# hyperplane-lab/RGBManip

Hardware: AMD Instinct MI355X
Metric: adapose_poses_per_sec_batch256 (higher is better)
Workload: dtype bf16

## Files before the change

include/rgbm.h:

```cpp
#ifndef RGBM_H_
#define RGBM_H_
#include <stddef.h>
#include <stdint.h>

#ifdef __cplusplus
extern "C" {
#endif

#define RGBM_VERSION 100
#define RGBM_F32 0
#define RGBM_BF16 1
#define RGBM_F16 2
#define RGBM_BF16X3 3

int rgbm_version(void);
const char* rgbm_last_error(void);

typedef struct rgbm_weight_desc {
  const char* name;
  const float* data;
  int ndim;
  const int64_t* shape;
} rgbm_weight_desc;

// ... 67 lines not shown
int rgbm_depth_fusion(const float* depth, const float* conf, const uint8_t* mask, const double* Kcrop, const double* E, int n, int V, int S,
                      double px_max, double rel_max, float conf_min, int n_min, float* fused, uint8_t* keep, uint8_t* nviews, uint16_t* agree,
                      void* stream);
int rgbm_cloud_pack_views(const float* fused, const uint8_t* keep, const double* Kcrop, const double* E, int n, int V, int S, int cap,
                          float* cloud, int32_t* index, int32_t* count, void* stream);
int rgbm_cloud_gather_views(const float* maps, const int32_t* index, int n, int V, int S2, int C, int cap, float* out, void* stream);

int rgbm_adapose_postprocess(int B, int P, int img_size, const float* nocs1, const float* depth1, const float* r1,
                             const int32_t* choose1, const double* Kcrop, const double* E1, double* bbox_world, double* ts,
                             int32_t* valid, void* stream);
int rgbm_adapose_postprocess_scratch_bytes(int B, size_t* bytes);
int rgbm_adapose_postprocess_ws(int B, int P, int img_size, const float* nocs1, const float* depth1, const float* r1,
                                const int32_t* choose1, const double* Kcrop, const double* E1, double* bbox_world, double* ts,
                                int32_t* valid, void* scratch, size_t scratch_bytes, void* stream);

int rgbm_adapose_postprocess_regressed(int B, int P, const float* nocs1, const float* r1, const float* t1, const float* s1,
                                       const double* E1, double* bbox_world, double* ts, int32_t* valid, void* stream);

int rgbm_adapose_postprocess_ransac(int B, int P, int img_size, uint32_t seed, const float* nocs1, const float* depth1,
                                    const int32_t* choose1, const double* Kcrop, const double* E1, double* bbox_world, double* srt,
                                    int32_t* valid, void* stream);
int rgbm_adapose_postprocess_pnp(int B, int P, uint32_t seed, const float* nocs1, const float* pts2d1, const float* nocs2,
                                 const float* pts2d2, const double* K, const double* E1, const double* E2, double* bbox_out,
                                 double* srt_out, int32_t* info_out, int32_t* valid_out, void* stream);

int rgbm_prepare_inputs(const float* rgb_dev, const uint8_t* mask_dev, const double* K_dev, int N, int H, int W, int S, int P,
                        uint32_t seed, float* img_out, int32_t* choose_out, float* pts2d_out, double* Kcrop_out,
                        int32_t* window_out, int32_t* valid_out, uint8_t* scratch, void* stream);

int rgbm_prepare_inputs_indexed(const float* rgb_dev, const uint8_t* mask_dev, const double* K_dev, const int32_t* frame_map_dev,
                                int N, int H, int W, int S, int P, uint32_t seed, float* img_out, int32_t* choose_out,
                                float* pts2d_out, double* Kcrop_out, int32_t* window_out, int32_t* valid_out, uint8_t* scratch,
                                void* stream);
int rgbm_prepare_inputs_ex(const float* rgb_dev, const uint8_t* mask_dev, const double* K_dev, const int32_t* frame_map_dev,
                           int frame0, int N, int H, int W, int S, int P, uint32_t seed, float* img_out, int32_t* choose_out,
                           float* pts2d_out, double* Kcrop_out, int32_t* window_out, int32_t* valid_out, uint8_t* scratch,
                           void* stream);
int rgbm_prepare_inputs_u8(const uint8_t* rgb_dev, const uint8_t* mask_dev, const double* K_dev, const int32_t* frame_map_dev,
                           int frame0, int N, int H, int W, int S, int P, uint32_t seed, float* img_out, int32_t* choose_out,
                           float* pts2d_out, double* Kcrop_out, int32_t* window_out, int32_t* valid_out, uint8_t* scratch,
                           void* stream);
int rgbm_prepare_inputs_opt(const void* rgb_dev, int pixel_type, int normalize, const uint8_t* mask_dev, const double* K_dev,
                            const int32_t* frame_map_dev, int frame0, int N, int H, int W, int S, int P, uint32_t seed, float* img_out,
                            int32_t* choose_out, float* pts2d_out, double* Kcrop_out, int32_t* window_out, int32_t* valid_out,
                            uint8_t* scratch, void* stream);
int rgbm_prepare_inputs_windows(const void* pix_dev, int pixel_type, int normalize, const uint8_t* mask_pix_dev, const int64_t* offset_dev,
                                const int32_t* window_dev, const int32_t* valid_in_dev, const double* K_dev, int frame0, int N, int H, int W,
                                int S, int P, uint32_t seed, float* img_out, int32_t* choose_out, float* pts2d_out, double* Kcrop_out,
                                int32_t* valid_out, uint8_t* scratch, void* stream);
int rgbm_quantize_frames(const float* src_dev, uint8_t* dst_dev, size_t n, void* stream);

int rgbm_projection(const double* Kcrop_dev, const double* E_dev, float* P_dev, int N, void* stream);
int rgbm_mask_extent(const uint8_t* mask_dev, int N, int H, int W, int32_t* ext_out, int32_t* count_out, void* stream);

int rgbm_lookat_quat(const double* dir_dev, int N, int batch_zero, double* quat_dev, void* stream);
int rgbm_control_action_to_pose(const float* action_dev, int lda, const double* pose_mid, const double* pose_min,
                                const double* pose_max, int N, double* pose_dev, void* stream);
typedef struct rgbm_control_reward_args {
  const float* action;
  const double* cam_pose;
  const double* target;
  const float* move_success;
  const double* bbox;
  const double* avail;
  const double* gt_bbox;
  const double* pred_bbox;
  const double* pose_cur;
  const double* pose_prev;
  const double* robot_pose;
  const double* success;
  double* reward;
  double* terms;
  double coef[14];
  double proper_pos[3];
  double precision2;
  int N, T, lda, pots, first;
  int pad_;
} rgbm_control_reward_args;
int rgbm_control_reward(const rgbm_control_reward_args* args, void* stream);
int rgbm_control_grasp_frame(const double* est_dev, int N, double* center_dev, double* direction_dev, void* stream);

typedef struct rgbm_synth_scene {
  const double* cam_pose;
  const double* robot_pose;
  const double* box;
  double fx, fy, cx, cy;
  int N, H, W, env0;
} rgbm_synth_scene;
int rgbm_synth_camera(const rgbm_synth_scene* scene, double* K_dev, double* E_dev, double* rays_dev, void* stream);
int rgbm_synth_render(const rgbm_synth_scene* scene, const double* rays_dev, float* color_dev, uint8_t* mask_dev, void* stream);
int rgbm_synth_render_u8(const rgbm_synth_scene* scene, const double* rays_dev, uint8_t* color_dev, uint8_t* mask_dev,
                         int32_t* extent_dev, int32_t* count_dev, void* stream);

int rgbm_gae(int T, int N, const float* rewards, const uint8_t* dones, const float* values, const float* last_values,
             float gamma, float lam, float* returns, float* adv, double* sums, void* stream);
int rgbm_adv_normalise(int64_t n_local, float* adv, const double* sums, double count_total, void* stream);

typedef struct rgbm_policy_layout {
  int dims[5];
  int log_std;
  int w[2][4];
  int b[2][4];
  int total;
} rgbm_policy_layout;
int rgbm_policy_forward(const float* params, const rgbm_policy_layout* L, int n, int mode, const float* obs, const float* noise,
                        float* actions, float* logp, float* value, float* mu, void* stream);
int rgbm_ppo_partial_floats(const rgbm_policy_layout* L, int n, size_t* count);
int rgbm_ppo_minibatch_fwd_bwd(const float* params, const rgbm_policy_layout* L, int n, const float* obs, const float* actions,
                               const float* old_logp, const float* adv, const float* returns, const float* old_values,
                               const float* old_mu, const float* old_log_std, float clip, float vcoef, float ecoef,
                               float* partial_scratch, float* grads_flat, void* stream);
int rgbm_ppo_clip_adam(float* params, const float* grads_flat, float* exp_avg, float* exp_avg_sq, void* opt_state,
                       const rgbm_policy_layout* L, float inv_world, float max_norm, float desired_kl, float lr_min,
                       float lr_max, int adaptive, void* stream);

#define RGBM_POLICY_MAX_HIDDEN 6
#define RGBM_POLICY_MAX_WIDTH 512
#define RGBM_POLICY_MAX_ACT 32
#define RGBM_ACT_ELU 0
#define RGBM_ACT_SELU 1
#define RGBM_ACT_RELU 2
#define RGBM_ACT_LRELU 3
#define RGBM_ACT_TANH 4
#define RGBM_ACT_SIGMOID 5
typedef struct rgbm_policy_desc {
  int obs_dim, state_dim, act_dim;
  int activation;
  int asymmetric;
  int n_hidden[2];
  int hidden[2][RGBM_POLICY_MAX_HIDDEN];
  int w[2][RGBM_POLICY_MAX_HIDDEN + 1];
  int b[2][RGBM_POLICY_MAX_HIDDEN + 1];
  int log_std;
  int total;
} rgbm_policy_desc;
int rgbm_policy_forward_ex(const float* params, const rgbm_policy_desc* D, int n, int mode, const float* obs, const float* states,
                           const float* noise, float* actions, float* logp, float* value, float* mu, void* stream);
int rgbm_ppo_scratch_floats_ex(const rgbm_policy_desc* D, int n, int clipped_value_loss, size_t* count);
int rgbm_ppo_minibatch_fwd_bwd_ex(const float* params, const rgbm_policy_desc* D, int n, const float* obs, const float* states,
                                  const float* actions, const float* old_logp, const float* adv, const float* returns,
                                  const float* old_values, const float* old_mu, const float* old_log_std, float clip, float vcoef,
                                  float ecoef, int clipped_value_loss, float* scratch, float* grads_flat, void* stream);
int rgbm_ppo_clip_adam_ex(float* params, const float* grads_flat, float* exp_avg, float* exp_avg_sq, void* opt_state, int total,
                          float inv_world, float max_norm, float desired_kl, float lr_min, float lr_max, int adaptive, void* stream);

int rgbm_conv_nd(int dtype, const void* in_dev, int N, int D, int H, int W, int Cin, int Cin_pad, const float* w_host,
                 int Cout, int Cout_pad, int KD, int KH, int KW, int stride_d, int stride_hw, int pad_d, int pad_hw,
                 int dil_hw, int transposed, const float* bias_host, const float* bn_scale_host, const float* bn_shift_host,
                 const void* res_dev, int res_mode, int act, float slope, void* out_dev, void* stream);
#define RGBM_CONV_PLAN_INTS 9
int rgbm_conv_plan(int dtype, int N, int D, int H, int W, int Cin, int Cin_pad, int Cout, int Cout_pad, int KD, int KH, int KW,
                   int stride_d, int stride_hw, int pad_d, int pad_hw, int dil_hw, int transposed, int has_bias, int res_mode, int act,
                   int cls, int n_cu, int32_t* plan);
int rgbm_bn_per_sample_scratch_bytes(int V, size_t* bytes);
int rgbm_bn_per_sample(int dtype, void* y_dev, const void* res_dev, const float* gamma_dev, const float* beta_dev, void* scratch_dev,
                       int V, int64_t nvox, int C, int relu, void* stream);
int rgbm_conv3d_tile(int layer, int dtype, const void* in_dev, int N, int D, int H, int W, const float* w_host,
                     const float* bn_scale_host, const float* bn_shift_host, const void* res_dev, void* out_dev, void* stream);
int rgbm_upsample_conv3x3(int dtype, const void* in_dev, int V, int h, int w, int Cin, const float* w_host, int Cout,
                          const float* bias_host, int act, float slope, void* z_scratch_dev, void* out_dev, void* stream);
int rgbm_upsample_conv3x3_final(int dtype, const void* in_dev, int V, int h, int w, const float* w3_host, const float* b3_host,
                                float slope, const float* wf_host, const float* bf_host, void* out_dev, int out_f32, void* stream);
int rgbm_stem(int dtype, const float* img1_dev, const float* img2_dev, const float* w_host, void* out_dev, int B, int S, void* stream);
int rgbm_maxpool3x3s2(int dtype, const void* in_dev, void* out_dev, int V, int H, int W, int C, void* stream);
int rgbm_resize_bilinear_ac(int dtype, const void* in_dev, void* out_dev, int V, int Hs, int Ws, int C, int Ho, int Wo,
                            void* stream);
int rgbm_adaptive_avgpool(int dtype, const void* in_dev, void* out_dev, int V, int H, int W, int C, int S, void* stream);
int rgbm_build_volume(int dtype, const void* feat_dev, const float* P_views_dev, const float* depths_dev, float* homog_scratch,
                      void* vol_dev, int V, int B, int D, int H, int W, void* stream);
int rgbm_conv0_sweep(const void* feat_dev, const float* P_views_dev, const float* depths_dev, float* homog_scratch,
                     const float* w_host, const float* bn_scale_host, const float* bn_shift_host, void* out_dev,
                     int V, int B, int D, int H, int W, void* stream);
int rgbm_conv0_sweep_dt(int dtype, const void* feat_dev, const float* P_views_dev, const float* depths_dev, float* homog_scratch,
                        const float* w_host, const float* bn_scale_host, const float* bn_shift_host, void* out_dev,
                        int V, int B, int D, int H, int W, void* stream);
int rgbm_conv0_sweep_f16feat(const void* feat_f16_dev, const float* P_views_dev, const float* depths_dev, float* homog_scratch,
                             const float* w_host, const float* bn_scale_host, const float* bn_shift_host, void* out_bf16_dev,
                             int V, int B, int D, int H, int W, void* stream);
int rgbm_adapose_forward_ex(rgbm_adapose_t* h, int B, const float* img1, const float* img2, const int32_t* choose1,
                            const int32_t* choose2, const float* P1, const float* P2, const float* depths, void* workspace,
                            size_t workspace_bytes, const rgbm_adapose_out* out, int stop_after, void* stream);
int rgbm_adapose_forward_graph(rgbm_adapose_t* h, int B, const float* img1, const float* img2, const int32_t* choose1,
                               const int32_t* choose2, const float* P1, const float* P2, const float* depths, void* workspace,
                               size_t workspace_bytes, const rgbm_adapose_out* out, void* stream, int32_t* n_nodes, int32_t* captured);
int rgbm_adapose_graph_clear(rgbm_adapose_t* h);
int rgbm_adapose_feature_bytes(rgbm_adapose_t* h, size_t* bytes);
int rgbm_adapose_features_workspace_bytes(rgbm_adapose_t* h, int V, size_t* bytes);
int rgbm_adapose_features(rgbm_adapose_t* h, int V, const float* img, const int32_t* slots_dev, void* pool, int pool_records,
                          void* workspace, size_t workspace_bytes, void* stream);
int rgbm_adapose_forward_cached(rgbm_adapose_t* h, int B, const void* pool, int pool_records, const int32_t* slot1_dev,
                                const int32_t* slot2_dev, const int32_t* choose1, const int32_t* choose2, const float* P1, const float* P2,
                                const float* depths, void* workspace, size_t workspace_bytes, const rgbm_adapose_out* out, void* stream);
int rgbm_adapose_fetch(rgbm_adapose_t* h, int B, void* workspace, const char* name, float* out_dev, size_t capacity,
                       size_t* n_elems, void* stream);
int rgbm_crop_fingerprint(const float* img, int V, int n_words, uint64_t* keys_out, void* stream);

#define RGBM_PROF_ROWS 42
int rgbm_debug_flags(int flags);
int rgbm_set_tuning(const char* key, long long value);
int rgbm_microbench_mfma_scratch_floats(int* n);
int rgbm_microbench_mfma(float* scratch, int iters, int random_operands, double* flops, void* stream);
int rgbm_microbench_copy(const void* src, void* dst, size_t bytes, void* stream);
int rgbm_prof_rows(void);
int rgbm_prof_start(void);
int rgbm_prof_stop(double* stats);
int rgbm_prof_select(int row);

#ifdef __cplusplus
}
#endif
#endif
```

rgbmanip_amd/_lib.py:

```python
from __future__ import annotations

import ctypes as C
import os

_HERE = os.path.dirname(os.path.abspath(__file__))
LIB_PATH = os.environ.get("RGBM_HIP_LIB") or os.path.join(_HERE, "librgbm_hip.so")

F32, BF16, F16, BF16X3 = 0, 1, 2, 3
ACT_NONE, ACT_RELU, ACT_PRELU, ACT_TANH = 0, 1, 2, 3
RES_NONE, RES_PRE_ACT, RES_POST_ACT = 0, 1, 2


PROF_ROWS = 42
PROF_KERNELS = [
    ("conv_igemm_glds_kernel<float, 16, 256>", "fp32"), ("conv_igemm_glds_kernel<float, 32, 256>", "fp32"),
    ("conv_igemm_glds_kernel<float, 64, 256>", "fp32"), ("conv_igemm_glds_kernel<float, 128, 128>", "fp32"),
    ("conv_igemm_glds_kernel<unsigned short, 16, 256>", "bf16"), ("conv_igemm_glds_kernel<unsigned short, 32, 256>", "bf16"),
    ("conv_igemm_glds_kernel<unsigned short, 64, 256>", "bf16"), ("conv_igemm_glds_kernel<unsigned short, 128, 128>", "bf16"),
    ("conv3d_tile_kernel<float, ...> (conv1..conv11)", "fp32"), ("conv3d_tile_kernel<unsigned short, ...> (conv1..conv11)", "bf16"),
    ("conv3d_tile_kernel<float, 32, 16, 4, 8, 8, 1, false, true> (conv0 + fused plane sweep)", "fp32"),
    ("conv3d_tile_kernel<unsigned short, 32, 16, 4, 8, 8, 1, false, true> (conv0 + fused plane sweep)", "bf16"),
    ("conv_igemm_ws_kernel<float, ...>", "fp32"), ("conv_igemm_ws_kernel<unsigned short, false, false> (128 channels x 256 pixels)", "bf16"),
    ("conv0_sweep_persistent_kernel<unsigned short> (conv0 + fused plane sweep of bf16 nets; sweep_f16 = 0 / fp16 nets: conv0_sweep_kernel)", "bf16"), ("conv_igemm_ws64_kernel", "bf16"),
    ("conv3d_tile_kernel<unsigned short, 32, 16, 6, 8, 8, 1, false, false> (conv0 on a materialised volume)", "bf16"),
    ("conv3d_tile_kernel<unsigned short, 8, 16, 2, 8, 8, 2, false, false> (conv1)", "bf16"),
    ("conv3d_tile_kernel<unsigned short, 16, 16, 4, 8, 8, 1, false, false> (conv2)", "bf16"),
    ("conv3d_tile_kernel<unsigned short, 16, 32, 2, 8, 8, 2, false, false> (conv3)", "bf16"),
    ("conv3d_tile_kernel<unsigned short, 32, 32, 2, 8, 8, 1, false, false> (conv4)", "bf16"),
    ("conv3d_tile_kernel<unsigned short, 32, 64, 1, 8, 8, 2, false, false> (conv5)", "bf16"),
    ("conv3d_tile_kernel<unsigned short, 64, 64, 1, 8, 8, 1, false, false> (conv6)", "bf16"),
    ("conv3d_tile_kernel<unsigned short, 64, 32, 1, 8, 8, 1, true, false> (conv7)", "bf16"),
    ("conv3d_tile_kernel<unsigned short, 32, 16, 2, 8, 8, 1, true, false> (conv9)", "bf16"),
    ("conv3d_tile_kernel<unsigned short, 16, 16, 4, 8, 8, 1, true, false> (conv11)", "bf16"),
] + [("conv_igemm_glds_kernel<bx3_t, ...> (all channel tiles)", "bf16x3"), ("conv3d_tile_kernel<bx3_t, ...> (conv1..conv11)", "bf16x3"),
     ("conv0 + fused plane sweep <bx3_t>", "bf16x3"), ("conv_igemm_ws_kernel<rgbm::bx3_t, false, false> (128 channels x 256 pixels)", "bf16x3"),
     ("pose_mlp1_kernel (pose_mlp1.0 + pose_mlp1.2 of a bf16 net in one launch)", "bf16"),
     ("conv_igemm_m32_kernel<unsigned short, 256, 256> (256 channels x 256 pixels, 32x32x16 MFMAs; gemm_kernel = 0: conv_igemm_ws_kernel<unsigned short, true, false>, 256 x 128)", "bf16"),
     ("pose_mlp2_kernel (pose_mlp2.0 + pose_mlp2.2 + the sum over points of a bf16 net in one launch)", "bf16"),
     ("conv_igemm_m32_kernel<rgbm::bx3_t, 256, 256> (256 channels x 256 pixels, 32x32x16 MFMAs; gemm_kernel = 0: conv_igemm_ws_kernel<rgbm::bx3_t, true, false>, 256 x 128)", "bf16x3"),
     ("conv_igemm_ws_kernel<rgbm::bx3_t, false, false, true> (64 channels x 256 pixels, four multiply waves)", "bf16x3"),
     ("conv_igemm_ws_kernel<unsigned short, false, false, true> (64 channels x 256 pixels, four multiply waves)", "bf16"),
     ("conv_igemm_ws_kernel<float, false, false, true> (64 channels x 256 pixels, four multiply waves)", "fp32"),
     ("upconv_combine_kernel<16-bit> (PSPUpsample tap combination)", "bf16"), ("upconv_combine_kernel<4-byte> (PSPUpsample tap combination)", "bf16x3"),
     ("upconv_final_kernel (up_3 + final in one kernel; either storage width)", "bf16"),
     ("conv_igemm_m32_kernel<unsigned short, 128, 64 / 128 / 256> (128-pixel tiles: tail and small-batch launches of the 256-channel GEMM)", "bf16"),
     ("conv_igemm_m32_kernel<rgbm::bx3_t, 128, 64 / 128 / 256> (128-pixel tiles: tail and small-batch launches of the 256-channel GEMM)", "bf16x3")]
assert len(PROF_KERNELS) == PROF_ROWS


class RgbmError(RuntimeError):
    pass


class WeightDesc(C.Structure):
    _fields_ = [("name", C.c_char_p), ("data", C.c_void_p), ("ndim", C.c_int), ("shape", C.POINTER(C.c_int64))]


class PolicyLayout(C.Structure):
    _fields_ = [("dims", C.c_int * 5), ("log_std", C.c_int), ("w", (C.c_int * 4) * 2), ("b", (C.c_int * 4) * 2), ("total", C.c_int)]


POLICY_MAX_HIDDEN, POLICY_MAX_WIDTH, POLICY_MAX_ACT = 6, 512, 32
POLICY_ACTIVATIONS = {"elu": 0, "selu": 1, "relu": 2, "crelu": 2, "lrelu": 3, "tanh": 4, "sigmoid": 5}


class PolicyDesc(C.Structure):
    _fields_ = [("obs_dim", C.c_int), ("state_dim", C.c_int), ("act_dim", C.c_int), ("activation", C.c_int), ("asymmetric", C.c_int),
                ("n_hidden", C.c_int * 2), ("hidden", (C.c_int * POLICY_MAX_HIDDEN) * 2),
                ("w", (C.c_int * (POLICY_MAX_HIDDEN + 1)) * 2), ("b", (C.c_int * (POLICY_MAX_HIDDEN + 1)) * 2),
                ("log_std", C.c_int), ("total", C.c_int)]


class AdaposeOut(C.Structure):
    _fields_ = [(n, C.c_void_p) for n in ("view1_nocs", "view2_nocs", "view1_depth", "view2_depth", "view1_r", "view2_r",
                                           "view1_t", "view2_t", "view1_s", "view2_s")]


class ControlRewardArgs(C.Structure):
    _fields_ = [(n, C.c_void_p) for n in ("action", "cam_pose", "target", "move_success", "bbox", "avail", "gt_bbox", "pred_bbox",
                                           "pose_cur", "pose_prev", "robot_pose", "success", "reward", "terms")] + [
        ("coef", C.c_double * 14), ("proper_pos", C.c_double * 3), ("precision2", C.c_double),
        ("N", C.c_int), ("T", C.c_int), ("lda", C.c_int), ("pots", C.c_int), ("first", C.c_int), ("pad_", C.c_int)]


class SynthScene(C.Structure):
    _fields_ = [("cam_pose", C.c_void_p), ("robot_pose", C.c_void_p), ("box", C.c_void_p),
                ("fx", C.c_double), ("fy", C.c_double), ("cx", C.c_double), ("cy", C.c_double),
                ("N", C.c_int), ("H", C.c_int), ("W", C.c_int), ("env0", C.c_int)]


_vp, _i, _f, _d, _sz, _i64 = C.c_void_p, C.c_int, C.c_float, C.c_double, C.c_size_t, C.c_int64

SIGNATURES = {
    "rgbm_version": (_i, []),
    "rgbm_last_error": (C.c_char_p, []),
    "rgbm_adapose_create": (_i, [C.POINTER(_vp), _i, C.POINTER(WeightDesc), _i, _i, _i]),
    "rgbm_adapose_create_baseline": (_i, [C.POINTER(_vp), _i, C.POINTER(WeightDesc), _i, _i, _i]),
    "rgbm_view_fusion": (_i, [_vp, _vp, _vp, _i, _i, _vp, _vp, _vp, _sz, _vp]),
    "rgbm_view_fusion_scratch_bytes": (_i, [_i, _i, C.POINTER(_sz)]),
    "rgbm_depth_head": (_i, [_vp, _vp, _i64, _vp, _vp]),
    "rgbm_adapose_destroy": (_i, [_vp]),
    "rgbm_adapose_set_chunk": (_i, [_vp, _i]),
    "rgbm_adapose_set_option": (_i, [_vp, C.c_char_p, _i]),
    "rgbm_adapose_workspace_bytes": (_i, [_vp, _i, C.POINTER(_sz)]),
    "rgbm_adapose_set_dropout": (_i, [_vp, _f, C.c_uint64]),
    "rgbm_adapose_dropout_masks": (_i, [_vp, _i, _vp]),
    "rgbm_adapose_set_dropout_masks": (_i, [_vp, _i, _vp]),
    "rgbm_adapose_forward": (_i, [_vp, _i, _vp, _vp, _vp, _vp, _vp, _vp, _vp, _vp, _sz, C.POINTER(AdaposeOut), _vp]),
    "rgbm_adapose_forward_ex": (_i, [_vp, _i, _vp, _vp, _vp, _vp, _vp, _vp, _vp, _vp, _sz, C.POINTER(AdaposeOut), _i, _vp]),
    "rgbm_adapose_forward_graph": (_i, [_vp, _i, _vp, _vp, _vp, _vp, _vp, _vp, _vp, _vp, _sz, C.POINTER(AdaposeOut), _vp, C.POINTER(C.c_int32),
                                        C.POINTER(C.c_int32)]),
    "rgbm_adapose_samples_workspace_bytes": (_i, [_vp, _i, _i, C.POINTER(_sz)]),
    "rgbm_adapose_forward_samples": (_i, [_vp, _i, _i, _vp, _vp, _vp, _vp, _vp, _vp, _vp, _vp, _sz, C.POINTER(AdaposeOut), _vp]),
    "rgbm_sample_box_stats": (_i, [_vp, _vp, _i, _i, _vp, _vp, _vp, _vp, _vp, _vp, _vp, _vp, _vp]),
    "rgbm_sample_point_stats": (_i, [_vp, _i, _i, _i64, _vp, _vp, _vp]),
    "rgbm_box_agreement": (_i, [_vp, _vp, _vp, _vp, _i] + [_vp] * 14),
    "rgbm_box_iou_matrix": (_i, [_vp, _vp, _vp, _vp, _i, _i, _i, _vp, _vp]),
    "rgbm_adapose_dense_workspace_bytes": (_i, [_vp, _i, C.POINTER(_sz)]),
    "rgbm_adapose_forward_dense": (_i, [_vp, _i, _vp, _vp, _vp, _vp, _vp, _vp, _vp, _vp, _sz, C.POINTER(AdaposeOut), _vp, _vp, _vp]),
    "rgbm_adapose_forward_maps": (_i, [_vp, _i, _vp, _vp, _vp, _vp, _vp, _vp, _vp, _vp, _sz, C.POINTER(AdaposeOut), _vp, _vp, _vp, _vp]),
    "rgbm_nocs_map": (_i, [_vp, _vp, _i, _i, _vp, _vp]),
    "rgbm_cloud_gather": (_i, [_vp, _vp, _vp, _i, _i, _i, _i, _vp, _vp]),
    "rgbm_cloud_similarity_scratch_bytes": (_i, [_i, _i, C.POINTER(_sz)]),
    "rgbm_cloud_similarity": (_i, [_vp, _vp, _vp, _i, _i, C.c_uint32, _vp, _vp, _vp, _vp, _vp, _sz, _vp]),
    "rgbm_depth_to_points": (_i, [_vp, _vp, _vp, _i, _i, _vp, _vp]),
    "rgbm_depth_consistency": (_i, [_vp, _vp, _vp, _vp, _vp, _vp, _vp, _vp, _i, _i, _d, _d, _f, _vp, _vp, _vp, _vp, _vp]),
    "rgbm_cloud_pack": (_i, [_vp, _vp, _vp, _vp, _vp, _vp, _vp, _vp, _i, _i, _i, _vp, _vp, _vp, _vp]),
    "rgbm_depth_fusion": (_i, [_vp, _vp, _vp, _vp, _vp, _i, _i, _i, _d, _d, _f, _i, _vp, _vp, _vp, _vp, _vp]),
    "rgbm_cloud_pack_views": (_i, [_vp, _vp, _vp, _vp, _i, _i, _i, _i, _vp, _vp, _vp, _vp]),
    "rgbm_cloud_gather_views": (_i, [_vp, _vp, _i, _i, _i, _i, _i, _vp, _vp]),
    "rgbm_adapose_graph_clear": (_i, [_vp]),
    "rgbm_adapose_feature_bytes": (_i, [_vp, C.POINTER(_sz)]),
    "rgbm_adapose_features_workspace_bytes": (_i, [_vp, _i, C.POINTER(_sz)]),
    "rgbm_adapose_features": (_i, [_vp, _i, _vp, _vp, _vp, _i, _vp, _sz, _vp]),
    "rgbm_adapose_forward_cached": (_i, [_vp, _i, _vp, _i, _vp, _vp, _vp, _vp, _vp, _vp, _vp, _vp, _sz, C.POINTER(AdaposeOut), _vp]),
    "rgbm_crop_fingerprint": (_i, [_vp, _i, _i, _vp, _vp]),
    "rgbm_adapose_fetch": (_i, [_vp, _i, _vp, C.c_char_p, _vp, _sz, C.POINTER(_sz), _vp]),
    "rgbm_adapose_postprocess": (_i, [_i, _i, _i, _vp, _vp, _vp, _vp, _vp, _vp, _vp, _vp, _vp, _vp]),
    "rgbm_adapose_postprocess_scratch_bytes": (_i, [_i, C.POINTER(_sz)]),
    "rgbm_adapose_postprocess_ws": (_i, [_i, _i, _i, _vp, _vp, _vp, _vp, _vp, _vp, _vp, _vp, _vp, _vp, _sz, _vp]),
    "rgbm_adapose_postprocess_regressed": (_i, [_i, _i, _vp, _vp, _vp, _vp, _vp, _vp, _vp, _vp, _vp]),
    "rgbm_adapose_postprocess_ransac": (_i, [_i, _i, _i, C.c_uint32, _vp, _vp, _vp, _vp, _vp, _vp, _vp, _vp, _vp]),
    "rgbm_adapose_postprocess_pnp": (_i, [_i, _i, C.c_uint32, _vp, _vp, _vp, _vp, _vp, _vp, _vp, _vp, _vp, _vp, _vp, _vp]),
    "rgbm_gae": (_i, [_i, _i, _vp, _vp, _vp, _vp, _f, _f, _vp, _vp, _vp, _vp]),
    "rgbm_adv_normalise": (_i, [_i64, _vp, _vp, _d, _vp]),
    "rgbm_policy_forward": (_i, [_vp, _vp, _i, _i, _vp, _vp, _vp, _vp, _vp, _vp, _vp]),
    "rgbm_ppo_partial_floats": (_i, [_vp, _i, C.POINTER(_sz)]),
    "rgbm_ppo_minibatch_fwd_bwd": (_i, [_vp, _vp, _i, _vp, _vp, _vp, _vp, _vp, _vp, _vp, _vp, _f, _f, _f, _vp, _vp, _vp]),
    "rgbm_ppo_clip_adam": (_i, [_vp, _vp, _vp, _vp, _vp, _vp, _f, _f, _f, _f, _f, _i, _vp]),
    "rgbm_policy_forward_ex": (_i, [_vp, _vp, _i, _i, _vp, _vp, _vp, _vp, _vp, _vp, _vp, _vp]),
    "rgbm_ppo_scratch_floats_ex": (_i, [_vp, _i, _i, C.POINTER(_sz)]),
    "rgbm_ppo_minibatch_fwd_bwd_ex": (_i, [_vp, _vp, _i, _vp, _vp, _vp, _vp, _vp, _vp, _vp, _vp, _vp, _f, _f, _f, _i, _vp, _vp, _vp]),
    "rgbm_ppo_clip_adam_ex": (_i, [_vp, _vp, _vp, _vp, _vp, _i, _f, _f, _f, _f, _f, _i, _vp]),
    "rgbm_conv_nd": (_i, [_i, _vp, _i, _i, _i, _i, _i, _i, _vp, _i, _i, _i, _i, _i, _i, _i, _i, _i, _i, _i, _vp, _vp, _vp,
                          _vp, _i, _i, _f, _vp, _vp]),
    "rgbm_conv_plan": (_i, [_i] * 23 + [C.POINTER(C.c_int32)]),
    "rgbm_bn_per_sample_scratch_bytes": (_i, [_i, C.POINTER(_sz)]),
    "rgbm_bn_per_sample": (_i, [_i, _vp, _vp, _vp, _vp, _vp, _i, _i64, _i, _i, _vp]),
    "rgbm_conv3d_tile": (_i, [_i, _i, _vp, _i, _i, _i, _i, _vp, _vp, _vp, _vp, _vp, _vp]),
    "rgbm_upsample_conv3x3": (_i, [_i, _vp, _i, _i, _i, _i, _vp, _i, _vp, _i, _f, _vp, _vp, _vp]),
    "rgbm_upsample_conv3x3_final": (_i, [_i, _vp, _i, _i, _i, _vp, _vp, _f, _vp, _vp, _vp, _i, _vp]),
    "rgbm_stem": (_i, [_i, _vp, _vp, _vp, _vp, _i, _i, _vp]),
    "rgbm_maxpool3x3s2": (_i, [_i, _vp, _vp, _i, _i, _i, _i, _vp]),
    "rgbm_resize_bilinear_ac": (_i, [_i, _vp, _vp, _i, _i, _i, _i, _i, _i, _vp]),
    "rgbm_adaptive_avgpool": (_i, [_i, _vp, _vp, _i, _i, _i, _i, _i, _vp]),
    "rgbm_build_volume": (_i, [_i, _vp, _vp, _vp, _vp, _vp, _i, _i, _i, _i, _i, _vp]),
    "rgbm_conv0_sweep": (_i, [_vp, _vp, _vp, _vp, _vp, _vp, _vp, _vp, _i, _i, _i, _i, _i, _vp]),
    "rgbm_conv0_sweep_dt": (_i, [_i, _vp, _vp, _vp, _vp, _vp, _vp, _vp, _vp, _i, _i, _i, _i, _i, _vp]),
    "rgbm_conv0_sweep_f16feat": (_i, [_vp, _vp, _vp, _vp, _vp, _vp, _vp, _vp, _i, _i, _i, _i, _i, _vp]),
    "rgbm_prepare_inputs": (_i, [_vp, _vp, _vp, _i, _i, _i, _i, _i, C.c_uint32, _vp, _vp, _vp, _vp, _vp, _vp, _vp, _vp]),
    "rgbm_prepare_inputs_indexed": (_i, [_vp, _vp, _vp, _vp, _i, _i, _i, _i, _i, C.c_uint32, _vp, _vp, _vp, _vp, _vp, _vp, _vp, _vp]),
    "rgbm_prepare_inputs_ex": (_i, [_vp, _vp, _vp, _vp, _i, _i, _i, _i, _i, _i, C.c_uint32, _vp, _vp, _vp, _vp, _vp, _vp, _vp, _vp]),
    "rgbm_prepare_inputs_u8": (_i, [_vp, _vp, _vp, _vp, _i, _i, _i, _i, _i, _i, C.c_uint32, _vp, _vp, _vp, _vp, _vp, _vp, _vp, _vp]),
    "rgbm_prepare_inputs_opt": (_i, [_vp, _i, _i, _vp, _vp, _vp, _i, _i, _i, _i, _i, _i, C.c_uint32, _vp, _vp, _vp, _vp, _vp, _vp, _vp, _vp]),
    "rgbm_prepare_inputs_windows": (_i, [_vp, _i, _i, _vp, _vp, _vp, _vp, _vp, _i, _i, _i, _i, _i, _i, C.c_uint32, _vp, _vp, _vp, _vp, _vp, _vp, _vp]),
    "rgbm_quantize_frames": (_i, [_vp, _vp, C.c_size_t, _vp]),
    "rgbm_projection": (_i, [_vp, _vp, _vp, _i, _vp]),
    "rgbm_mask_extent": (_i, [_vp, _i, _i, _i, _vp, _vp, _vp]),
    "rgbm_lookat_quat": (_i, [_vp, _i, _i, _vp, _vp]),
    "rgbm_control_action_to_pose": (_i, [_vp, _i, C.POINTER(C.c_double), C.POINTER(C.c_double), C.POINTER(C.c_double), _i, _vp, _vp]),
    "rgbm_control_reward": (_i, [C.POINTER(ControlRewardArgs), _vp]),
    "rgbm_control_grasp_frame": (_i, [_vp, _i, _vp, _vp, _vp]),
    "rgbm_synth_camera": (_i, [C.POINTER(SynthScene), _vp, _vp, _vp, _vp]),
    "rgbm_synth_render": (_i, [C.POINTER(SynthScene), _vp, _vp, _vp, _vp]),
    "rgbm_synth_render_u8": (_i, [C.POINTER(SynthScene), _vp, _vp, _vp, _vp, _vp, _vp]),
    "rgbm_debug_flags": (_i, [_i]),
    "rgbm_set_tuning": (_i, [C.c_char_p, _i64]),
    "rgbm_prof_rows": (_i, []),
    "rgbm_microbench_mfma_scratch_floats": (_i, [C.POINTER(C.c_int)]),
    "rgbm_microbench_mfma": (_i, [_vp, _i, _i, C.POINTER(C.c_double), _vp]),
    "rgbm_microbench_copy": (_i, [_vp, _vp, C.c_size_t, _vp]),
    "rgbm_prof_start": (_i, []),
    "rgbm_prof_select": (_i, [_i]),
    "rgbm_prof_stop": (_i, [C.POINTER(C.c_double)]),
}

_lib = None


def load():
    global _lib
    if _lib is not None:
        return _lib
    if not os.path.exists(LIB_PATH):
        raise RgbmError(f"{LIB_PATH} not found: build it with rgbmanip_amd/csrc/build.sh "
                        f"(or `python -c 'import __graft_entry__ as g; g.build()'`). There is no CPU fallback.")
    lib = C.CDLL(LIB_PATH)
    for name, (res, args) in SIGNATURES.items():
        fn = getattr(lib, name)
        fn.restype = res
        fn.argtypes = args
    if lib.rgbm_prof_rows() != PROF_ROWS:
        raise RgbmError(f"{LIB_PATH}: rgbm_prof_rows() = {lib.rgbm_prof_rows()}, this binding expects {PROF_ROWS} (stale build?)")
    _lib = lib
    return lib


def check(rc: int, what: str = ""):
    if rc != 0:
        msg = load().rgbm_last_error()
        raise RgbmError(f"{what} failed (code {rc}): {msg.decode() if msg else ''}")


def stream_ptr(stream=None):
    import torch
    s = stream if stream is not None else torch.cuda.current_stream()
    return C.c_void_p(s.cuda_stream)


def ptr(t):
    return C.c_void_p(t.data_ptr()) if t is not None else C.c_void_p(0)
```

rgbmanip_amd/csrc/adapose.cpp:

```cpp
#include "adapose.h"
#include "cost3d.h"
#include "sample_stats.h"
#include "view_fusion.h"

#include <math.h>
#include <string.h>

namespace rgbm {

static const int kLayerPlanes[4] = {64, 128, 256, 512};
static const int kLayerBlocks[4] = {3, 4, 6, 3};
static const int kLayerStride[4] = {1, 2, 1, 1};
static const int kLayerDil[4] = {1, 1, 2, 4};
static const int kPspBins[4] = {1, 2, 3, 6};
static const int kPspSmallViews = 32;


static const HostTensor* find(const StateDict& sd, const std::string& name) {
  auto it = sd.find(name);
  return it == sd.end() ? nullptr : &it->second;
}

#define GET(var, name)                                               \
  const HostTensor* var = find(sd, name);                            \
// ... 242 lines not shown
  }
  return 0;
}

bool AdaPose::feat_f32_only() const {
  return dtype == BF16X3 && cost_impl == 3 && sweep_w && norm_mode == 0 && !(g_debug_flags & DBG_TILE_CONV0);
}

bool AdaPose::feat_f16() const {
  return dtype == BF16 && sweep_f16 != 0 && cost_impl == 3 && sweep_w_f16 && norm_mode == 0 && !(g_debug_flags & DBG_TILE_CONV0) && (upconv & 4) &&
         tail.ready() && tail.f16_ready();
}

bool AdaPose::sparse_tail_active(bool dense) const {
  const bool b16 = dtype_size(dtype) == 2;
  return !dense && sparse_tail && norm_mode == 0 && cost_impl == 3 && (b16 || (dtype == BF16X3 && w11_x3));
}

bool AdaPose::sparse_active(bool dense) const {
  return sparse_dec != 0 && sparse_tail_active(dense) && sweep_w && !(g_debug_flags & DBG_TILE_CONV0);
}

int AdaPose::chunk_poses(int B) const {
  const int cap = max_chunk / 2 > 0 ? max_chunk / 2 : 1;
  return B < cap ? B : cap;
}

int AdaPose::chunk_views(int V) const {
  const int cap = norm_mode == 1 && max_chunk > 32 ? 32 : max_chunk;
  return V < cap ? V : cap;
}

int AdaPose::plan(int B, Arena& A, Buffers& bf) const {
  const int V = 2 * B, P = n_pts, S = img;
  const size_t es = dtype_size(dtype);
  const size_t VP = (size_t)V * P;
  bf.Pviews = (float*)A.alloc((size_t)V * 16 * 4);
  bf.homog = (float*)A.alloc((size_t)V * 12 * 4);
  bf.choose = (int*)A.alloc(VP * 4);
  bf.masks = (unsigned char*)A.alloc((size_t)V * sparse_mask_bytes_per_view(img));
  bf.sweep_list = (int*)A.alloc((size_t)V * ((img + 11) / 12) * ((img + 15) / 16) * 4);
  bf.sweep_count = (int*)A.alloc((size_t)(V + 64) * 4);
  bf.feat = A.alloc((size_t)V * S * S * 32 * es);
  bf.featf = dtype == BF16X3 ? (float*)A.alloc((size_t)V * S * S * 32 * 4) : nullptr;
  bf.X0 = (float*)A.alloc(VP * 32 * 4);
  bf.X1 = (float*)A.alloc(VP * 64 * 4);
  bf.H128 = (float*)A.alloc(VP * 128 * 4);
  bf.H64 = (float*)A.alloc(VP * 64 * 4);
  bf.nocs4 = (float*)A.alloc(VP * 4 * 4);
  bf.N32 = (float*)A.alloc(VP * 32 * 4);
  bf.PF96 = (float*)A.alloc(VP * 96 * 4);
  bf.PF96h = pose_dtype() == F16 ? A.alloc(VP * 96 * 2) : nullptr;
  bf.prob = (float*)A.alloc(VP * n_depth * 4);
  bf.depth = (float*)A.alloc(VP * 4);
  bf.Q128a = (float*)A.alloc(VP * 128 * 4);
  bf.Q128b = (float*)A.alloc(VP * 128 * 4);
  bf.G256a = (float*)A.alloc(VP * 256 * 4);
  bf.G256b = (float*)A.alloc(VP * 256 * 4);
  bf.glob = (float*)A.alloc((size_t)V * 128 * 4);
  bf.vbias = (float*)A.alloc((size_t)V * 256 * 4);
  bf.pf2 = (float*)A.alloc((size_t)V * 256 * 4);
  bf.h1 = (float*)A.alloc((size_t)V * 256 * 4);
  bf.h2 = (float*)A.alloc((size_t)V * 128 * 4);
  bf.r6 = (float*)A.alloc((size_t)V * 8 * 4);
  bf.R = (float*)A.alloc((size_t)V * 9 * 4);
  bf.tv = (float*)A.alloc((size_t)V * 4 * 4);
  bf.sv = (float*)A.alloc((size_t)V * 4 * 4);
  const size_t m0 = A.mark();
  bf.imgpad = A.alloc((size_t)V * S * S * img_cpad * es);
  bf.c1 = A.alloc((size_t)V * (S / 2) * (S / 2) * 64 * es);
  const size_t lbuf = (size_t)V * ((size_t)(S / 4) * (S / 4) * 64 > (size_t)(S / 8) * (S / 8) * 512 ? (size_t)(S / 4) * (S / 4) * 64 : (size_t)(S / 8) * (S / 8) * 512) * es;
  for (int i = 0; i < 4; ++i) bf.lb[i] = A.alloc(lbuf);
  for (int i = 0; i < 4; ++i) {
    bf.pooled[i] = A.alloc((size_t)V * kPspBins[i] * kPspBins[i] * 512 * es);
    bf.stage[i] = A.alloc((size_t)V * kPspBins[i] * kPspBins[i] * 128 * es);
  }
  const size_t f8 = (size_t)(S / 8) * (S / 8), f4 = (size_t)(S / 4) * (S / 4), f2 = (size_t)(S / 2) * (S / 2), f1 = (size_t)S * S;
  bf.cat = A.alloc((size_t)V * f8 * 1024 * es);
  bf.ups = A.alloc((size_t)V * f4 * 1024 * es);
  bf.u1 = A.alloc((size_t)V * f4 * 256 * es);
  bf.u2 = A.alloc((size_t)V * f2 * 64 * es);
  bf.u3 = A.alloc((size_t)V * f1 * 64 * es);
  A.release(m0);
  bf.fused = nullptr; bf.vf_scratch = nullptr;
  if (arch == ARCH_BASELINE) {
    bf.fused = (float*)A.alloc(VP * 32 * 4);
    bf.vf_scratch = A.alloc(view_fusion_scratch_bytes(chunk_poses(B), P));
    bf.vol = bf.bn_scratch = nullptr;
    for (auto& c : bf.c3) c = nullptr;
    A.release(m0);
    return 0;
  }
  const int Vc = chunk_views(V);
  const int D = n_depth;
  const size_t vox = (size_t)D * S * S;
  bf.vol = (cost_impl >= 2 && norm_mode == 0) ? nullptr : A.alloc((size_t)Vc * vox * 32 * es);
  bf.bn_scratch = norm_mode == 1 ? A.alloc(bn_scratch_bytes(Vc)) : nullptr;
  for (int l = 0; l < kCost3dLayers; ++l) bf.c3[l] = A.alloc(cost3d_out_elems(l, Vc, D, S) * es);
  A.release(m0);
  return 0;
}

size_t AdaPose::workspace_bytes(int B) const {
  Arena A(nullptr, 0);
  Buffers bf;
  plan(B, A, bf);
  return A.peak + 256;
}

int AdaPose::pspnet(const Buffers& bf, int Vout, const float* img1, const float* img2, const Call& call, int samples) const {
  const int S = img;
  int V = Vout / samples;
  hipStream_t s = call.stream;
  const float* drop = call.dropout != Dropout::None ? drop_masks.get<float>() : nullptr;
  int H = S / 2, W = S / 2;
  if (stem && stem_w) {
    if (img2 == nullptr) { if (int rc = launch_stem_views(dtype, img1, stem_w.get(), bf.lb[0], V, S, s)) return rc; }
    else if (int rc = launch_stem(dtype, img1, img2, stem_w.get(), bf.lb[0], V / 2, V, S, s)) return rc;
  } else {
    const size_t es = dtype_size(dtype);
    const int B = img2 == nullptr ? V : V / 2;
    if (int rc = launch_nchw_to_nhwc_pad(dtype, img1, bf.imgpad, B, 3, S, S, img_cpad, s)) return rc;
    if (img2 != nullptr)
      if (int rc = launch_nchw_to_nhwc_pad(dtype, img2, (char*)bf.imgpad + (size_t)B * S * S * img_cpad * es, B, 3, S, S, img_cpad, s)) return rc;
    if (int rc = conv1.run(bf.imgpad, bf.c1, V, 1, S, S, 64, nullptr, 0, nullptr, 0, s)) return rc;
    if (int rc = launch_maxpool3x3s2(dtype, bf.c1, bf.lb[0], V, H, W, 64, s)) return rc;
  }
  H = S / 4; W = S / 4;
  int xi = 0;
  for (int i = 0; i < n_blocks; ++i) {
    const Block& blk = blocks[i];
    void* x = bf.lb[xi];
    void* t = bf.lb[(xi + 1) & 3];
    void* r = bf.lb[(xi + 2) & 3];
    void* y = bf.lb[(xi + 3) & 3];
    int Do, Ho, Wo;
    blk.c1.out_dims(1, H, W, Do, Ho, Wo);
    if (int rc = blk.c1.run(x, t, V, 1, H, W, blk.planes, nullptr, 0, nullptr, 0, s)) return rc;
    const void* res = x;
    if (blk.has_ds) {
      if (int rc = blk.ds.run(x, r, V, 1, H, W, blk.planes, nullptr, 0, nullptr, 0, s)) return rc;
      res = r;
    }
    if (int rc = blk.c2.run(t, y, V, 1, Ho, Wo, blk.planes, res, RES_PRE_ACT, nullptr, 0, s)) return rc;
    H = Ho; W = Wo;
    xi = (xi + 3) & 3;
  }
  const void* f = bf.lb[xi];
  RGBM_REQUIRE(H == S / 8 && W == S / 8, "feature stride");
  if (g_debug_flags & DBG_PSP_STAGE_R5) {
    if (int rc = launch_copy_channels(dtype, f, bf.cat, (long long)V * H * W, 512, 1024, 0, s)) return rc;
    {
      void* outs[4] = {bf.pooled[0], bf.pooled[1], bf.pooled[2], bf.pooled[3]};
      if (int rc = launch_adaptive_avgpool_multi(dtype, f, outs, kPspBins, 4, V, H, W, 512, s)) return rc;
    }
    for (int i = 0; i < 4; ++i) {
      const int Sb = kPspBins[i];
      if (int rc = psp[i].run(bf.pooled[i], bf.stage[i], V, 1, Sb, Sb, 128, nullptr, 0, nullptr, 0, s)) return rc;
      if (int rc = launch_resize_bilinear_ac(dtype, bf.stage[i], bf.cat, V, Sb, Sb, 128, H, W, 1024, 512 + 128 * i, s)) return rc;
    }
  } else {
    bool small = V <= kPspSmallViews;
    for (int i = 0; i < 4; ++i)
      small = small && psp[i].packs.size() == 1 && psp[i].packs[0].Kpad == 512 && psp[i].Cout_pad == 128 && !psp[i].bias;
    if (small) {
      const void* w[4] = {psp[0].packs[0].w.get(), psp[1].packs[0].w.get(), psp[2].packs[0].w.get(), psp[3].packs[0].w.get()};
      void* outs[4] = {bf.stage[0], bf.stage[1], bf.stage[2], bf.stage[3]};
      if (int rc = launch_psp_pool_conv(dtype, f, 512, w, outs, kPspBins, V, H, W, psp[0].g.act, psp[0].g.slope, s)) return rc;
    } else {
      void* outs[4] = {bf.pooled[0], bf.pooled[1], bf.pooled[2], bf.pooled[3]};
      if (int rc = launch_adaptive_avgpool_multi(dtype, f, outs, kPspBins, 4, V, H, W, 512, s)) return rc;
      for (int i = 0; i < 4; ++i)
        if (int rc = psp[i].run(bf.pooled[i], bf.stage[i], V, 1, kPspBins[i], kPspBins[i], 128, nullptr, 0, nullptr, 0, s)) return rc;
    }
    const void* stages[4] = {bf.stage[0], bf.stage[1], bf.stage[2], bf.stage[3]};
    if (int rc = launch_psp_resize_cat(dtype, f, stages, kPspBins, bf.cat, V, H, W, s)) return rc;
  }
  RGBM_REQUIRE(drop == nullptr || (upconv & 3) == 3, "dropout needs option upconv bits 0 and 1 (up_1 / up_2 through the tap combination)");
  if (samples > 1) {
    RGBM_REQUIRE(drop != nullptr && (upconv & 3) == 3 && img2 != nullptr && V % 2 == 0, "pspnet: samples need Dropout2d masks and both views");
    const int B = V / 2;
    const size_t zview = up1c.scratch_elems(1, H, W) * dtype_size(dtype), oview = (size_t)4 * H * W * 256 * dtype_size(dtype);
    if (int rc = up1c.run_gemm(bf.cat, bf.ups, V, H, W, s)) return rc;
    for (int half = 0; half < 2; ++half)
      for (int k = 0; k < samples; ++k) {
        const size_t row = (size_t)half * samples * B + (size_t)k * B;
        if (int rc = up1c.combine((const char*)bf.ups + (size_t)half * B * zview, (char*)bf.u1 + row * oview, B, H, W, 256, s,
                                  drop + row * kDropoutPerView)) return rc;
      }
    V = Vout;
  } else if (upconv & 1) {
    if (int rc = up1c.run(bf.cat, bf.ups, bf.u1, V, H, W, 256, s, drop)) return rc;
  } else {
    if (int rc = launch_resize_bilinear_ac(dtype, bf.cat, bf.ups, V, H, W, 1024, 2 * H, 2 * W, 1024, 0, s)) return rc;
    if (int rc = up1.run(bf.ups, bf.u1, V, 1, 2 * H, 2 * W, 256, nullptr, 0, nullptr, 0, s)) return rc;
  }
  if (upconv & 2) {
    if (int rc = up2c.run(bf.u1, bf.ups, bf.u2, V, 2 * H, 2 * W, 64, s, drop ? drop + 256 : nullptr)) return rc;
  } else {
    if (int rc = launch_resize_bilinear_ac(dtype, bf.u1, bf.ups, V, 2 * H, 2 * W, 256, 4 * H, 4 * W, 256, 0, s)) return rc;
    if (int rc = up2.run(bf.ups, bf.u2, V, 1, 4 * H, 4 * W, 64, nullptr, 0, nullptr, 0, s)) return rc;
  }
  const bool plain_f32 = feat_f32_only();
  if ((upconv & 4) && tail.ready())
    return tail.run(bf.u2, plain_f32 ? (void*)bf.featf : bf.feat, plain_f32 ? 1 : feat_f16() ? 2 : 0, V, 4 * H, 4 * W, s);
  if (int rc = launch_resize_bilinear_ac(dtype, bf.u2, bf.ups, V, 4 * H, 4 * W, 64, 8 * H, 8 * W, 64, 0, s)) return rc;
  return up3.run_then_1x1(fin, bf.ups, bf.u3, 64, plain_f32 ? (void*)bf.featf : bf.feat, 32, V, 1, 8 * H, 8 * W, fuse_final != 0, nullptr, s, plain_f32);
}

int AdaPose::cost_volume(const Buffers& bf, int V, int B, const float* depths, const Call& call) const {
  const int S = img, D = n_depth, P = n_pts;
  hipStream_t s = call.stream;
  const int Vh = view2_heads ? V : B;
  const int Vc0 = chunk_views(V);
  const bool b16 = dtype_size(dtype) == 2;
  struct Layer3d { const void* in; void* out; const void* res; int div, C; };
  Layer3d l3d[kCost3dLayers];
  for (int i = 0; i < kCost3dLayers; ++i)
    l3d[i] = {i == 0 ? bf.vol : bf.c3[i - 1], bf.c3[i], kCost3d[i].skip >= 0 ? bf.c3[kCost3d[i].skip] : nullptr, kCost3d[i].in_div, kCost3d[i].cout};
  void* const u11 = bf.c3[kCost3dLayers - 1];
  bool sweep_sparse = false;
  auto tile = [&](int layer, const Layer3d& l, int Vc, int v0, const unsigned char* tmask) -> int {
    const int li = layer == 10 ? 0 : layer;
    const int Cin = kCost3d[li].cin, Cout = kCost3d[li].cout, qi = l.div, qo = cost3d_out_div(li);
    const bool transposed = kCost3d[li].transposed;
    const int Di = D / qi, Hi = S / qi, Wi = S / qi, Do = D / qo, Ho = S / qo, Wo = S / qo;
    const void* res = l.res;
    Conv3dTileDesc d;
    memset(&d, 0, sizeof(d));
    d.in = layer == 10 ? nullptr : l.in; d.wgt = t3d[li].w.get(); d.out = l.out; d.bias = t3d[li].bias.get<float>(); d.res = res;
    d.N = Vc; d.Di = Di; d.Hi = Hi; d.Wi = Wi; d.Do = Do; d.Ho = Ho; d.Wo = Wo;
    d.Dq = transposed ? Di : Do; d.Hq = transposed ? Hi : Ho; d.Wq = transposed ? Wi : Wo;
    d.Cout = Cout; d.relu = 1;
    d.feat = bf.feat; d.homog = bf.homog; d.depths = depths; d.v0 = v0; d.V = V; d.B = B;
    d.out_classmajor = layer == 9 ? 1 : 0;
    d.tile_mask = tmask;
    d.tile_mask_stride = sparse_mask_bytes_per_view(S);
    if (layer == 10 && sweep_sparse) { d.tile_list = bf.sweep_list; d.tile_count = bf.sweep_count; }
    d.prof_variant = dtype == BF16X3 ? (layer == 10 ? 28 : 27) : layer == 10 ? 10 + (dtype != F32 ? 1 : 0) : (dtype != F32 ? 16 + layer : 8);
    d.algo_flops = 2.0 * Vc * (double)(transposed ? Di * Hi * Wi : Do * Ho * Wo) * Cout * 27.0 * Cin;
    d.algo_bytes = ((layer == 10 ? (double)Vc * Hi * Wi * Cin : (double)Vc * Di * Hi * Wi * Cin) +
                    (double)Vc * Do * Ho * Wo * Cout * (res ? 2 : 1)) * (double)dtype_size(dtype);
    if (layer == 10 && cost_impl == 3 && b16 && sweep_w && !(g_debug_flags & DBG_TILE_CONV0)) {
      d.wgt = sweep_w.get();
      if (feat_f16()) { d.wgt = sweep_w_f16.get(); d.feat_f16 = 1; }
      return launch_conv0_sweep(d, dtype, s);
    }
    if (layer == 10 && cost_impl == 3 && dtype == BF16X3 && sweep_w && !(g_debug_flags & DBG_TILE_CONV0)) {
      d.wgt = sweep_w.get();
      d.feat = bf.featf;
      return launch_conv0_sweep_x3(d, s);
    }
    return launch_conv3d_tile(layer, dtype, d, s);
  };
  const bool sparse_ok = sparse_active(call.dense);
  for (int v0 = 0; v0 < Vh; v0 += Vc0) {
    const int Vc = Vh - v0 < Vc0 ? Vh - v0 : Vc0;
    int classmajor = 0;
    if (norm_mode == 1) {
      if (int rc = launch_build_volume(dtype, bf.feat, bf.homog, depths, bf.vol, v0, Vc, V, B, D, S, S, s)) return rc;
      for (int i = 0; i < 10; ++i) {
        const Layer3d& l = l3d[i];
        const ConvLayer& L = c3d_raw[i];
        int Do, Ho, Wo;
        L.out_dims(D / l.div, S / l.div, S / l.div, Do, Ho, Wo);
        if (int rc = L.run(l.in, l.out, Vc, D / l.div, S / l.div, S / l.div, l.C, nullptr, RES_NONE, nullptr, 0, s)) return rc;
        if (int rc = launch_bn_per_sample(dtype, l.out, l.res, bn_gamma[i].get<float>(), bn_beta[i].get<float>(), bf.bn_scratch, Vc,
                                          (long long)Do * Ho * Wo, l.C, 1, s)) return rc;
      }
    } else if (cost_impl == 0) {
      if (int rc = launch_build_volume(dtype, bf.feat, bf.homog, depths, bf.vol, v0, Vc, V, B, D, S, S, s)) return rc;
      for (int i = 0; i < 10; ++i) {
        const Layer3d& l = l3d[i];
        if (int rc = c3d[i].run(l.in, l.out, Vc, D / l.div, S / l.div, S / l.div, l.C, l.res, RES_POST_ACT, nullptr, 0, s)) return rc;
      }
    } else {
      const unsigned char* mk[10] = {nullptr, nullptr, nullptr, nullptr, nullptr, nullptr, nullptr, nullptr, nullptr, nullptr};
      sweep_sparse = false;
      if (sparse_ok) {
        int td, th, tw;
        for (int L : {1, 2, 3, 4, 5, 7, 8}) RGBM_REQUIRE(!conv3d_tile_dims(L, dtype, &td, &th, &tw) && th == 8 && tw == 8, "sparse cost regularisation: 8 x 8 tiles expected");
        if (int rc = launch_sparse_masks(bf.choose, v0, Vc, P, S, bf.masks, bf.sweep_list, bf.sweep_count, s)) return rc;
        for (int L : {7, 8}) mk[L] = bf.masks + sparse_mask_offset(S, L);
        if (sparse_dec >= 2) {
          for (int L : {1, 2, 3, 4, 5}) mk[L] = bf.masks + sparse_mask_offset(S, L);
          sweep_sparse = true;
        }
      }
      const bool tail_sparse = sparse_tail_active(call.dense);
      for (int i = 0; i < (tail_sparse ? 9 : kCost3dLayers); ++i) {
        const Layer3d& l = l3d[i];
        if (i == 0 && cost_impl == 1) {
          if (int rc = launch_build_volume(dtype, bf.feat, bf.homog, depths, bf.vol, v0, Vc, V, B, D, S, S, s)) return rc;
          if (int rc = tile(0, l, Vc, v0, nullptr)) return rc;
        } else if (i == 0) {
          if (int rc = tile(10, l, Vc, v0, nullptr)) return rc;
        } else if (i == 6 && cost_impl == 3 && (b16 || dtype == BF16X3) && igemm_conv6) {
          if (int rc = c3d[6].run(l.in, l.out, Vc, D / l.div, S / l.div, S / l.div, l.C, nullptr, RES_NONE, nullptr, 0, s)) return rc;
        } else {
          if (int rc = tile(i, l, Vc, v0, mk[i])) return rc;
        }
      }
      if (tail_sparse) {
        if (int rc = launch_prob_sparse(l3d[9].in, l3d[9].res, dtype == BF16X3 ? w11_x3.get() : t3d[9].w.get(), t3d[9].bias.get<float>(),
                                        wprob.get<float>(), bf.choose, depths, bf.prob, bf.depth, v0, Vc, B, P, D, S, S, dtype, s, w11_taps.get())) return rc;
        continue;
      }
      classmajor = 1;
    }
    if (int rc = launch_prob_softmax_depth(dtype, u11, wprob.get<float>(), bf.choose, depths, bf.prob, bf.depth, v0, Vc, B, P, D, S, S, classmajor, s)) return rc;
    if (call.depth_map != nullptr)
      if (int rc = launch_dense_depth(dtype, u11, wprob.get<float>(), depths, call.depth_map, call.conf_map, v0, Vc, B, D, S, S, classmajor, s)) return rc;
  }
  return 0;
}

int AdaPose::forward(int B, const float* img1, const float* img2, const int* choose1, const int* choose2, const float* P1,
                     const float* P2, const float* depths, void* workspace, size_t workspace_size, const Outputs& out,
                     const Call& call) const {
  RGBM_REQUIRE(call.depth_map == nullptr || call.dense, "forward: depth_map needs a dense call");
  RGBM_REQUIRE(call.depth_map != nullptr || call.conf_map == nullptr, "forward_maps: conf_map without depth_map");
  RGBM_REQUIRE(call.nocs_map == nullptr || pmlp_table, "forward_maps: no point MLP table");
  RGBM_REQUIRE(B > 0, "batch");
  RGBM_REQUIRE(arch != ARCH_BASELINE || !(call.dense || call.depth_map || call.conf_map || call.nocs_map),
               "baseline network: the dense / maps forwards are not implemented (they read the cost volume this network does not have)");
  RGBM_REQUIRE(arch != ARCH_BASELINE || call.dropout == Dropout::None, "baseline network: Dropout2d is not implemented");
  RGBM_REQUIRE(((uintptr_t)workspace & 255) == 0, "workspace must be 256-byte aligned");
  RGBM_REQUIRE(n_depth % 8 == 0 && img % 8 == 0, "depth/img must be multiples of 8");
  const size_t need = workspace_bytes(B);
// ... 274 lines not shown
```

rgbmanip_amd/csrc/capi.cpp:

```cpp
#include "../../include/rgbm.h"

#include <string.h>

#include <algorithm>
#include <initializer_list>
#include <memory>
#include <string>
#include <utility>
#include <vector>

#include "adapose.h"
#include "box_overlap.h"
#include "control.h"
#include "cost3d.h"
#include "conv_plan.h"
#include "prof.h"
#include "sample_stats.h"
#include "view_fusion.h"

using namespace rgbm;

struct ForwardGraph {
  int B = 0;
  hipStream_t stream = nullptr;
// ... 419 lines not shown
  hipStream_t s = call.stream;
  RGBM_REQUIRE(s != nullptr, "forward_graph: stream capture is not allowed on the default (null) stream; pass a created stream");
  auto forward = [&](const AdaPose::Call& c) {
    return h->net.forward(B, img1, img2, choose1, choose2, P1, P2, depths, workspace, workspace_bytes, to_out(out), c);
  };
  const void* in[7] = {img1, img2, choose1, choose2, P1, P2, depths};
  ForwardGraph* hit = nullptr;
  for (size_t i = 0; i < h->graphs.size();) {
    ForwardGraph& g = h->graphs[i];
    if (g.opt_version != h->opt_version || g.tuning_version != g_tuning_version) {
      drop_graph(g);
      h->graphs.erase(h->graphs.begin() + i);
      continue;
    }
    if (g.B == B && g.stream == s && !memcmp(g.in, in, sizeof(in)) && g.ws == workspace && g.ws_bytes == workspace_bytes &&
        !memcmp(&g.out, out, sizeof(*out))) hit = &g;
    ++i;
  }
  if (!hit) {
    AdaPose::Call warm = call;
    if (call.dropout == AdaPose::Dropout::Draw) warm.dropout = AdaPose::Dropout::DrawNoAdvance;
    if (int rw = forward(warm)) return rw;
    ForwardGraph g;
    g.B = B; g.stream = s; memcpy(g.in, in, sizeof(in)); g.ws = workspace; g.ws_bytes = workspace_bytes; g.out = *out;
    g.opt_version = h->opt_version; g.tuning_version = g_tuning_version;
    RGBM_CHECK_HIP(hipStreamBeginCapture(s, hipStreamCaptureModeThreadLocal));
    const int rc = forward(call);
    const hipError_t ee = hipStreamEndCapture(s, &g.graph);
    if (rc) { if (g.graph) (void)hipGraphDestroy(g.graph); return rc; }
    if (ee != hipSuccess || !g.graph) { set_error(std::string("hipStreamEndCapture: ") + hipGetErrorString(ee)); return -2; }
    if (hipGraphGetNodes(g.graph, nullptr, &g.nodes) != hipSuccess) g.nodes = 0;
    const hipError_t ei = hipGraphInstantiate(&g.exec, g.graph, nullptr, nullptr, 0);
    if (ei != hipSuccess) { (void)hipGraphDestroy(g.graph); set_error(std::string("hipGraphInstantiate: ") + hipGetErrorString(ei)); return -2; }
    if (h->graphs.size() >= kMaxGraphs) {
      size_t lru = 0;
      for (size_t i = 1; i < h->graphs.size(); ++i) if (h->graphs[i].last_use < h->graphs[lru].last_use) lru = i;
      drop_graph(h->graphs[lru]);
      h->graphs.erase(h->graphs.begin() + lru);
    }
    h->graphs.push_back(g);
    hit = &h->graphs.back();
    if (captured) *captured = 1;
  }
  hit->last_use = ++h->tick;
  if (n_nodes) *n_nodes = (int32_t)hit->nodes;
  RGBM_CHECK_HIP(hipGraphLaunch(hit->exec, s));
  return finish_call(h, B, call, 0);
}

int rgbm_adapose_fetch(rgbm_adapose_t* h, int B, void* workspace, const char* name, float* out_dev, size_t capacity,
                       size_t* n_elems, void* stream) {
  RGBM_REQUIRE(h && workspace && name && out_dev && n_elems, "fetch arguments");
  const AdaPose& n = h->net;
  Arena A(workspace, 0);
  AdaPose::Buffers bf;
  n.plan(B, A, bf);
  const size_t V = 2 * (size_t)B, S = n.img, P = n.n_pts, D = n.n_depth;
  const size_t Vc = n.chunk_views((int)V);
  const std::string nm = name;
  const void* src = nullptr; size_t cnt = 0; int dt = n.dtype;
  if (nm == "imgpad") { src = bf.imgpad; cnt = V * S * S * n.img_cpad; }
  else if (nm == "conv1") { src = bf.c1; cnt = V * (S / 2) * (S / 2) * 64; }
  else if (nm == "layer4") { src = bf.lb[n.layer4_index()]; cnt = V * (S / 8) * (S / 8) * 512; }
  else if (nm == "cat") { src = bf.cat; cnt = V * (S / 8) * (S / 8) * 1024; }
  else if (nm == "u1") { src = bf.u1; cnt = V * (S / 4) * (S / 4) * 256; }
  else if (nm == "u2") { src = bf.u2; cnt = V * (S / 2) * (S / 2) * 64; }
  else if (nm == "u3") { src = bf.u3; cnt = V * S * S * 64; }
  else if (nm == "feat") { src = bf.feat; cnt = V * S * S * 32; if (n.feat_f32_only()) { src = bf.featf; dt = F32; } else if (n.feat_f16()) dt = F16; }
  else if (nm == "vol") { src = bf.vol; cnt = Vc * D * S * S * 32; }
  else if (nm == "homog") { src = bf.homog; cnt = V * 12; dt = F32; }
  else if (nm == "prob") { src = bf.prob; cnt = V * P * D; dt = F32; }
  else if (nm == "pf96") { src = bf.PF96; cnt = V * P * 96; dt = n.pose_dtype() == BF16X3 ? BF16X3 : F32; }
  else if (nm == "pf2") { src = bf.pf2; cnt = V * 256; dt = F32; }
  else if (nm == "r6") { src = bf.r6; cnt = V * 6; dt = F32; }
  else if (nm == "fused1" && bf.fused) { src = bf.fused; cnt = (size_t)B * P * 32; dt = F32; }
  else if (nm == "fused2" && bf.fused) { src = bf.fused + (size_t)B * P * 32; cnt = (size_t)B * P * 32; dt = F32; }
  static const struct { const char* name; int row; } taps3d[] = {{"c0", 0}, {"c2", 2}, {"c4", 4}, {"c6", 6}, {"u7", 7}, {"u9", 8}, {"u11", 9}};
  int row3d = -1;
  for (const auto& t : taps3d)
    if (nm == t.name) { row3d = t.row; src = bf.c3[row3d]; cnt = cost3d_out_elems(row3d, (int)Vc, (int)D, (int)S); }
  if (is_baseline(h))
    RGBM_REQUIRE(nm == "feat" || nm == "fused1" || nm == "fused2" || nm == "pf96" || nm == "pf2" || nm == "r6" || nm == "layer4" || nm == "cat" ||
                 nm == "u1" || nm == "u2", "tap '" + nm + "' does not exist in the baseline network");
  RGBM_REQUIRE(src != nullptr, "unknown intermediate name: " + nm);
  const bool tap3d = row3d >= 0 && row3d < 9;
  RGBM_REQUIRE(!(tap3d && n.sparse_active()), "tap '" + nm + "' needs a dense cost regularisation: set option sparse_dec = 0 before the forward "
               "(the default computes it only inside the chosen pixels' dependency cones)");
  *n_elems = cnt;
  RGBM_REQUIRE(cnt <= capacity, "fetch capacity too small");
  return launch_to_f32(dt, src, out_dev, (long long)cnt, (hipStream_t)stream);
}

int rgbm_adapose_postprocess(int B, int P, int img_size, const float* nocs1, const float* depth1, const float* r1,
                             const int32_t* choose1, const double* Kcrop, const double* E1, double* bbox_world, double* ts,
                             int32_t* valid, void* stream) {
  RGBM_REQUIRE(B > 0 && nocs1 && depth1 && r1 && choose1 && Kcrop && E1 && bbox_world && ts && valid, "postprocess arguments");
  return launch_postprocess(nocs1, depth1, r1, choose1, Kcrop, E1, bbox_world, ts, valid, B, P, img_size, (hipStream_t)stream);
}

int rgbm_adapose_postprocess_scratch_bytes(int B, size_t* bytes) {
  RGBM_REQUIRE(B > 0 && bytes, "postprocess_scratch_bytes arguments");
  *bytes = postprocess_slices(B) > 1 ? postprocess_scratch_bytes(B) : 0;
  return 0;
}

int rgbm_adapose_postprocess_ws(int B, int P, int img_size, const float* nocs1, const float* depth1, const float* r1,
                                const int32_t* choose1, const double* Kcrop, const double* E1, double* bbox_world, double* ts,
                                int32_t* valid, void* scratch, size_t scratch_bytes, void* stream) {
  RGBM_REQUIRE(B > 0 && nocs1 && depth1 && r1 && choose1 && Kcrop && E1 && bbox_world && ts && valid, "postprocess arguments");
  return launch_postprocess(nocs1, depth1, r1, choose1, Kcrop, E1, bbox_world, ts, valid, B, P, img_size, (hipStream_t)stream,
                            scratch, scratch_bytes);
}

int rgbm_adapose_postprocess_ransac(int B, int P, int img_size, uint32_t seed, const float* nocs1, const float* depth1,
                                    const int32_t* choose1, const double* Kcrop, const double* E1, double* bbox_world, double* srt,
                                    int32_t* valid, void* stream) {
  return launch_umeyama_ransac(nocs1, depth1, choose1, Kcrop, E1, bbox_world, srt, valid, B, P, img_size, seed, (hipStream_t)stream);
}

int rgbm_gae(int T, int N, const float* rewards, const uint8_t* dones, const float* values, const float* last_values,
             float gamma, float lam, float* returns, float* adv, double* sums, void* stream) {
  RGBM_REQUIRE(rewards && dones && values && last_values && returns && adv && sums, "gae arguments");
  return launch_gae(T, N, rewards, dones, values, last_values, gamma, lam, returns, adv, sums, (hipStream_t)stream);
}

int rgbm_adv_normalise(int64_t n_local, float* adv, const double* sums, double count_total, void* stream) {
  RGBM_REQUIRE(adv && sums && n_local > 0 && count_total > 1.0, "adv_normalise arguments");
  return launch_adv_normalise(n_local, adv, sums, count_total, (hipStream_t)stream);
}

static ConvGeom conv_nd_geom(int Cin, int Cout, int KD, int KH, int KW, int stride_d, int stride_hw, int pad_d, int pad_hw, int dil_hw,
                             int transposed, int act, float slope) {
  ConvGeom g;
  g.Cin = Cin; g.Cout = Cout; g.KD = KD; g.KH = KH; g.KW = KW;
  g.sd = stride_d; g.sh = g.sw = stride_hw; g.pd = pad_d; g.ph = g.pw = pad_hw;
  g.dild = 1; g.dilh = g.dilw = dil_hw; g.transposed = transposed != 0; g.act = act; g.slope = slope;
  return g;
}

int rgbm_conv_nd(int dtype, const void* in_dev, int N, int D, int H, int W, int Cin, int Cin_pad, const float* w_host,
                 int Cout, int Cout_pad, int KD, int KH, int KW, int stride_d, int stride_hw, int pad_d, int pad_hw,
                 int dil_hw, int transposed, const float* bias_host, const float* bn_scale_host, const float* bn_shift_host,
                 const void* res_dev, int res_mode, int act, float slope, void* out_dev, void* stream) {
  RGBM_REQUIRE(in_dev && w_host && out_dev, "conv arguments");
  const ConvGeom g = conv_nd_geom(Cin, Cout, KD, KH, KW, stride_d, stride_hw, pad_d, pad_hw, dil_hw, transposed, act, slope);
  ConvLayer L;
  if (int rc = L.init(dtype, g, w_host, bias_host, bn_scale_host, bn_shift_host, Cin_pad, Cout_pad)) return rc;
  return finish_one_shot(L.run(in_dev, out_dev, N, D, H, W, Cout_pad, res_dev, res_mode, nullptr, 0, (hipStream_t)stream), stream);
}

int rgbm_conv_plan(int dtype, int N, int D, int H, int W, int Cin, int Cin_pad, int Cout, int Cout_pad, int KD, int KH, int KW,
                   int stride_d, int stride_hw, int pad_d, int pad_hw, int dil_hw, int transposed, int has_bias, int res_mode, int act,
                   int cls, int n_cu, int32_t* plan) {
  RGBM_REQUIRE(plan && n_cu >= 0 && dtype >= F32 && dtype <= BF16X3 && N > 0 && D > 0 && H > 0 && W > 0, "conv_plan arguments");
  const ConvGeom g = conv_nd_geom(Cin, Cout, KD, KH, KW, stride_d, stride_hw, pad_d, pad_hw, dil_hw, transposed, act, 0.f);
  PackedConv pc;
  if (int rc = conv_pack_geom(g, dtype, Cin_pad, Cout_pad, cls, &pc)) return rc;
  ConvDesc d;
  conv_desc_geom(d, g, pc, Cin_pad, Cout_pad, N, D, H, W, Cout_pad, cls);
  alignas(16) static const float buffer[4] = {};
  d.in = d.wgt = buffer; d.out = const_cast<float*>(buffer);
  d.bias = has_bias ? buffer : nullptr;
  d.res = res_mode != RES_NONE ? buffer : nullptr;
  d.res_mode = res_mode;
  ConvTuning t;
  ConvPlan p;
  if (int rc = conv_tuning(n_cu, &t)) return rc;
  if (int rc = plan_conv(d, dtype, t, &p)) return rc;
  const int32_t v[RGBM_CONV_PLAN_INTS] = {p.kernel, p.bch, p.bpix, p.ksplit, (int32_t)p.main_rows, p.tail_bch, p.identity_residual, (int32_t)d.M, d.KT};
  memcpy(plan, v, sizeof(v));
  return 0;
}

int rgbm_upsample_conv3x3(int dtype, const void* in_dev, int V, int h, int w, int Cin, const float* w_host, int Cout,
                          const float* bias_host, int act, float slope, void* z_scratch_dev, void* out_dev, void* stream) {
  RGBM_REQUIRE(in_dev && w_host && z_scratch_dev && out_dev, "upsample_conv3x3 arguments");
  UpConvLayer L;
  if (int rc = L.init(dtype, Cin, Cout, w_host, bias_host, act, slope)) return rc;
  return finish_one_shot(L.run(in_dev, z_scratch_dev, out_dev, V, h, w, Cout, (hipStream_t)stream), stream);
}

int rgbm_upsample_conv3x3_final(int dtype, const void* in_dev, int V, int h, int w, const float* w3_host, const float* b3_host,
                                float slope, const float* wf_host, const float* bf_host, void* out_dev, int out_f32, void* stream) {
  RGBM_REQUIRE(in_dev && w3_host && b3_host && wf_host && bf_host && out_dev, "upsample_conv3x3_final arguments");
  UpConvFinal L;
  if (int rc = L.init(dtype, w3_host, b3_host, slope, wf_host, bf_host)) return rc;
  return finish_one_shot(L.run(in_dev, out_dev, out_f32, V, h, w, (hipStream_t)stream), stream);
}

int rgbm_stem(int dtype, const float* img1_dev, const float* img2_dev, const float* w_host, void* out_dev, int B, int S, void* stream) {
  RGBM_REQUIRE(img1_dev && img2_dev && w_host && out_dev && B > 0, "stem arguments");
  std::vector<float> pk;
  stem_pack(w_host, pk);
  DevBuf wd;
  if (int rc = upload_packed(pk, dtype, wd)) return rc;
  return finish_one_shot(launch_stem(dtype, img1_dev, img2_dev, wd.get(), out_dev, B, 2 * B, S, (hipStream_t)stream), stream);
}

int rgbm_bn_per_sample_scratch_bytes(int V, size_t* bytes) {
  RGBM_REQUIRE(V > 0 && bytes, "bn_per_sample_scratch_bytes arguments");
  *bytes = bn_scratch_bytes(V);
  return 0;
}
int rgbm_bn_per_sample(int dtype, void* y_dev, const void* res_dev, const float* gamma_dev, const float* beta_dev, void* scratch_dev,
                       int V, int64_t nvox, int C, int relu, void* stream) {
  RGBM_REQUIRE(y_dev && gamma_dev && beta_dev && scratch_dev, "bn_per_sample arguments");
  return launch_bn_per_sample(dtype, y_dev, res_dev, gamma_dev, beta_dev, scratch_dev, V, (long long)nvox, C, relu, (hipStream_t)stream);
}
int rgbm_maxpool3x3s2(int dtype, const void* in_dev, void* out_dev, int V, int H, int W, int C, void* stream) {
  return launch_maxpool3x3s2(dtype, in_dev, out_dev, V, H, W, C, (hipStream_t)stream);
}
int rgbm_resize_bilinear_ac(int dtype, const void* in_dev, void* out_dev, int V, int Hs, int Ws, int C, int Ho, int Wo,
                            void* stream) {
  return launch_resize_bilinear_ac(dtype, in_dev, out_dev, V, Hs, Ws, C, Ho, Wo, C, 0, (hipStream_t)stream);
}
int rgbm_adaptive_avgpool(int dtype, const void* in_dev, void* out_dev, int V, int H, int W, int C, int S, void* stream) {
  return launch_adaptive_avgpool(dtype, in_dev, out_dev, V, H, W, C, S, (hipStream_t)stream);
}
int rgbm_build_volume(int dtype, const void* feat_dev, const float* P_views_dev, const float* depths_dev, float* homog_scratch,
                      void* vol_dev, int V, int B, int D, int H, int W, void* stream) {
  if (int rc = launch_homography(P_views_dev, homog_scratch, V, B, (hipStream_t)stream)) return rc;
  return launch_build_volume(dtype, feat_dev, homog_scratch, depths_dev, vol_dev, 0, V, V, B, D, H, W, (hipStream_t)stream);
}

}

#include "prof.h"
extern "C" {
int rgbm_prof_rows(void) { return rgbm::kProfVariants; }
int rgbm_microbench_mfma_scratch_floats(int* n) {
  RGBM_REQUIRE(n, "microbench_mfma_scratch_floats arguments");
  return rgbm::microbench_mfma_scratch_floats(n);
}
int rgbm_microbench_mfma(float* scratch, int iters, int random_operands, double* flops, void* stream) {
  return rgbm::launch_microbench_mfma(scratch, iters, random_operands, flops, (hipStream_t)stream);
}
int rgbm_microbench_copy(const void* src, void* dst, size_t bytes, void* stream) {
  return rgbm::launch_microbench_copy(src, dst, bytes, (hipStream_t)stream);
}
int rgbm_prof_start(void) { return rgbm::prof_start(); }
int rgbm_prof_select(int row) {
  RGBM_REQUIRE(row >= -1 && row < rgbm::kProfVariants, "prof_select: row out of range");
  return rgbm::prof_select(row);
}
int rgbm_prof_stop(double* stats) {
  RGBM_REQUIRE(stats != nullptr, "prof_stop arguments");
  return rgbm::prof_stop(stats, rgbm::kProfVariants);
}
}

extern "C" int rgbm_conv3d_tile(int layer, int dtype, const void* in_dev, int N, int D, int H, int W, const float* w_host,
                                const float* bn_scale_host, const float* bn_shift_host, const void* res_dev, void* out_dev,
                                void* stream) {
  RGBM_REQUIRE(layer >= 0 && layer < kCost3dLayers && in_dev && w_host && bn_scale_host && bn_shift_host && out_dev, "conv3d_tile arguments");
  const Cost3dLayer& L = kCost3d[layer];
  const int coutp = cost3d_coutp(layer);
  std::vector<float> packed;
  conv3d_tile_pack(w_host, bn_scale_host, L.cin, L.cout, coutp, L.transposed, dtype, packed);
  DevBuf wdev, bdev;
  if (upload_packed(packed, dtype, wdev)) return -2;
  std::vector<float> bpad(coutp, 0.f);
  for (int o = 0; o < L.cout; ++o) bpad[o] = bn_shift_host[o];
  if (upload_f32(bpad.data(), bpad.size(), bdev)) return -2;
  Conv3dTileDesc d;
  memset(&d, 0, sizeof(d));
  d.in = in_dev; d.wgt = wdev.get(); d.out = out_dev; d.bias = bdev.get<float>(); d.res = res_dev;
  d.N = N; d.Di = D; d.Hi = H; d.Wi = W;
  if (L.transposed) { d.Do = 2 * D; d.Ho = 2 * H; d.Wo = 2 * W; d.Dq = D; d.Hq = H; d.Wq = W; }
  else {
    const int s = L.stride;
    d.Do = (D + 2 - 3) / s + 1; d.Ho = (H + 2 - 3) / s + 1; d.Wo = (W + 2 - 3) / s + 1;
    d.Dq = d.Do; d.Hq = d.Ho; d.Wq = d.Wo;
  }
  d.Cout = L.cout; d.relu = 1; d.prof_variant = -1;
  return finish_one_shot(launch_conv3d_tile(layer, dtype, d, (hipStream_t)stream), stream);
}

static int conv0_sweep_entry(int dtype, int feat_f16, const void* feat_dev, const float* P_views_dev, const float* depths_dev,
                             float* homog_scratch, const float* w_host, const float* bn_scale_host, const float* bn_shift_host,
                             void* out_dev, int V, int B, int D, int H, int W, void* stream) {
  RGBM_REQUIRE(feat_dev && P_views_dev && depths_dev && homog_scratch && w_host && bn_scale_host && bn_shift_host && out_dev,
               "conv0_sweep arguments");
  RGBM_REQUIRE(dtype == BF16 || dtype == F16 || dtype == BF16X3, "conv0_sweep: 16-bit storage types or bf16x3 (fp32 features in, split-pair c0 out)");
  if (int rc = launch_homography(P_views_dev, homog_scratch, V, B, (hipStream_t)stream)) return rc;
  std::vector<float> packed;
  conv0_sweep_pack(w_host, bn_scale_host, packed);
  DevBuf wdev, bdev;
  if (dtype == BF16X3) { if (conv0_sweep_x3_upload(packed, wdev.out())) return -2; }
  else if (upload_packed(packed, feat_f16 ? (int)F16 : dtype, wdev)) return -2;
  std::vector<float> bpad(cost3d_coutp(0), 0.f);
  for (int o = 0; o < kCost3d[0].cout; ++o) bpad[o] = bn_shift_host[o];
  if (upload_f32(bpad.data(), bpad.size(), bdev)) return -2;
  Conv3dTileDesc d;
  memset(&d, 0, sizeof(d));
  d.wgt = wdev.get(); d.out = out_dev; d.bias = bdev.get<float>();
  d.N = V; d.Di = D; d.Hi = H; d.Wi = W; d.Do = D; d.Ho = H; d.Wo = W; d.Dq = D; d.Hq = H; d.Wq = W;
  d.Cout = kCost3d[0].cout; d.relu = 1; d.prof_variant = -1;
  d.feat = feat_dev; d.homog = homog_scratch; d.depths = depths_dev; d.v0 = 0; d.V = V; d.B = B;
  d.feat_f16 = feat_f16;
  return finish_one_shot(dtype == BF16X3 ? launch_conv0_sweep_x3(d, (hipStream_t)stream) : launch_conv0_sweep(d, dtype, (hipStream_t)stream), stream);
}

extern "C" int rgbm_conv0_sweep_dt(int dtype, const void* feat_dev, const float* P_views_dev, const float* depths_dev,
                                   float* homog_scratch, const float* w_host, const float* bn_scale_host, const float* bn_shift_host,
                                   void* out_dev, int V, int B, int D, int H, int W, void* stream) {
  return conv0_sweep_entry(dtype, 0, feat_dev, P_views_dev, depths_dev, homog_scratch, w_host, bn_scale_host, bn_shift_host, out_dev, V, B, D,
                           H, W, stream);
}

extern "C" int rgbm_conv0_sweep_f16feat(const void* feat_f16_dev, const float* P_views_dev, const float* depths_dev,
                                        float* homog_scratch, const float* w_host, const float* bn_scale_host,
                                        const float* bn_shift_host, void* out_bf16_dev, int V, int B, int D, int H, int W, void* stream) {
  return conv0_sweep_entry(BF16, 1, feat_f16_dev, P_views_dev, depths_dev, homog_scratch, w_host, bn_scale_host, bn_shift_host, out_bf16_dev,
                           V, B, D, H, W, stream);
}

extern "C" int rgbm_conv0_sweep(const void* feat_dev, const float* P_views_dev, const float* depths_dev, float* homog_scratch,
                                const float* w_host, const float* bn_scale_host, const float* bn_shift_host, void* out_dev,
                                int V, int B, int D, int H, int W, void* stream) {
  return rgbm_conv0_sweep_dt(BF16, feat_dev, P_views_dev, depths_dev, homog_scratch, w_host, bn_scale_host, bn_shift_host, out_dev,
                             V, B, D, H, W, stream);
}

extern "C" int rgbm_prepare_inputs(const float* rgb_dev, const uint8_t* mask_dev, const double* K_dev, int N, int H, int W, int S,
                                   int P, uint32_t seed, float* img_out, int32_t* choose_out, float* pts2d_out, double* Kcrop_out,
                                   int32_t* window_out, int32_t* valid_out, uint8_t* scratch, void* stream) {
  return launch_prepare_inputs(rgb_dev, mask_dev, K_dev, nullptr, N, H, W, S, P, seed, img_out, choose_out, pts2d_out, Kcrop_out,
                               window_out, valid_out, scratch, (hipStream_t)stream);
}

extern "C" int rgbm_prepare_inputs_indexed(const float* rgb_dev, const uint8_t* mask_dev, const double* K_dev,
                                           const int32_t* frame_map_dev, int N, int H, int W, int S, int P, uint32_t seed,
                                           float* img_out, int32_t* choose_out, float* pts2d_out, double* Kcrop_out,
                                           int32_t* window_out, int32_t* valid_out, uint8_t* scratch, void* stream) {
  RGBM_REQUIRE(frame_map_dev, "prepare_inputs_indexed frame_map");
  return launch_prepare_inputs(rgb_dev, mask_dev, K_dev, frame_map_dev, N, H, W, S, P, seed, img_out, choose_out, pts2d_out,
                               Kcrop_out, window_out, valid_out, scratch, (hipStream_t)stream);
}

extern "C" int rgbm_prepare_inputs_ex(const float* rgb_dev, const uint8_t* mask_dev, const double* K_dev, const int32_t* frame_map_dev,
                                      int frame0, int N, int H, int W, int S, int P, uint32_t seed, float* img_out, int32_t* choose_out,
                                      float* pts2d_out, double* Kcrop_out, int32_t* window_out, int32_t* valid_out, uint8_t* scratch,
                                      void* stream) {
  RGBM_REQUIRE(frame0 >= 0, "prepare_inputs_ex frame0");
  return launch_prepare_inputs(rgb_dev, mask_dev, K_dev, frame_map_dev, N, H, W, S, P, seed, img_out, choose_out, pts2d_out,
                               Kcrop_out, window_out, valid_out, scratch, (hipStream_t)stream, frame0);
}

extern "C" int rgbm_prepare_inputs_u8(const uint8_t* rgb_dev, const uint8_t* mask_dev, const double* K_dev, const int32_t* frame_map_dev,
                                      int frame0, int N, int H, int W, int S, int P, uint32_t seed, float* img_out, int32_t* choose_out,
                                      float* pts2d_out, double* Kcrop_out, int32_t* window_out, int32_t* valid_out, uint8_t* scratch,
                                      void* stream) {
  RGBM_REQUIRE(frame0 >= 0, "prepare_inputs_u8 frame0");
  return launch_prepare_inputs_u8(rgb_dev, mask_dev, K_dev, frame_map_dev, N, H, W, S, P, seed, img_out, choose_out, pts2d_out,
                                  Kcrop_out, window_out, valid_out, scratch, (hipStream_t)stream, frame0);
}

extern "C" int rgbm_prepare_inputs_opt(const void* rgb_dev, int pixel_type, int normalize, const uint8_t* mask_dev, const double* K_dev,
                                       const int32_t* frame_map_dev, int frame0, int N, int H, int W, int S, int P, uint32_t seed,
                                       float* img_out, int32_t* choose_out, float* pts2d_out, double* Kcrop_out, int32_t* window_out,
                                       int32_t* valid_out, uint8_t* scratch, void* stream) {
  RGBM_REQUIRE(frame0 >= 0, "prepare_inputs_opt frame0");
  return launch_prepare_inputs_opt(rgb_dev, pixel_type, normalize, mask_dev, K_dev, frame_map_dev, N, H, W, S, P, seed, img_out, choose_out,
                                   pts2d_out, Kcrop_out, window_out, valid_out, scratch, (hipStream_t)stream, frame0);
}

extern "C" int rgbm_prepare_inputs_windows(const void* pix_dev, int pixel_type, int normalize, const uint8_t* mask_pix_dev,
                                           const int64_t* offset_dev, const int32_t* window_dev, const int32_t* valid_in_dev, const double* K_dev,
                                           int frame0, int N, int H, int W, int S, int P, uint32_t seed, float* img_out, int32_t* choose_out,
                                           float* pts2d_out, double* Kcrop_out, int32_t* valid_out, uint8_t* scratch, void* stream) {
// ... 141 lines not shown
```

rgbmanip_amd/csrc/conv_igemm_glds.hip:

```cpp
#include <map>
#include <mutex>
#include <type_traits>
#include <vector>
#include "common.h"
#include "conv_plan.h"
#include "kernels.h"
#include "prof.h"

#ifndef WS_BUF
#define WS_BUF 1
#endif

namespace rgbm {

int g_gemm_kernel = 2;
__device__ uint4 g_zero_page[4];

typedef __attribute__((address_space(3))) void* lds_ptr_t;
typedef const __attribute__((address_space(1))) void* gbl_ptr_t;

__device__ __forceinline__ void glds16(const void* gsrc, unsigned lds_off) {
  asm volatile("s_mov_b32 m0, %1\n\ts_nop 0\n\tglobal_load_lds_dwordx4 %0, off" :: "v"(gsrc), "s"(lds_off) : "memory");
}
__device__ __forceinline__ void blds16(unsigned voff, const __amdgpu_buffer_rsrc_t& rsrc, unsigned soff, unsigned lds_off) {
// ... 1041 lines not shown
    for (int b = 0; b < FN; ++b) {
      const long long m = (long long)pix_tile * BPIX + wpix + b * 16 + lr;
      pok[b] = m < d.M;
      if (dense_out && (interior || d.bias_stride == 0)) {
        nn[b] = 0;
        obase[b] = (pok[b] ? m : 0ll) * d.ldo;
        continue;
      }
      unsigned n, qd, qh, qw;
      decode_row(d, pok[b] ? (unsigned)m : 0u, n, qd, qh, qw);
      nn[b] = (int)n;
      obase[b] = ((((long long)n * d.Do + (qd * d.osd + d.opd)) * d.Ho + (qh * d.osh + d.oph)) * d.Wo + (qw * d.osw + d.opw)) * d.ldo;
    }
    const int chL = ch_tile * BCH + wch + lg * 16;
    constexpr int CHK = 16 / (int)sizeof(T);
    constexpr int NQ = 16 / CHK;
    if (interior) {
      const float nslope = d.act == ACT_RELU ? 0.f : d.act == ACT_PRELU ? d.slope : 1.f;
      auto fast = [&](auto resc) {
        constexpr int RES = decltype(resc)::value;
        constexpr int GRP = 2;
#pragma unroll
        for (int bh = 0; bh < FN; bh += GRP) {
          uint4 rr[NQ][GRP];
          if (RES != RES_NONE) {
#pragma unroll
            for (int bb = 0; bb < GRP; ++bb)
#pragma unroll
              for (int q = 0; q < NQ; ++q)
                rr[q][bb] = *reinterpret_cast<const uint4*>(res + obase[bh + bb] + chL + q * CHK);
          }
#pragma unroll
          for (int bb = 0; bb < GRP; ++bb) {
            const int b = bh + bb;
#pragma unroll
            for (int q = 0; q < NQ; ++q) {
              float v[CHK], rv[CHK];
#pragma unroll
              for (int e = 0; e < CHK; ++e) v[e] = acc[(q * CHK + e) >> 2][b][(q * CHK + e) & 3];
              if (RES != RES_NONE) unpack_chunk(rr[q][bb], rv, T());
              if (RES == RES_PRE_ACT) {
#pragma unroll
                for (int e = 0; e < CHK; ++e) v[e] += rv[e];
              }
#pragma unroll
              for (int e = 0; e < CHK; ++e) v[e] = v[e] < 0.f ? __builtin_fmaxf(v[e], -3.402823466e38f) * nslope : v[e];
              if (RES == RES_POST_ACT) {
#pragma unroll
                for (int e = 0; e < CHK; ++e) v[e] += rv[e];
              }
              const uint4 pk = pack_chunk(v, T());
              *reinterpret_cast<uint4*>(out + obase[b] + chL + q * CHK) = pk;
            }
          }
        }
      };
      if (d.res_mode == RES_NONE) fast(IC<RES_NONE>{});
      else if (d.res_mode == RES_PRE_ACT) fast(IC<RES_PRE_ACT>{});
      else fast(IC<RES_POST_ACT>{});
      continue;
    }
#pragma unroll
    for (int bh = 0; bh < FN; bh += 2) {
      uint4 rr[NQ][2];
#pragma unroll
      for (int bb = 0; bb < 2; ++bb)
#pragma unroll
        for (int q = 0; q < NQ; ++q) rr[q][bb] = make_uint4(0u, 0u, 0u, 0u);
      if (d.res_mode != RES_NONE) {
#pragma unroll
        for (int bb = 0; bb < 2; ++bb)
#pragma unroll
          for (int q = 0; q < NQ; ++q) {
            const int c = chL + q * CHK;
            const bool ok = pok[bh + bb] && c + CHK <= d.Cout;
            rr[q][bb] = *reinterpret_cast<const uint4*>(res + (ok ? obase[bh + bb] + c : 0ll));
          }
      }
#pragma unroll
      for (int bb = 0; bb < 2; ++bb) {
        const int b = bh + bb;
#pragma unroll
        for (int q = 0; q < NQ; ++q) {
          const int c = chL + q * CHK;
          if (!pok[b] || c >= d.Cout) continue;
          const bool whole = c + CHK <= d.Cout;
          float v[CHK], rv[CHK];
#pragma unroll
          for (int e = 0; e < CHK; ++e) v[e] = acc[(q * CHK + e) >> 2][b][(q * CHK + e) & 3];
          if (d.bias) {
            const float* bp = d.bias + (long long)nn[b] * d.bias_stride + c;
#pragma unroll
            for (int e = 0; e < CHK; ++e) if (e < 4 || whole) v[e] += bp[e];
          }
#pragma unroll
          for (int e = 0; e < CHK; ++e) rv[e] = 0.f;
          if (d.res_mode != RES_NONE) {
            if (whole) unpack_chunk(rr[q][bb], rv, T());
            else load4(res + obase[b] + c, rv);
          }
          if (d.res_mode == RES_PRE_ACT) {
#pragma unroll
            for (int e = 0; e < CHK; ++e) v[e] += rv[e];
          }
#pragma unroll
          for (int e = 0; e < CHK; ++e) v[e] = apply_act_g(v[e], d.act, d.slope);
          if (d.res_mode == RES_POST_ACT) {
#pragma unroll
            for (int e = 0; e < CHK; ++e) v[e] += rv[e];
          }
          if (whole) *reinterpret_cast<uint4*>(out + obase[b] + c) = pack_chunk(v, T());
          else store4(out + obase[b] + c, v);
        }
      }
    }
  }
}

static void make_fastdiv(int dvs, unsigned& m, int& sh) {
  int s = 0;
  while ((1ll << s) < (long long)dvs) ++s;
  sh = 31 + s;
  m = (unsigned)(((1ull << sh) + (unsigned long long)dvs - 1ull) / (unsigned long long)dvs);
}

template <typename T, bool WIDE, bool RH, bool SLIM = false>
static int launch_ws(ConvDesc d, const ConvPlan& p, hipStream_t s) {
  constexpr int BCH = SLIM ? 64 : WIDE ? 256 : 128, BPIX = (WIDE && !SLIM) ? 128 : 256;
  constexpr size_t LDS = (RH ? (3 * (size_t)(BCH + 136) * 8 + 8) : 3 * (size_t)(BCH + BPIX) * 8) * sizeof(uint4) + 2048 * sizeof(float);
  d.n_pix_tiles = (int)((d.M + BPIX - 1) / BPIX);
  d.n_ch_tiles = (d.Cout + BCH - 1) / BCH;
  const long long ntiles = (long long)d.n_pix_tiles * d.n_ch_tiles;
  RGBM_REQUIRE(ntiles > 0 && ntiles < (1ll << 31) && d.M < (1ll << 31), "conv grid out of range");
  d.n_tiles = (int)ntiles;
  make_fastdiv(d.Wq, d.fd_m[0], d.fd_s[0]);
  make_fastdiv(d.Hq, d.fd_m[1], d.fd_s[1]);
  make_fastdiv(d.Dq, d.fd_m[2], d.fd_s[2]);
  d.korder = p.korder;
  d.buf_ok = p.buf_ok;
  if (int rc = ensure_dynamic_lds(reinterpret_cast<const void*>(conv_igemm_ws_kernel<T, WIDE, RH, SLIM>), (int)LDS)) return rc;
  int n_cu = 0;
  if (int rc = persistent_grid_cus(&n_cu)) return rc;
  const int grid = ntiles < n_cu ? (int)ntiles : n_cu;
  prof_begin_launch(s, SLIM ? (std::is_same<T, bx3_t>::value ? 34 : sizeof(T) == 2 ? 35 : 36) : RH ? 32 : WIDE && sizeof(T) == 2 ? 31 : WIDE && std::is_same<T, bx3_t>::value ? 33 : prof_row_ws<T>(), d.algo_flops, d.algo_bytes);
  hipLaunchKernelGGL((conv_igemm_ws_kernel<T, WIDE, RH, SLIM>), dim3((unsigned)grid), dim3(SLIM ? 512 : 768), LDS, s, d);
  prof_end_launch(s);
  RGBM_CHECK_HIP(hipGetLastError());
  return 0;
}

#include "conv_igemm_m32.inc"


template <bool RH, typename T>
__global__ __launch_bounds__(768) void conv_igemm_ws64_kernel(const ConvDesc d) {
  constexpr int BCH = 64, BPIX = 256;
  constexpr int E = 8, BK = 64;
  constexpr int XR = BPIX / 32;
  constexpr int WL = BCH / 32;
  constexpr int NP = XR + WL;
  constexpr int FM = 4, FN = 4;
  constexpr int HXROWS = 264;
  constexpr int HWROWS = 3 * BCH;
  constexpr int NST = RH ? 2 : 3;
  constexpr int STAGE = RH ? (HWROWS + HXROWS) * 8 : (BCH + BPIX) * 8;
  constexpr int SROW = 144;
  extern __shared__ __attribute__((aligned(16))) uint4 lds3[];
  const uint4* zrow = lds3 + NST * STAGE;
  unsigned char* stg = reinterpret_cast<unsigned char*>(lds3 + NST * STAGE + (RH ? 8 : 0));
  static_assert(NP == 10, "the counted waits below assume 10 pieces per tile");

  const int tid = threadIdx.x;
  const int lane = tid & 63;
  const int wave = __builtin_amdgcn_readfirstlane(tid >> 6);
  const int NCC = d.Cin >> 6;
  const int KT = RH ? 3 * NCC : d.KT;
  if (RH && tid < 8) lds3[NST * STAGE + tid] = make_uint4(0u, 0u, 0u, 0u);
  float* lbias = reinterpret_cast<float*>(stg + BPIX * SROW);
  const bool bias_lds = d.bias == nullptr || d.bias_stride == 0;
  if (tid < BCH) lbias[tid] = (d.bias && bias_lds && tid < d.Cout) ? d.bias[tid] : 0.f;
  __syncthreads();
  const int n_my = ((int)d.n_tiles - (int)blockIdx.x + (int)gridDim.x - 1) / (int)gridDim.x;
  const int total = n_my * KT;
  auto tile_of = [&](int k) {
    const int v = (int)blockIdx.x + k * (int)gridDim.x;
    const int nblk = d.n_tiles, bq = nblk >> 3, br = nblk & 7, xcd = v & 7, bidx = v >> 3;
    return (xcd < br ? xcd * (bq + 1) : br * (bq + 1) + (xcd - br) * bq) + bidx;
  };

  if (wave >= 8) {
    const int ts = tid - 512;
    const int c = ts & 7;
    const int r0 = ts >> 3;
    T* __restrict__ out = reinterpret_cast<T*>(d.out);
    const int ch = c * 8;
    const int nch = d.Cout - ch;
    const int per = (8 + (KT - 1) - 1) / (KT - 1);
    auto flush = [&](int k, int i0, int i1) {
      if (nch <= 0) return;
      const int pix_tile = tile_of(k);
      for (int i = i0; i < i1 && i < 8; ++i) {
        const int r = r0 + 32 * i;
        const long long m = (long long)pix_tile * BPIX + r;
        if (m >= d.M) continue;
        unsigned n, qd, qh, qw;
        decode_row(d, (unsigned)m, n, qd, qh, qw);
        const long long o = ((((long long)n * d.Do + (qd * d.osd + d.opd)) * d.Ho + (qh * d.osh + d.oph)) * d.Wo + (qw * d.osw + d.opw)) * d.ldo + ch;
        const uint4 v = *reinterpret_cast<const uint4*>(stg + r * SROW + c * 16);
        if (nch >= 8) *reinterpret_cast<uint4*>(out + o) = v;
        else *reinterpret_cast<uint2*>(out + o) = make_uint2(v.x, v.y);
      }
    };
    const int sw = wave - 8;
    const int lr = lane & 15, lg = lane >> 4;
    uint4 A2[2][2];
    float b2[2][4];
    if (d.w2) {
      const unsigned short* w2 = reinterpret_cast<const unsigned short*>(d.w2);
#pragma unroll
      for (int of = 0; of < 2; ++of)
#pragma unroll
        for (int ks = 0; ks < 2; ++ks) {
          A2[of][ks] = make_uint4(0u, 0u, 0u, 0u);
          if (of * 16 < d.cout2) A2[of][ks] = *reinterpret_cast<const uint4*>(w2 + (long long)(of * 16 + lr) * d.kpad2 + ks * 32 + lg * 8);
        }
#pragma unroll
      for (int of = 0; of < 2; ++of)
#pragma unroll
        for (int e = 0; e < 4; ++e) {
          const int c2 = of * 16 + lg * 4 + e;
          b2[of][e] = (d.bias2 && c2 < d.cout2) ? d.bias2[c2] : 0.f;
        }
    }
    const int perf = (4 + (KT - 1) - 1) / (KT - 1);
    auto flush_fused = [&](int k, int j0, int j1) {
      const int pix_tile = tile_of(k);
      T* out2 = reinterpret_cast<T*>(d.out2);
      for (int j = j0; j < j1 && j < 4; ++j) {
        const int r = sw * 64 + j * 16 + lr;
        const long long m = (long long)pix_tile * BPIX + r;
        const uint4 B0 = *reinterpret_cast<const uint4*>(stg + r * SROW + lg * 16);
        const uint4 B1 = *reinterpret_cast<const uint4*>(stg + r * SROW + 64 + lg * 16);
        unsigned n, qd, qh, qw;
        decode_row(d, m < d.M ? (unsigned)m : 0u, n, qd, qh, qw);
        const long long o = ((((long long)n * d.Do + (qd * d.osd + d.opd)) * d.Ho + (qh * d.osh + d.oph)) * d.Wo + (qw * d.osw + d.opw)) * d.ldo2;
#pragma unroll
        for (int of = 0; of < 2; ++of) {
          if (of * 16 >= d.cout2) break;
          f32x4 acc = f32x4{0.f, 0.f, 0.f, 0.f};
          acc = MmaG<T>::run2(A2[of][0], B0, acc);
          acc = MmaG<T>::run2(A2[of][1], B1, acc);
          if (m < d.M) {
            float v[4];
#pragma unroll
            for (int e = 0; e < 4; ++e) v[e] = apply_act_g(acc[e] + b2[of][e], d.act2, d.slope2);
            store4(out2 + o + of * 16 + lg * 4, v);
          }
        }
      }
    };
    int g = 0;
    for (int k = 0; k < n_my; ++k)
      for (int kt = 0; kt < KT; ++kt, ++g) {
        RGBM_BARRIER();
        if (k > 0 && kt < KT - 1) {
          if (d.w2) flush_fused(k - 1, kt * perf, (kt + 1) * perf);
          else flush(k - 1, kt * per, (kt + 1) * per);
        }
      }
    RGBM_BARRIER();
    if (d.w2) flush_fused(n_my - 1, 0, 4);
    else flush(n_my - 1, 0, 8);
    return;
  }

  if (wave >= 4) {
    if constexpr (RH) {
      const T* __restrict__ in = reinterpret_cast<const T*>(d.in);
      const T* __restrict__ wgt = reinterpret_cast<const T*>(d.wgt);
      const int pw = wave - 4;
      const int j = lane & 7, r8 = lane >> 3;
      const int dil = d.dilw;
      constexpr int NXP = HXROWS / 8;
      constexpr int NWP = HWROWS / 8;
      constexpr int MXP = (NXP + 3) / 4, MWP = NWP / 4;
      const char* xrowp[MXP];
      unsigned xmask[MXP];
      const char* wrowp[MWP];
      const char* zero = reinterpret_cast<const char*>(g_zero_page);
      const unsigned ldsb = __builtin_amdgcn_readfirstlane(lds_addr(lds3));
#pragma unroll
      for (int i = 0; i < MWP; ++i) {
        const int wr = (pw + 4 * i) * 8 + r8;
        const int kw = wr >> 6, ch = wr & 63;
        wrowp[i] = reinterpret_cast<const char*>(wgt + (long long)ch * d.Kpad + (long long)kw * d.Cin + (j ^ ((wr >> 1) & 7)) * E);
      }
      auto enter_tile = [&](int k) {
        const long long p0 = (long long)tile_of(k) * BPIX;
#pragma unroll
        for (int i = 0; i < MXP; ++i) {
          const int xr = (pw + 4 * i) * 8 + r8;
          const long long m = p0 - dil + xr;
          unsigned mk = 0;
          long long pix0 = 0;
          if ((pw + 4 * i) < NXP && xr < BPIX + 2 * dil && m >= 0 && m < d.M) {
            unsigned n, qd, qh, qw;
            decode_row(d, (unsigned)m, n, qd, qh, qw);
            for (int kh = 0; kh < 3; ++kh) mk |= (unsigned)((unsigned)((int)qh + (kh - 1) * dil) < (unsigned)d.Hi) << kh;
            pix0 = ((long long)n * d.Hi + ((int)qh - dil)) * d.Wi + (int)qw;
          }
          xmask[i] = mk;
          xrowp[i] = reinterpret_cast<const char*>(in) + (pix0 * d.Cin + (j ^ ((xr >> 1) & 7)) * E) * 2ll;
        }
      };
      int ikh = 0, icc = 0, itile = 0;
      auto issue = [&](int stage) {
        if (ikh == 0 && icc == 0) enter_tile(itile);
        const unsigned sbase = ldsb + (unsigned)stage * (STAGE * 16);
        const long long xoff = ((long long)ikh * dil * d.Wi * d.Cin + icc * 64) * 2ll;
        const long long woff = ((long long)ikh * 3 * d.Cin + icc * 64) * 2ll;
#pragma unroll
        for (int i = 0; i < MXP; ++i) {
          if (pw + 4 * i < NXP) {
            const char* src = ((xmask[i] >> ikh) & 1u) ? xrowp[i] + xoff : zero;
            glds16(src, sbase + (HWROWS * 8 + (pw + 4 * i) * 64) * 16);
          }
        }
#pragma unroll
        for (int i = 0; i < MWP; ++i) glds16(wrowp[i] + woff, sbase + ((pw + 4 * i) * 64) * 16);
        if (++icc == NCC) { icc = 0; if (++ikh == 3) { ikh = 0; ++itile; } }
      };
      if (total > 0) issue(0);
      for (int g = 0; g < total; ++g) {
        asm volatile("s_waitcnt vmcnt(0)" ::: "memory");
        RGBM_BARRIER();
        if (g + 1 < total) issue((g + 1) & 1);
      }
      RGBM_BARRIER();
      return;
    }
    const T* __restrict__ in = reinterpret_cast<const T*>(d.in);
    const T* __restrict__ wgt = reinterpret_cast<const T*>(d.wgt);
    const int pw = wave - 4;
    const int tp = tid - 256;
    const int j = tp & 7;
    const int r0 = tp >> 3;
    const int js = j ^ ((r0 >> 1) & 7);
    const char* rowp[XR];
    unsigned rmask[XR];
    const char* wrow[WL];
    const char* zero = reinterpret_cast<const char*>(g_zero_page);
    int tkd = 0, tkh = 0, tkw = 0, tc = 0;
    const unsigned lds0 = __builtin_amdgcn_readfirstlane(lds_addr(lds3 + pw * 64));

    long long mybase = 0;
    unsigned mymask = 0;
    auto prepare_tile = [&](int k) {
      const int pix_tile = tile_of(k);
      mybase = 0;
      mymask = 0;
      if (j < XR) {
        const long long m = (long long)pix_tile * BPIX + r0 + 32 * j;
        int xn = 0, xd0 = -(1 << 20), xh0 = 0, xw0 = 0;
        if (m < d.M) {
          unsigned n, qd, qh, qw;
          decode_row(d, (unsigned)m, n, qd, qh, qw);
          xn = (int)n * d.Di;
          xd0 = (int)qd * d.sd - d.pd;
          xh0 = (int)qh * d.sh - d.ph;
          xw0 = (int)qw * d.sw - d.pw;
        }
        for (int kk = 0; kk < d.KD; ++kk) mymask |= (unsigned)((unsigned)(xd0 + kk * d.dild) < (unsigned)d.Di) << kk;
        for (int kk = 0; kk < d.KH; ++kk) mymask |= (unsigned)((unsigned)(xh0 + kk * d.dilh) < (unsigned)d.Hi) << (8 + kk);
        for (int kk = 0; kk < d.KW; ++kk) mymask |= (unsigned)((unsigned)(xw0 + kk * d.dilw) < (unsigned)d.Wi) << (16 + kk);
        const long long pix0 = ((long long)(xn + xd0) * d.Hi + xh0) * d.Wi + xw0;
        mybase = pix0 * d.Cin * (long long)sizeof(T);
      }
    };
    auto enter_tile = [&]() {
      const int grp = (tp & 63) & 56;
#pragma unroll
      for (int i = 0; i < XR; ++i) {
        const long long bb = __shfl(mybase, grp | i, 64);
        rmask[i] = (unsigned)__shfl((int)mymask, grp | i, 64);
        rowp[i] = reinterpret_cast<const char*>(in) + bb + (long long)(js * E) * (long long)sizeof(T);
      }
      tkd = tkh = tkw = tc = 0;
    };
#pragma unroll
    for (int i = 0; i < WL; ++i)
      wrow[i] = reinterpret_cast<const char*>(wgt + (long long)(r0 + 32 * i) * d.Kpad + js * E);

    int ikt = 0, itile = 0;
    auto issue = [&](int stage) {
      if (ikt == 0) enter_tile();
      const unsigned sbase = lds0 + (unsigned)stage * (STAGE * 16);
      const unsigned sel = (1u << tkd) | (256u << tkh) | (65536u << tkw);
      const long long soff =
          ((long long)((tkd * d.dild * d.Hi + tkh * d.dilh) * d.Wi + tkw * d.dilw) * d.Cin + tc) * (long long)sizeof(T);
      const bool cok = tkd < d.KD && tc + js * E < d.Cin;
#pragma unroll
      for (int i = 0; i < XR; ++i) {
        const bool ok = cok && (rmask[i] & sel) == sel;
        const char* src = ok ? rowp[i] + soff : zero;
        glds16(src, sbase + (BCH * 8 + i * 256) * 16);
      }
      const long long wk = (long long)ikt * BK * (long long)sizeof(T);
#pragma unroll
      for (int i = 0; i < WL; ++i) glds16(wrow[i] + wk, sbase + (i * 256) * 16);
      tc += BK;
      if (d.lcin >= 0 && tc >= d.Cin) {
        tc = 0;
        if (++tkw == d.KW) { tkw = 0; if (++tkh == d.KH) { tkh = 0; ++tkd; } }
      }
      if (++ikt == KT) { ikt = 0; ++itile; if (itile < n_my) prepare_tile(itile); }
    };

    if (total > 0) prepare_tile(0);
    if (total > 0) issue(0);
    if (total > 1) issue(1);
    int st = 0;
    for (int g = 0; g < total; ++g) {
      if (g + 1 < total) asm volatile("s_waitcnt vmcnt(10)" ::: "memory");
      else asm volatile("s_waitcnt vmcnt(0)" ::: "memory");
      RGBM_BARRIER();
      if (g + 2 < total) issue(st == 0 ? 2 : st - 1);
      st = st == 2 ? 0 : st + 1;
    }
    RGBM_BARRIER();
    return;
  }

  const int wpix = wave * 64;
  const int lr = lane & 15, lg = lane >> 4;
  uint4 af0[FM], bf0[FN], af1[FM], bf1[FN];
  f32x4 acc[FM][FN];
  auto load_half = [&](int st, int s, uint4 (&af)[FM], uint4 (&bf)[FN]) {
    const uint4* W = lds3 + st * STAGE;
    const uint4* X = W + BCH * 8;
    const int cidx = s * 4 + lg;
#pragma unroll
    for (int a = 0; a < FM; ++a) {
      const int row = a * 16 + lr;
      af[a] = W[row * 8 + (cidx ^ ((row >> 1) & 7))];
    }
#pragma unroll
    for (int b = 0; b < FN; ++b) {
      const int row = wpix + b * 16 + lr;
      bf[b] = X[row * 8 + (cidx ^ ((row >> 1) & 7))];
    }
  };
  auto mma_half = [&](const uint4 (&af)[FM], const uint4 (&bf)[FN]) {
#pragma unroll
    for (int a = 0; a < FM; ++a)
#pragma unroll
      for (int b = 0; b < FN; ++b) MmaG<T>::run(af[a], bf[b], acc[a][b]);
  };
  int st = 0;
  for (int k = 0; k < n_my; ++k) {
#pragma unroll
    for (int a = 0; a < FM; ++a) {
      const f32x4 b4 = *reinterpret_cast<const f32x4*>(lbias + a * 16 + lg * 4);
#pragma unroll
      for (int b = 0; b < FN; ++b) acc[a][b] = b4;
    }
    if constexpr (RH) {
      const int dil = d.dilw;
      const long long p0 = (long long)tile_of(k) * BPIX;
      bool eL[FN], eR[FN];
#pragma unroll
      for (int b = 0; b < FN; ++b) {
        const long long m = p0 + wpix + b * 16 + lr;
        unsigned n, qd, qh, qw;
        decode_row(d, m < d.M ? (unsigned)m : 0u, n, qd, qh, qw);
        eL[b] = (int)qw - dil < 0;
        eR[b] = (int)qw + dil >= d.Wi;
      }
      for (int kt = 0; kt < KT; ++kt) {
        asm volatile("s_waitcnt lgkmcnt(0)" ::: "memory");
        RGBM_BARRIER();
        const uint4* W = lds3 + (st & 1) * STAGE;
        const uint4* X = W + HWROWS * 8;
#pragma unroll
        for (int kw = 0; kw < 3; ++kw) {
#pragma unroll
          for (int s2 = 0; s2 < 2; ++s2) {
            const int cidx = s2 * 4 + lg;
            uint4 af[FM], bf[FN];
#pragma unroll
            for (int a = 0; a < FM; ++a) {
              const int row = kw * 64 + a * 16 + lr;
              af[a] = W[row * 8 + (cidx ^ ((row >> 1) & 7))];
            }
#pragma unroll
            for (int b = 0; b < FN; ++b) {
              const int row = wpix + b * 16 + lr + kw * dil;
              const bool edge = kw == 0 ? eL[b] : (kw == 2 ? eR[b] : false);
              const uint4* src = edge ? zrow + cidx : X + row * 8 + (cidx ^ ((row >> 1) & 7));
              bf[b] = *src;
            }
#pragma unroll
            for (int a = 0; a < FM; ++a)
#pragma unroll
              for (int b = 0; b < FN; ++b) MmaG<T>::run(af[a], bf[b], acc[a][b]);
          }
        }
        ++st;
      }
    } else {
    for (int kt = 0; kt < KT; ++kt) {
      asm volatile("s_waitcnt lgkmcnt(0)" ::: "memory");
      RGBM_BARRIER();
      load_half(st, 0, af0, bf0);
      __builtin_amdgcn_sched_barrier(0);
      if (kt > 0) mma_half(af1, bf1);
      __builtin_amdgcn_sched_barrier(0);
      load_half(st, 1, af1, bf1);
      __builtin_amdgcn_sched_barrier(0);
      mma_half(af0, bf0);
      __builtin_amdgcn_sched_barrier(0);
      st = st == 2 ? 0 : st + 1;
    }
    mma_half(af1, bf1);
    }
    if (bias_lds && d.act != ACT_TANH) {
      const float slope = d.slope;
      auto pack_tile = [&](auto actc) {
        constexpr int ACT = decltype(actc)::value;
#pragma unroll
        for (int b = 0; b < FN; ++b) {
          const int row = wpix + b * 16 + lr;
#pragma unroll
          for (int a = 0; a < FM; ++a) {
            float v[4];
#pragma unroll
            for (int e = 0; e < 4; ++e) {
              const float x = acc[a][b][e];
              v[e] = ACT == ACT_RELU ? (x < 0.f ? 0.f : x) : ACT == ACT_PRELU ? (x < 0.f ? x * slope : x) : x;
            }
            store4(reinterpret_cast<T*>(stg + row * SROW + (a * 16 + lg * 4) * 2), v);
          }
        }
      };
      if (d.act == ACT_RELU) pack_tile(IC<ACT_RELU>{});
      else if (d.act == ACT_PRELU) pack_tile(IC<ACT_PRELU>{});
      else pack_tile(IC<ACT_NONE>{});
      continue;
    }
    const int pix_tile = tile_of(k);
#pragma unroll
    for (int b = 0; b < FN; ++b) {
      const int row = wpix + b * 16 + lr;
      int n = 0;
      if (d.bias && d.bias_stride != 0) {
        const long long m = (long long)pix_tile * BPIX + row;
        unsigned nn, qd, qh, qw;
        decode_row(d, m < d.M ? (unsigned)m : 0u, nn, qd, qh, qw);
        n = (int)nn;
      }
#pragma unroll
      for (int a = 0; a < FM; ++a) {
        const int ch = a * 16 + lg * 4;
        float v[4] = {acc[a][b][0], acc[a][b][1], acc[a][b][2], acc[a][b][3]};
        if (d.bias && !bias_lds && ch < d.Cout) {
          const float* bp = d.bias + (long long)n * d.bias_stride + ch;
#pragma unroll
          for (int e = 0; e < 4; ++e) v[e] += bp[e];
        }
#pragma unroll
        for (int e = 0; e < 4; ++e) v[e] = apply_act_g(v[e], d.act, d.slope);
        store4(reinterpret_cast<T*>(stg + row * SROW + ch * 2), v);
      }
    }
  }
  asm volatile("s_waitcnt lgkmcnt(0)" ::: "memory");
  RGBM_BARRIER();
}

template <typename T>
static int launch_ws64(ConvDesc d, bool rh, hipStream_t s) {
  constexpr int BCH = 64, BPIX = 256;
  const size_t LDS = (rh ? 2 * (size_t)(3 * BCH + 264) * 8 * sizeof(uint4) + 128 + (size_t)BPIX * 144
                         : 3 * (size_t)(BCH + BPIX) * 8 * sizeof(uint4) + (size_t)BPIX * 144) + BCH * sizeof(float);
  d.n_pix_tiles = (int)((d.M + BPIX - 1) / BPIX);
  d.n_ch_tiles = 1;
  d.n_tiles = d.n_pix_tiles;
  make_fastdiv(d.Wq, d.fd_m[0], d.fd_s[0]);
  make_fastdiv(d.Hq, d.fd_m[1], d.fd_s[1]);
  make_fastdiv(d.Dq, d.fd_m[2], d.fd_s[2]);
  if (int rc = ensure_dynamic_lds(reinterpret_cast<const void*>(conv_igemm_ws64_kernel<false, T>), 160 * 1024)) return rc;
  if (int rc = ensure_dynamic_lds(reinterpret_cast<const void*>(conv_igemm_ws64_kernel<true, T>), 160 * 1024)) return rc;
  int n_cu = 0;
  if (int rc = persistent_grid_cus(&n_cu)) return rc;
  const int grid = d.n_tiles < n_cu ? d.n_tiles : n_cu;
  prof_begin_launch(s, 15, d.algo_flops, d.algo_bytes);
  if (rh) hipLaunchKernelGGL((conv_igemm_ws64_kernel<true, T>), dim3((unsigned)grid), dim3(768), LDS, s, d);
  else hipLaunchKernelGGL((conv_igemm_ws64_kernel<false, T>), dim3((unsigned)grid), dim3(768), LDS, s, d);
  prof_end_launch(s);
  RGBM_CHECK_HIP(hipGetLastError());
  return 0;
}

template <typename T, bool UNI>
static int launch_v3(ConvDesc d, hipStream_t s) {
  constexpr int BCH = 128, BPIX = 256;
  constexpr size_t LDS = 3 * (BCH + BPIX) * 8 * sizeof(uint4);
  d.n_pix_tiles = (int)((d.M + BPIX - 1) / BPIX);
  d.n_ch_tiles = (d.Cout + BCH - 1) / BCH;
  const long long nblk = (long long)d.n_pix_tiles * d.n_ch_tiles;
  RGBM_REQUIRE(nblk > 0 && nblk < (1ll << 31), "conv grid out of range");
  if (int rc = ensure_dynamic_lds(reinterpret_cast<const void*>(conv_igemm_v3_kernel<T, UNI>), (int)LDS)) return rc;
  prof_begin_launch(s, prof_row_ws<T>(), d.algo_flops, d.algo_bytes);
  hipLaunchKernelGGL((conv_igemm_v3_kernel<T, UNI>), dim3((unsigned)nblk), dim3(512), LDS, s, d);
  prof_end_launch(s);
  RGBM_CHECK_HIP(hipGetLastError());
  return 0;
}

template <typename T, int BCH, int BPIX, bool UNI>
static int launch_one_g(ConvDesc d, hipStream_t s) {
  d.n_pix_tiles = (int)((d.M + BPIX - 1) / BPIX);
  d.n_ch_tiles = (d.Cout + BCH - 1) / BCH;
  const long long nblk = (long long)d.n_pix_tiles * d.n_ch_tiles;
  RGBM_REQUIRE(nblk > 0 && nblk < (1ll << 31), "conv grid out of range");
  prof_begin_launch(s, prof_row_generic<T>(BCH), d.algo_flops, d.algo_bytes);
  hipLaunchKernelGGL((conv_igemm_glds_kernel<T, BCH, BPIX, UNI>), dim3((unsigned)nblk), dim3(256), 0, s, d);
  prof_end_launch(s);
  RGBM_CHECK_HIP(hipGetLastError());
  return 0;
}

int conv_tuning(int n_cu, ConvTuning* t) {
  *t = ConvTuning{g_debug_flags, g_gemm_kernel, g_ws_min_rows, n_cu};
  return n_cu > 0 ? 0 : persistent_grid_cus(&t->n_cu);
}

template <typename T>
static int launch_plan(const ConvDesc& d, const ConvPlan& p, hipStream_t s) {
  constexpr bool M32 = sizeof(T) == 2 || std::is_same<T, bx3_t>::value;
  switch (p.kernel) {
    case CONV_GENERIC: {
      auto tile = [&](auto uni) {
        constexpr bool UNI = decltype(uni)::value;
        switch (p.bch) {
          case 16: return launch_one_g<T, 16, 256, UNI>(d, s);
          case 32: return launch_one_g<T, 32, 256, UNI>(d, s);
          case 64: return launch_one_g<T, 64, 256, UNI>(d, s);
          default: return launch_one_g<T, 128, 128, UNI>(d, s);
        }
      };
      return p.uniform_taps ? tile(IC<true>{}) : tile(IC<false>{});
    }
    case CONV_M32_SMALL:
      if constexpr (M32) return launch_m32_small<T>(d, p, s);
      break;
    case CONV_WS_SLIM: return launch_ws<T, false, false, true>(d, p, s);
    case CONV_M32:
      if constexpr (M32) return launch_m32<T>(d, p, s);
      break;
    case CONV_WS_WIDE: return launch_ws<T, true, false>(d, p, s);
    case CONV_WS: return launch_ws<T, false, false>(d, p, s);
    case CONV_V3: return p.uniform_taps ? launch_v3<T, true>(d, s) : launch_v3<T, false>(d, s);
    case CONV_WS64:
    case CONV_WS64_ROWHALO:
      if constexpr (sizeof(T) == 2) return launch_ws64<T>(d, p.kernel == CONV_WS64_ROWHALO, s);
      break;
  }
  RGBM_REQUIRE(false, "conv plan names a kernel this storage type does not have");
}

int launch_conv(const ConvDesc& d, int dtype, hipStream_t s) {
  ConvTuning t;
  ConvPlan p;
  if (int rc = conv_tuning(0, &t)) return rc;
  if (int rc = plan_conv(d, dtype, t, &p)) return rc;
  return dtype == BF16 ? launch_plan<unsigned short>(d, p, s) : dtype == F16 ? launch_plan<f16_t>(d, p, s)
         : dtype == BF16X3 ? launch_plan<bx3_t>(d, p, s) : launch_plan<float>(d, p, s);
}

bool conv_ws64_eligible(const ConvDesc& d, int dtype) {
  ConvTuning t;
  ConvPlan p;
  return !conv_tuning(0, &t) && !plan_conv(d, dtype, t, &p) && (p.kernel == CONV_WS64 || p.kernel == CONV_WS64_ROWHALO);
}

}
```

rgbmanip_amd/csrc/conv_plan.cpp:

```cpp
#include "conv_plan.h"

#include "kernels.h"

namespace rgbm {

#ifndef M32_KSPLIT_MAX
#define M32_KSPLIT_MAX 4
#endif
#ifndef M32_KSPLIT_MINSTEPS
#define M32_KSPLIT_MINSTEPS 8
#endif

namespace {

bool uniform_taps(const ConvDesc& d, int bk) {
  if (d.KD > 8 || d.KH > 8 || d.KW > 8) return false;
  if (d.lcin < 0) return d.ntaps == 1;
  return d.Cin % bk == 0;
}

bool buffer_offsets_ok(const ConvDesc& d, int bch, long long esz) {
  const long long xbytes = ((long long)d.N * d.Di * d.Hi * d.Wi + (long long)(d.pd * d.Hi + d.ph) * d.Wi + d.pw) * d.Cin * esz;
  const long long wbytes = (long long)((d.Cout + bch - 1) / bch) * bch * d.Kpad * esz;
  return xbytes < (1ll << 32) - 65536 && wbytes < (1ll << 32) - 65536 && d.pd >= 0 && d.ph >= 0 && d.pw >= 0;
}

bool rowhalo_ok(const ConvDesc& d) {
  return d.KD == 1 && d.KH == 3 && d.KW == 3 && d.sd == 1 && d.sh == 1 && d.sw == 1 && d.Dq == 1 && d.Di == 1 &&
         d.dilh == d.dilw && d.dilw >= 1 && d.dilw <= 4 && d.ph == d.dilh && d.pw == d.dilw && d.pd == 0 &&
         d.lcin >= 6 && d.Hq == d.Hi && d.Wq == d.Wi && d.Wi > 2 * d.dilw && d.osh == 1 && d.osw == 1;
}

int m32_small_choice(const ConvDesc& d, int n_cu, bool slim_ok) {
  const long long p128 = (d.M + 127) / 128, p256 = (d.M + 255) / 256;
  auto cost = [&](long long tiles, int kb) { return (double)((tiles + n_cu - 1) / n_cu) * (double)(kb + 8); };
  double best = slim_ok ? cost(p256 * (d.Cout / 64), 40) : 1e30;
  int pick = 0;
  const int bch[3] = {64, 128, 256}, kb[3] = {24, 32, 48};
  for (int i = 0; i < 3; ++i) {
    if (d.Cout % bch[i]) continue;
    const double c = cost(p128 * (d.Cout / bch[i]), kb[i]);
    if (c < best * 0.999) { best = c; pick = bch[i]; }
  }
  return pick;
}

int m32_ksplit_choice(const ConvDesc& d, int flags, long long tiles, int n_cu, int bch, int n_waves) {
  if ((flags & DBG_NO_KSPLIT) || tiles <= 0 || bch > 128) return 1;
  int n = (int)(n_cu / tiles);
  if (n > M32_KSPLIT_MAX) n = M32_KSPLIT_MAX;
  while (n > 1 && d.KT / n < M32_KSPLIT_MINSTEPS) --n;
  if (n < 2) return 1;
  if ((size_t)tiles * n * bch * 128 > kM32SplitFloats || (size_t)tiles * n_waves > kM32SplitCounters) return 1;
  return n;
}

}

int plan_conv(const ConvDesc& d, int dtype, const ConvTuning& t, ConvPlan* out) {
  RGBM_REQUIRE(d.M > 0 && d.M < (1ll << 31), "conv M out of range");
  RGBM_REQUIRE(d.Cout % 4 == 0 && d.ldo % 4 == 0, "conv Cout/ldo must be multiples of 4");
  RGBM_REQUIRE(d.KT > 0 && d.Kpad == d.KT * conv_bk(dtype), "conv K padding mismatch");
  RGBM_REQUIRE(d.Cin % dtype_chunk(dtype) == 0, "conv Cin must be a multiple of the 16-byte chunk");
  if (d.lcin >= 0) {
    RGBM_REQUIRE((1 << d.lcin) == d.Cin, "conv lcin mismatch");
  } else {
    RGBM_REQUIRE(d.ntaps == 1, "linear-K mode needs a single tap");
  }
  const int f = t.flags, n_cu = t.n_cu;
  const long long esz = (long long)dtype_size(dtype);
  const bool bits16 = esz == 2, mfma32 = dtype != F32;
  const int ch_tile = conv_ch_tile(d.Cout);
  const bool uni = uniform_taps(d, conv_bk(dtype)) && !(f & DBG_NONUNIFORM_TAPS);
  const bool out16 = (((unsigned long long)d.out | (unsigned long long)(d.ldo * esz)) & 15ull) == 0ull;
  const bool rows16 = out16 && ((unsigned long long)d.res & 15ull) == 0ull;
  const bool dense_out = d.osd == 1 && d.osh == 1 && d.osw == 1 && d.opd == 0 && d.oph == 0 && d.opw == 0 && d.Dq == d.Do && d.Hq == d.Ho && d.Wq == d.Wo;
  const bool ident_ok = dense_out && d.res_mode == RES_PRE_ACT && d.res != nullptr && d.M * d.ldo * esz < (1ll << 32) - 65536;
  const bool ws_rows = d.M >= (t.ws_min_rows > 0 ? t.ws_min_rows : 1024);

  ConvPlan p = {};
  p.uniform_taps = uni;
  p.ksplit = 1;
  p.korder = (f & DBG_KORDER_TAPS_OUTER) ? 0 : 1;
  auto pick = [&](int kernel, int bch, int bpix) {
    p.kernel = kernel; p.bch = bch; p.bpix = bpix;
    p.buf_ok = buffer_offsets_ok(d, bch, esz) && !(f & DBG_GLOBAL_ADDR);
    *out = p;
    return 0;
  };
  auto generic = [&]() { return pick(CONV_GENERIC, ch_tile, ch_tile == 128 ? 128 : 256); };
  auto small = [&](int bch) {
    p.ksplit = m32_ksplit_choice(d, f, ((d.M + 127) / 128) * ((d.Cout + bch - 1) / bch), n_cu, bch, 4);
    p.identity_residual = ident_ok && d.Cout % 256 == 0;
    return pick(CONV_M32_SMALL, bch, 128);
  };

  if (d.out_f32) {
    RGBM_REQUIRE(dtype == BF16X3 && d.w2 == nullptr, "out_f32 is a bf16x3 option of the generic kernel");
    return generic();
  }
  if (ch_tile == 128 && !(f & DBG_NO_WS) && ws_rows) {
    if (!uni || (f & DBG_V3_FOR_WS) || !rows16) return pick(CONV_V3, 128, 256);
    if (!(f & DBG_NO_SLIM_SMALL) && d.Cout % 64 == 0) {
      const long long slim_tiles = ((d.M + 255) / 256) * (d.Cout / 64);
      if (mfma32) {
        if (d.Cout % 256 == 0 && ((d.M + 255) / 256) * (d.Cout / 256) < n_cu && t.gemm_kernel >= 1 && !(f & (DBG_M32_TAILS_R5 | DBG_WS_128x256)) &&
            buffer_offsets_ok(d, 256, esz)) {
          const int bch = t.gemm_kernel == 1 ? 256 : m32_small_choice(d, n_cu, slim_tiles <= n_cu);
          if (bch) return small(bch);
        }
        if (d.Cout == 128 && ((d.M + 127) / 128) * 2 * 2 <= n_cu && t.gemm_kernel == 2 &&
            !(f & (DBG_M32_TAILS_R5 | DBG_WS_128x256 | DBG_NO_KSPLIT | DBG_L2_SLIM_TILE)) && d.w2 == nullptr && buffer_offsets_ok(d, 64, esz))
          return small(64);
      }
      if (slim_tiles <= n_cu) return pick(CONV_WS_SLIM, 64, 256);
    }
    if (d.Cout % 256 == 0 && !(f & DBG_WS_128x256)) {
      if (!(mfma32 && buffer_offsets_ok(d, 256, esz) && t.gemm_kernel >= 1)) return pick(CONV_WS_WIDE, 256, 128);
      const bool big_ok = dense_out && (d.bias == nullptr || (d.bias_stride == 0 && d.Cout <= 2560)) && d.act != ACT_TANH &&
                          (d.res_mode == RES_NONE || (d.res_mode == RES_PRE_ACT && d.res != nullptr)) && d.M * d.ldo * esz < (1ll << 32) - 65536;
      const long long P = d.M / 256, n_ch = d.Cout / 256, tiles = P * n_ch;
      long long Pm = 0;
      if (t.gemm_kernel != 1 && big_ok && tiles >= n_cu) {
        const long long rem = tiles % n_cu;
        Pm = (rem == 0 || rem * 10 >= (long long)n_cu * 6) ? P : (tiles - rem) / n_ch;
      }
      p.main_rows = Pm * 256;
      p.identity_residual = ident_ok;
      p.tail_bch = p.main_rows == d.M ? 0 : 256;
      const long long pt = (d.M - p.main_rows + 127) / 128;
      if (p.tail_bch && t.gemm_kernel != 1 && !(f & DBG_M32_TAILS_R5)) {
        if (pt * (d.Cout / 64) <= n_cu) p.tail_bch = 64;
        else if (pt * (d.Cout / 128) <= n_cu) p.tail_bch = 128;
      }
      return pick(CONV_M32, 256, 256);
    }
    return pick(CONV_WS, 128, 256);
  }
  if (bits16 && uni && !(f & DBG_NO_WS64) && ch_tile == 64 && d.res_mode == RES_NONE && d.KT >= 2 && ws_rows &&
      (d.w2 ? d.Cout == 64 && d.kpad2 == 64 && (d.cout2 == 16 || d.cout2 == 32) && d.ldo2 % 4 == 0 : out16))
    return rowhalo_ok(d) && !(f & DBG_NO_ROWHALO) ? pick(CONV_WS64_ROWHALO, 64, 256) : pick(CONV_WS64, 64, 256);
  RGBM_REQUIRE(d.w2 == nullptr, "a fused 1x1 needs the ws64 kernel (check conv_ws64_eligible first)");
  if (ch_tile == 64 && uni && ws_rows && !(f & (DBG_NO_WS | DBG_V3_FOR_WS | DBG_NO_SLIM64)) && rows16) return pick(CONV_WS_SLIM, 64, 256);
  return generic();
}

}
```

rgbmanip_amd/csrc/kernels.h:

```cpp
#pragma once
#include <vector>

#include "common.h"

namespace rgbm {

int launch_nchw_to_nhwc_pad(int dtype, const float* in, void* out, int V, int C, int H, int W, int Cp, hipStream_t s);
int launch_maxpool3x3s2(int dtype, const void* in, void* out, int V, int H, int W, int C, hipStream_t s);
int launch_resize_bilinear_ac(int dtype, const void* in, void* out, int V, int Hs, int Ws, int C, int Ho, int Wo, int ldo,
                              int ch_off, hipStream_t s);
int launch_copy_channels(int dtype, const void* in, void* out, long long npix, int C, int ldo, int ch_off, hipStream_t s);
int launch_adaptive_avgpool(int dtype, const void* in, void* out, int V, int H, int W, int C, int S, hipStream_t s);
int launch_adaptive_avgpool_multi(int dtype, const void* in, void* const* outs, const int* bins, int nb, int V, int H, int W, int C,
                                  hipStream_t s);
int launch_psp_pool_conv(int dtype, const void* in, int ldi, const void* const* w, void* const* outs, const int* bins, int V, int H, int W,
                         int act, float slope, hipStream_t s);
int launch_psp_resize_cat(int dtype, const void* f, const void* const* stages, const int* bins, void* out, int V, int Ho, int Wo, hipStream_t s);
int launch_homography(const float* P_views, float* out, int V, int B, hipStream_t s);
int launch_build_volume(int dtype, const void* feat, const float* homog, const float* depths, void* vol, int v0, int Vc, int V,
                        int B, int D, int H, int W, hipStream_t s);

int launch_upconv_combine(int dtype, const void* z, const float* bias, void* out, int V, int h, int w, int Co, int ldo, int act,
                          float slope, hipStream_t s, const float* drop = nullptr);
int launch_upconv_final(int dtype, const void* x, const void* wz, const float* bias, float slope, const void* wf, const float* biasf,
                        void* out, int out_f32, int V, int h, int w, hipStream_t s, const void* wf_f16 = nullptr);

constexpr int kDropoutPerView = 256 + 64;
unsigned dropout_threshold(float p);
float dropout_scale(float p);
int launch_dropout_masks(float* masks, unsigned long long* state, int B, float p, unsigned long long seed, int advance, hipStream_t s);

size_t bn_scratch_bytes(int V);
int launch_bn_per_sample(int dtype, void* y, const void* res, const float* gamma, const float* beta, void* scratch, int V,
                         long long nvox, int C, int relu, hipStream_t s);

int launch_to_f32(int dtype, const void* in, float* out, long long n, hipStream_t s);

int launch_gather_points(int dtype, const void* feat, const int* choose, float* out, int V, int P, int HW, int C, hipStream_t s);
int launch_prob_softmax_depth(int dtype, const void* u11, const float* wprob, const int* choose, const float* depths,
                              float* prob, float* depth_out, int v0, int Vc, int B, int P, int D, int H, int W, int classmajor,
                              hipStream_t s);
int launch_dense_depth(int dtype, const void* u11, const float* wprob, const float* depths, float* depth_map, float* conf_map,
                       int v0, int Vc, int B, int D, int H, int W, int classmajor, hipStream_t s);
int launch_depth_to_points(const float* depth, const double* Kc, const double* E, int n, int S, float* points, hipStream_t s);
int launch_depth_consistency(const float* depth_a, const float* conf_a, const unsigned char* mask_a, const double* Ka, const double* Ea,
                             const float* depth_b, const double* Kb, const double* Eb, int n, int S, double px_max, double rel_max,
                             float conf_min, float* fused, float* reproj, float* rel, unsigned char* keep, hipStream_t s);
int launch_cloud_pack(const float* fused1, const unsigned char* keep1, const double* K1, const double* E1, const float* fused2,
                      const unsigned char* keep2, const double* K2, const double* E2, int n, int S, int cap, float* cloud, int* index,
                      int* count, hipStream_t s);
int launch_depth_fusion(const float* depth, const float* conf, const unsigned char* mask, const double* Kc, const double* E, int n, int V,
                        int S, double px_max, double rel_max, float conf_min, int n_min, float* fused, unsigned char* keep,
                        unsigned char* nviews, unsigned short* agree, hipStream_t s);
int launch_cloud_pack_views(const float* fused, const unsigned char* keep, const double* Kc, const double* E, int n, int V, int S, int cap,
                            float* cloud, int* index, int* count, hipStream_t s);
int launch_cloud_gather_views(const float* maps, const int* index, int n, int V, int S2, int C, int cap, float* out, hipStream_t s);
int launch_fuse_points(int dtype, const void* feat, const float* homog, const float* depths, const int* choose,
                       const float* prob, float* out, int V, int B, int P, int D, int H, int W, int ldo, int ch_off,
                       hipStream_t s, int Vn = -1);
int launch_mean_points(int dtype, const void* in, float* out, float* scratch, int V, int P, int C, hipStream_t s);
int launch_f32_to_f16(const float* in, void* out, long long n, hipStream_t s);
void stem_pack(const float* w, std::vector<float>& packed);
int launch_stem(int dtype, const float* img1, const float* img2, const void* wpk, void* out, int B, int V, int S, hipStream_t s);
int launch_stem_views(int dtype, const float* img, const void* wpk, void* out, int V, int S, hipStream_t s);
int launch_feature_store(const void* src, void* pool, const int* slots, int V, int pool_records, size_t part_off, size_t part_bytes,
                         size_t record_bytes, hipStream_t s);
int launch_feature_gather(const void* pool, void* dst, const int* slot1, const int* slot2, int B, int pool_records, size_t part_off,
                          size_t part_bytes, size_t record_bytes, hipStream_t s);
int launch_feature_bad_slot_nan(const int* slot1, const int* slot2, int B, int pool_records, float* const out[10], const int per_pose[10],
                                hipStream_t s);
int launch_crop_fingerprint(const float* img, int V, int n_words, unsigned long long* keys_out, hipStream_t s);
int launch_f32_to_bx3(const float* in, void* out, long long n, hipStream_t s);
int launch_view_linear(const float* x, const float* W, const float* bias, float* out, int V, int I, int O, int ldw, int i0,
                       int relu, hipStream_t s);
struct PointMlpDesc {
  const float* table;
  const void* feat;
  const int* choose;
  float* nocs4;
  float* pf;
  int ldpf, P, HW;
  long long N;
};
int point_mlp_table_floats();
void point_mlp_pack(const float* const w[6], const float* const b[6], float* table);
int launch_point_mlp(int feat_dtype, const PointMlpDesc& d, hipStream_t s);
int launch_dense_nocs(int feat_dtype, const float* table, const void* feat, float* out, long long N, hipStream_t s);
int launch_ortho6d(const float* r6, float* R, int V, hipStream_t s);
int launch_mean_points_partial(int dtype, const void* in, float* scratch, int V, int P, int C, hipStream_t s);
int launch_view_linear_mean(const float* partial, int P, float* mean_out, const float* W, const float* bias, float* out, int V, int I, int O,
                            int ldw, int i0, int relu, hipStream_t s);
int launch_pose_heads_mean(const float* partial, int P, float* mean_out, float* R, float* const w[3][3], float* const b[3][3],
                           float* const out[3], const int odim[3], int V, hipStream_t s);
constexpr int kMeanSplit = 8;
constexpr int kPoseMlpSlab = 128;
struct PoseMlpDesc {
  const float* pf96;
  const void* w[4];
  int ldw[4];
  const float* bias[4];
  const float* vbias;
  void* q128;
  float* part128;
  float* part256;
  int V, P;
};
bool pose_mlp_fits(int P);
int launch_pose_mlp1(const PoseMlpDesc& d, hipStream_t s);
int launch_pose_mlp2(const PoseMlpDesc& d, hipStream_t s);
int launch_pose_heads(const float* pf2, float* const w[3][3], float* const b[3][3], float* const out[3], const int odim[3], int V,
                      hipStream_t s);
int launch_stage_in(const float* P1, const float* P2, const int* c1, const int* c2, float* Pviews, int* choose, int B, int P, hipStream_t s);
int launch_stage_out(const float* nocs4, const float* depth, const float* R, const float* tv, const float* sv, float* const nocs[2],
                     float* const dep[2], float* const r[2], float* const t[2], float* const sz[2], int B, int P, int view2, hipStream_t s);
int launch_copy_cols(const float* in, float* out, long long rows, int ldi, int ldo, int n, hipStream_t s);

struct Conv3dTileDesc {
  const void* in; const void* wgt; void* out; const float* bias; const void* res;
  int N, Di, Hi, Wi;
  int Do, Ho, Wo;
  int Dq, Hq, Wq;
  int ntd, nth, ntw;
  int Cout, relu;
  const void* feat; const float* homog; const float* depths; int v0, V, B;
  int prof_variant; double algo_flops, algo_bytes;
  int out_classmajor;
  int feat_f16;
  const int* tile_list; const int* tile_count;
  int tile_mask_stride;
  const unsigned char* tile_mask;
};
enum DebugFlag {
  DBG_NO_WS = 8, DBG_NONUNIFORM_TAPS = 16, DBG_V3_FOR_WS = 64, DBG_NO_WS64 = 128, DBG_NO_ROWHALO = 256, DBG_GENERIC_RESIZE = 512,
  DBG_PSP_STAGE_R5 = 1024, DBG_POINT_MLP_R5 = 2048, DBG_TILE_CONV0 = 4096, DBG_NO_KSPLIT = 16384, DBG_L2_SLIM_TILE = 32768,
  DBG_WS_128x256 = 65536, DBG_NO_SLIM64 = 262144, DBG_KORDER_TAPS_OUTER = 1 << 20, DBG_SWEEP_ALT_BLEND = 1 << 21, DBG_SWEEP_DOT2 = 1 << 22,
  DBG_PP_ONE_KERNEL = 1 << 23, DBG_NO_SLIM_SMALL = 1 << 24, DBG_PP_GENERIC_SELECT = 1 << 25, DBG_PP_GUARD = 1 << 26, DBG_GLOBAL_ADDR = 1 << 27,
  DBG_SWEEP_PER_TILE = 1 << 28, DBG_SPARSE_TAIL_R5 = 1 << 29, DBG_M32_TAILS_R5 = 1 << 30, DBG_POSE_MLP_R6 = 1 << 19,
};
extern int g_debug_flags;
extern long long g_ws_min_rows;
extern int g_tuning_version;
extern int g_gemm_kernel;
void conv3d_tile_pack(const float* w, const float* scale, int Cin, int Cout, int coutp, bool transposed, int dtype,
                      std::vector<float>& packed);
int launch_conv3d_tile(int layer, int dtype, const Conv3dTileDesc& d, hipStream_t s);
int sparse_mask_bytes_per_view(int S);
int sparse_mask_offset(int S, int layer);
int launch_sparse_masks(const int* choose, int v0, int Vc, int P, int S, unsigned char* masks, int* sweep_list, int* sweep_count,
                        hipStream_t s);
int conv3d_tile_dims(int layer, int dtype, int* TD, int* TH, int* TW);

void conv0_sweep_pack(const float* w, const float* scale, std::vector<float>& packed);
int launch_conv0_sweep(const Conv3dTileDesc& d, int dtype, hipStream_t s);

int conv0_sweep_x3_upload(const std::vector<float>& packed, void** dev);
int launch_conv0_sweep_x3(const Conv3dTileDesc& d, hipStream_t s);
int launch_bx3_to_f32(const void* in, float* out, long long n, hipStream_t s);

int launch_prob_sparse(const void* u9, const void* c0, const void* w11_packed, const float* bias11, const float* wprob,
                       const int* choose, const float* depths, float* prob, float* depth_out, int v0, int Vc, int B, int P,
                       int D, int H, int W, int dtype, hipStream_t s, const void* w11_taps = nullptr);
void prob_sparse_pack(const float* w, const float* scale, std::vector<float>& packed);

int launch_prepare_inputs(const float* rgb, const unsigned char* mask, const double* K, const int* frame_map, int N, int H, int W, int S, int P,
                          unsigned seed, float* img, int* choose, float* pts2d, double* Kcrop, int* window, int* valid,
                          unsigned char* small_scratch, hipStream_t s, int frame0 = 0);
int launch_prepare_inputs_u8(const unsigned char* rgb, const unsigned char* mask, const double* K, const int* frame_map, int N, int H, int W,
                             int S, int P, unsigned seed, float* img, int* choose, float* pts2d, double* Kcrop, int* window, int* valid,
                             unsigned char* small_scratch, hipStream_t s, int frame0 = 0);
int launch_prepare_inputs_opt(const void* rgb, int pixel_type, int normalize, const unsigned char* mask, const double* K, const int* frame_map,
                              int N, int H, int W, int S, int P, unsigned seed, float* img, int* choose, float* pts2d, double* Kcrop,
                              int* window, int* valid, unsigned char* small_scratch, hipStream_t s, int frame0 = 0);
int launch_prepare_inputs_windows(const void* pix, int pixel_type, int normalize, const unsigned char* mask_pix, const long long* offset,
                                  const int* window, const int* valid_in, const double* K, int frame0, int N, int H, int W, int S, int P,
                                  unsigned seed, float* img, int* choose, float* pts2d, double* Kcrop, int* valid, unsigned char* small_scratch,
                                  hipStream_t s);
int launch_quantize_frames(const float* src, unsigned char* dst, size_t n, hipStream_t s);

int launch_umeyama_ransac(const float* nocs, const float* depth, const int* choose, const double* Kc, const double* E1,
                          double* bbox, double* srt, int* valid, int B, int P, int img, unsigned seed, hipStream_t s);

int launch_cloud_gather(const float* map1, const float* map2, const int* index, int n, int S2, int C, int cap, float* out, hipStream_t s);
size_t cloud_similarity_scratch_bytes(int n, int cap);
int launch_cloud_similarity(const float* nocs, const float* cloud, const int* count, int n, int cap, unsigned seed, double* bbox, double* srt,
                            int* info, int* valid, void* scratch, size_t scratch_bytes, hipStream_t s);

int launch_projection(const double* Kc, const double* E, float* P, int n, hipStream_t s);
int launch_pnp_ransac(const float* nocs1, const float* pts1, const float* nocs2, const float* pts2, const double* K, const double* E1,
                      const double* E2, double* bbox, double* srt, int* info, int* valid, int B, int P, unsigned seed, hipStream_t s);

int launch_mask_extent(const unsigned char* mask, int N, int H, int W, int* ext, int* count, hipStream_t s);

int launch_postprocess(const float* nocs, const float* depth, const float* rot, const int* choose, const double* Kc,
                       const double* E1, double* bbox, double* ts_out, int* valid, int B, int P, int img, hipStream_t s,
                       void* scratch = nullptr, size_t scratch_bytes = 0);
int launch_postprocess_regressed(const float* nocs, const float* rot, const float* tr, const float* sv, const double* E1, double* bbox,
                                 double* ts_out, int* valid, int B, int P, hipStream_t s);
int launch_microbench_mfma(float* scratch, int iters, int random_operands, double* flops, hipStream_t s);
int microbench_mfma_scratch_floats(int* n);
int launch_microbench_copy(const void* src, void* dst, size_t bytes, hipStream_t s);
size_t postprocess_scratch_bytes(int B);
int postprocess_slices(int B);

int launch_gae(int T, int N, const float* rewards, const unsigned char* dones, const float* values, const float* last_values,
               float gamma, float lam, float* returns, float* adv, double* sums, hipStream_t s);
int launch_adv_normalise(long long n_local, float* adv, const double* sums, double count_total, hipStream_t s);

struct PolicyLayout { int dims[5]; int log_std; int w[2][4]; int b[2][4]; int total; };
struct PolicyOptState { int t; int n_updates; float lr; float last_kl; float last_norm; float pad_; double sum_surr; double sum_vloss; };
int launch_policy_forward(const float* params, const PolicyLayout& L, int n, int mode, const float* obs, const float* noise,
                          float* actions, float* logp, float* value, float* mu, hipStream_t s);
int policy_partial_floats(const PolicyLayout& L, int n);
int launch_ppo_minibatch(const float* params, const PolicyLayout& L, int n, const float* obs, const float* actions,
                         const float* old_logp, const float* adv, const float* returns, const float* old_values,
                         const float* old_mu, const float* old_sigma, float clip, float vcoef, float ecoef, float* partial,
                         float* grads, hipStream_t s);
constexpr int POLICY_MAX_HIDDEN = 6, POLICY_MAX_WIDTH = 512, POLICY_MAX_ACT = 32;
enum { PACT_ELU = 0, PACT_SELU = 1, PACT_RELU = 2, PACT_LRELU = 3, PACT_TANH = 4, PACT_SIGMOID = 5 };
struct PolicyDesc {
  int obs_dim, state_dim, act_dim, activation, asymmetric;
  int n_hidden[2];
  int hidden[2][POLICY_MAX_HIDDEN];
  int w[2][POLICY_MAX_HIDDEN + 1];
  int b[2][POLICY_MAX_HIDDEN + 1];
  int log_std, total;
};
int launch_policy_forward_ex(const float* params, const PolicyDesc& D, int n, int mode, const float* obs, const float* states,
                             const float* noise, float* actions, float* logp, float* value, float* mu, hipStream_t s);
int ppo_scratch_floats_ex(const PolicyDesc& D, int n, int clipped_vloss, size_t* count);
int launch_ppo_minibatch_ex(const float* params, const PolicyDesc& D, int n, const float* obs, const float* states,
                            const float* actions, const float* old_logp, const float* adv, const float* returns,
                            const float* old_values, const float* old_mu, const float* old_sigma, float clip, float vcoef, float ecoef,
                            int clipped_vloss, float* scratch, float* grads, hipStream_t s);
int launch_ppo_adam(float* params, const float* grads, float* m, float* v, PolicyOptState* st, int total, float inv_world,
                    float max_norm, float desired_kl, float lr_min, float lr_max, int adaptive, hipStream_t s);

}
```

rgbmanip_amd/csrc/misc_kernels.hip:

```cpp
#include "common.h"
#include "kernels.h"

namespace rgbm {

static inline unsigned grid_for(long long n, int block = 256) {
  long long g = (n + block - 1) / block;
  const long long cap = 256ll * 32;
  return (unsigned)(g < cap ? (g > 0 ? g : 1) : cap);
}

template <typename T>
__global__ void nchw_to_nhwc_pad_kernel(const float* __restrict__ in, T* __restrict__ out, int V, int C, int H, int W,
                                        int Cp) {
  const long long total = (long long)V * H * W;
  for (long long i = blockIdx.x * (long long)blockDim.x + threadIdx.x; i < total; i += (long long)gridDim.x * blockDim.x) {
    const long long v = i / ((long long)H * W);
    const long long hw = i - v * H * W;
    for (int c0 = 0; c0 < Cp; c0 += 4) {
      float vals[4];
#pragma unroll
      for (int e = 0; e < 4; ++e) {
        const int c = c0 + e;
        vals[e] = c < C ? in[(v * C + c) * H * W + hw] : 0.f;
      }
// ... 119 lines not shown
__device__ __forceinline__ void st_nt(T* p, const uint4& v) {
  typedef unsigned u4 __attribute__((ext_vector_type(4)));
  __builtin_nontemporal_store(u4{v.x, v.y, v.z, v.w}, reinterpret_cast<u4*>(p));
}

template <typename T>
__global__ __launch_bounds__(256) void resize2x_ac_kernel(const T* __restrict__ in, T* __restrict__ out, int V, int Hs, int Ws, int C,
                                                            int ldo, int ch_off, float sy, float sx) {
  constexpr int E = 16 / sizeof(T);
  const int cpp = C / E, Ho = 2 * Hs, Wo = 2 * Ws;
  const int Hp = (Hs + 1) >> 1, Wp = (Ws + 1) >> 1;
  const long long total = (long long)V * Hp * Wp * cpp;
  const long long nchunk = (total + 255) / 256, per_xcd = (nchunk + 7) / 8;
  for (long long q = blockIdx.x; q < per_xcd * 8; q += gridDim.x) {
    const long long chunk = (q & 7) * per_xcd + (q >> 3);
    const long long idx = chunk * 256 + threadIdx.x;
    if (chunk >= nchunk || idx >= total) continue;
    const unsigned u = (unsigned)idx;
    const unsigned pp = u / (unsigned)cpp;
    const int cc = (int)(u - pp * (unsigned)cpp);
    const unsigned row = pp / (unsigned)Wp;
    const int j = 2 * (int)(pp - row * (unsigned)Wp);
    const unsigned vv = row / (unsigned)Hp;
    const int i = 2 * (int)(row - vv * (unsigned)Hp);
    const long long v = vv;
    const T* base = in + v * Hs * Ws * C + cc * E;
    T* obase = out + (v * Ho * Wo) * ldo + ch_off + cc * E;
    const int nrow = i + 1 < Hs ? 4 : 2, ncol = j + 1 < Ws ? 4 : 2;
    Lerp ly[4], lx[4];
#pragma unroll
    for (int k = 0; k < 4; ++k) {
      ly[k] = lerp_ac(min(2 * i + k, Ho - 1), Hs, sy);
      lx[k] = lerp_ac(min(2 * j + k, Wo - 1), Ws, sx);
    }
    bool fast = nrow == 4 && ncol == 4;
#pragma unroll
    for (int k = 0; k < 4; ++k)
      fast = fast && ly[k].i0 == i - 1 + ((k + 1) >> 1) && ly[k].i1 == i + ((k + 1) >> 1) &&
             lx[k].i0 == j - 1 + ((k + 1) >> 1) && lx[k].i1 == j + ((k + 1) >> 1);
    if (fast) {
      uint4 p[4][4];
#pragma unroll
      for (int a = 0; a < 4; ++a)
#pragma unroll
        for (int b = 0; b < 4; ++b)
          p[a][b] = *reinterpret_cast<const uint4*>(base + ((long long)(i - 1 + a) * Ws + (j - 1 + b)) * C);
#pragma unroll
      for (int m = 0; m < 4; ++m) {
        const int r0 = (m + 1) >> 1;
#pragma unroll
        for (int k = 0; k < 4; ++k) {
          const int c0 = (k + 1) >> 1;
          float ta[E], tb[E], tc[E], td[E], r[E];
          unpack_chunk(p[r0][c0], ta, T());
          unpack_chunk(p[r0][c0 + 1], tb, T());
          unpack_chunk(p[r0 + 1][c0], tc, T());
          unpack_chunk(p[r0 + 1][c0 + 1], td, T());
#pragma unroll
          for (int e = 0; e < E; ++e) r[e] = bilerp(ta[e], tb[e], tc[e], td[e], lx[k], ly[m]);
          st_nt(obase + ((long long)(2 * i + m) * Wo + 2 * j + k) * ldo, pack_chunk(r, T()));
        }
      }
    } else {
      for (int m = 0; m < nrow; ++m) {
        const Lerp lym = lerp_ac(2 * i + m, Hs, sy);
        for (int k = 0; k < ncol; ++k) {
          const Lerp lxk = lerp_ac(2 * j + k, Ws, sx);
          float a[E], b[E], c[E], dd[E], r[E];
          unpack_chunk(*reinterpret_cast<const uint4*>(base + ((long long)lym.i0 * Ws + lxk.i0) * C), a, T());
          unpack_chunk(*reinterpret_cast<const uint4*>(base + ((long long)lym.i0 * Ws + lxk.i1) * C), b, T());
          unpack_chunk(*reinterpret_cast<const uint4*>(base + ((long long)lym.i1 * Ws + lxk.i0) * C), c, T());
          unpack_chunk(*reinterpret_cast<const uint4*>(base + ((long long)lym.i1 * Ws + lxk.i1) * C), dd, T());
#pragma unroll
          for (int e = 0; e < E; ++e) r[e] = bilerp(a[e], b[e], c[e], dd[e], lxk, lym);
          st_nt(obase + ((long long)(2 * i + m) * Wo + 2 * j + k) * ldo, pack_chunk(r, T()));
        }
      }
    }
  }
}

int launch_resize_bilinear_ac(int dtype, const void* in, void* out, int V, int Hs, int Ws, int C, int Ho, int Wo, int ldo,
                              int ch_off, hipStream_t s) {
  const int E = dtype_chunk(dtype);
  RGBM_REQUIRE(C % E == 0 && ldo % E == 0 && ch_off % E == 0, "resize channel alignment");
  const float sy = Ho > 1 ? (float)(Hs - 1) / (float)(Ho - 1) : 0.f;
  const float sx = Wo > 1 ? (float)(Ws - 1) / (float)(Wo - 1) : 0.f;
  if (Ho == 2 * Hs && Wo == 2 * Ws && Hs >= 2 && Ws >= 2 && (long long)V * Hs * Ws * (C / E) < (1ll << 31) && !(g_debug_flags & DBG_GENERIC_RESIZE)) {
    const long long blocks = (long long)V * ((Hs + 1) / 2) * ((Ws + 1) / 2) * (C / E);
    if (dtype == BF16)
      hipLaunchKernelGGL(resize2x_ac_kernel<unsigned short>, dim3(grid_for(blocks)), dim3(256), 0, s, (const unsigned short*)in,
                         (unsigned short*)out, V, Hs, Ws, C, ldo, ch_off, sy, sx);
    else if (dtype == F16)
      hipLaunchKernelGGL(resize2x_ac_kernel<f16_t>, dim3(grid_for(blocks)), dim3(256), 0, s, (const f16_t*)in,
                         (f16_t*)out, V, Hs, Ws, C, ldo, ch_off, sy, sx);
    else if (dtype == BF16X3)
      hipLaunchKernelGGL(resize2x_ac_kernel<bx3_t>, dim3(grid_for(blocks)), dim3(256), 0, s, (const bx3_t*)in,
                         (bx3_t*)out, V, Hs, Ws, C, ldo, ch_off, sy, sx);
    else
      hipLaunchKernelGGL(resize2x_ac_kernel<float>, dim3(grid_for(blocks)), dim3(256), 0, s, (const float*)in, (float*)out, V, Hs,
                         Ws, C, ldo, ch_off, sy, sx);
    RGBM_CHECK_HIP(hipGetLastError());
    return 0;
  }
  const long long total = (long long)V * Ho * Wo * (C / E);
  if (dtype == BF16)
    hipLaunchKernelGGL(resize_bilinear_ac_kernel<unsigned short>, dim3(grid_for(total)), dim3(256), 0, s,
                       (const unsigned short*)in, (unsigned short*)out, V, Hs, Ws, C, Ho, Wo, ldo, ch_off, sy, sx);
  else if (dtype == F16)
    hipLaunchKernelGGL(resize_bilinear_ac_kernel<f16_t>, dim3(grid_for(total)), dim3(256), 0, s,
                       (const f16_t*)in, (f16_t*)out, V, Hs, Ws, C, Ho, Wo, ldo, ch_off, sy, sx);
  else if (dtype == BF16X3)
    hipLaunchKernelGGL(resize_bilinear_ac_kernel<bx3_t>, dim3(grid_for(total)), dim3(256), 0, s,
                       (const bx3_t*)in, (bx3_t*)out, V, Hs, Ws, C, Ho, Wo, ldo, ch_off, sy, sx);
  else
    hipLaunchKernelGGL(resize_bilinear_ac_kernel<float>, dim3(grid_for(total)), dim3(256), 0, s, (const float*)in,
                       (float*)out, V, Hs, Ws, C, Ho, Wo, ldo, ch_off, sy, sx);
  RGBM_CHECK_HIP(hipGetLastError());
  return 0;
}

template <typename T>
__global__ void copy_channels_kernel(const T* __restrict__ in, T* __restrict__ out, long long npix, int C, int ldo, int ch_off) {
  constexpr int E = 16 / sizeof(T);
  const int cpp = C / E;
  const long long total = npix * cpp;
  for (long long i = blockIdx.x * (long long)blockDim.x + threadIdx.x; i < total; i += (long long)gridDim.x * blockDim.x) {
    const int cc = (int)(i % cpp);
    const long long p = i / cpp;
    *reinterpret_cast<uint4*>(out + p * ldo + ch_off + cc * E) = *reinterpret_cast<const uint4*>(in + p * C + cc * E);
  }
}

int launch_copy_channels(int dtype, const void* in, void* out, long long npix, int C, int ldo, int ch_off, hipStream_t s) {
  const int E = dtype_chunk(dtype);
  RGBM_REQUIRE(C % E == 0 && ldo % E == 0 && ch_off % E == 0, "copy channel alignment");
  const long long total = npix * (C / E);
  if (dtype == BF16)
    hipLaunchKernelGGL(copy_channels_kernel<unsigned short>, dim3(grid_for(total)), dim3(256), 0, s,
                       (const unsigned short*)in, (unsigned short*)out, npix, C, ldo, ch_off);
  else if (dtype == F16)
    hipLaunchKernelGGL(copy_channels_kernel<f16_t>, dim3(grid_for(total)), dim3(256), 0, s,
                       (const f16_t*)in, (f16_t*)out, npix, C, ldo, ch_off);
  else if (dtype == BF16X3)
    hipLaunchKernelGGL(copy_channels_kernel<bx3_t>, dim3(grid_for(total)), dim3(256), 0, s,
                       (const bx3_t*)in, (bx3_t*)out, npix, C, ldo, ch_off);
  else
    hipLaunchKernelGGL(copy_channels_kernel<float>, dim3(grid_for(total)), dim3(256), 0, s, (const float*)in, (float*)out,
                       npix, C, ldo, ch_off);
  RGBM_CHECK_HIP(hipGetLastError());
  return 0;
}

struct PoolBins { void* out[4]; int S[4]; int first[5]; int n; };

template <typename T>
__global__ __launch_bounds__(512) void adaptive_avgpool_kernel(const T* __restrict__ in, const PoolBins pb, int V, int H, int W, int C) {
  constexpr int E = 16 / sizeof(T);
  constexpr int PL = 8;
  __shared__ float red[PL][64][E];
  const int ncell = pb.first[pb.n];
  const int cell_all = blockIdx.x % ncell;
  const long long v = blockIdx.x / ncell;
  int g = 0;
#pragma unroll
  for (int i = 1; i < 4; ++i) if (i < pb.n && cell_all >= pb.first[i]) g = i;
  const int S = pb.S[g], cell = cell_all - pb.first[g];
  const int sy = cell / S, sx = cell % S;
  const int h0 = (sy * H) / S, h1 = ((sy + 1) * H + S - 1) / S;
  const int w0 = (sx * W) / S, w1 = ((sx + 1) * W + S - 1) / S;
  const int ww = w1 - w0, npx = (h1 - h0) * ww;
  const float inv = 1.0f / (float)npx;
  const int cl = threadIdx.x & 63, pl = threadIdx.x >> 6;
  T* __restrict__ out = reinterpret_cast<T*>(pb.out[g]);
  for (int c0 = 0; c0 < C / E; c0 += 64) {
    const int cc = c0 + cl;
    float acc[E];
#pragma unroll
    for (int e = 0; e < E; ++e) acc[e] = 0.f;
    if (cc < C / E)
#pragma unroll 4
      for (int p = pl; p < npx; p += PL) {
        const int h = h0 + p / ww, w = w0 + p % ww;
        float x[E];
        unpack_chunk(*reinterpret_cast<const uint4*>(in + ((v * H + h) * W + w) * C + cc * E), x, T());
#pragma unroll
        for (int e = 0; e < E; ++e) acc[e] += x[e];
      }
#pragma unroll
    for (int e = 0; e < E; ++e) red[pl][cl][e] = acc[e];
    __syncthreads();
    if (pl == 0 && cc < C / E) {
#pragma unroll
      for (int e = 0; e < E; ++e) {
        float t = red[0][cl][e];
#pragma unroll
        for (int q = 1; q < PL; ++q) t += red[q][cl][e];
        acc[e] = t * inv;
      }
      *reinterpret_cast<uint4*>(out + ((long long)v * S * S + cell) * C + cc * E) = pack_chunk(acc, T());
    }
    __syncthreads();
  }
}

int launch_adaptive_avgpool_multi(int dtype, const void* in, void* const* outs, const int* bins, int nb, int V, int H, int W, int C,
                                  hipStream_t s) {
  const int E = dtype_chunk(dtype);
  RGBM_REQUIRE(C % E == 0 && nb >= 1 && nb <= 4, "avgpool channel alignment / bin count");
  PoolBins pb;
  pb.n = nb;
  pb.first[0] = 0;
  for (int i = 0; i < 4; ++i) {
    pb.out[i] = i < nb ? outs[i] : nullptr;
    pb.S[i] = i < nb ? bins[i] : 1;
    pb.first[i + 1] = pb.first[i] + (i < nb ? bins[i] * bins[i] : 0);
  }
  pb.first[nb] = pb.first[nb];
  const long long blocks = (long long)V * pb.first[nb];
  RGBM_REQUIRE(blocks > 0 && blocks < (1ll << 31), "avgpool grid");
  if (dtype == BF16)
    hipLaunchKernelGGL(adaptive_avgpool_kernel<unsigned short>, dim3((unsigned)blocks), dim3(512), 0, s, (const unsigned short*)in, pb, V, H, W, C);
  else if (dtype == F16)
    hipLaunchKernelGGL(adaptive_avgpool_kernel<f16_t>, dim3((unsigned)blocks), dim3(512), 0, s, (const f16_t*)in, pb, V, H, W, C);
  else if (dtype == BF16X3)
    hipLaunchKernelGGL(adaptive_avgpool_kernel<bx3_t>, dim3((unsigned)blocks), dim3(512), 0, s, (const bx3_t*)in, pb, V, H, W, C);
  else
    hipLaunchKernelGGL(adaptive_avgpool_kernel<float>, dim3((unsigned)blocks), dim3(512), 0, s, (const float*)in, pb, V, H, W, C);
  RGBM_CHECK_HIP(hipGetLastError());
  return 0;
}

int launch_adaptive_avgpool(int dtype, const void* in, void* out, int V, int H, int W, int C, int S, hipStream_t s) {
  void* outs[1] = {out};
  return launch_adaptive_avgpool_multi(dtype, in, outs, &S, 1, V, H, W, C, s);
}

struct PspStage { const void* in[4]; const void* w[4]; void* out[4]; int S[4]; int first[5]; float sy[4], sx[4]; };

template <typename T>
__global__ __launch_bounds__(512) void psp_pool_conv_kernel(const T* __restrict__ in, const PspStage ps, int V, int H, int W, int ldi, int act,
                                                              float slope) {
  constexpr int E = 16 / sizeof(T);
  constexpr int C = 512, CO = 128, NCH = C / E;
  constexpr int PL = 8;
  __shared__ float red[PL][64][E];
  __shared__ uint4 pooled[NCH];
  __shared__ float res[CO];
  const int ncell = ps.first[4];
  const int cell_all = blockIdx.x % ncell;
  const long long v = blockIdx.x / ncell;
  int g = 0;
#pragma unroll
  for (int i = 1; i < 4; ++i) if (cell_all >= ps.first[i]) g = i;
  const int S = ps.S[g], cell = cell_all - ps.first[g];
  const int sy = cell / S, sx = cell % S;
  const int h0 = (sy * H) / S, h1 = ((sy + 1) * H + S - 1) / S;
  const int w0 = (sx * W) / S, w1 = ((sx + 1) * W + S - 1) / S;
  const int ww = w1 - w0, npx = (h1 - h0) * ww;
  const float inv = 1.0f / (float)npx;
  const int cl = threadIdx.x & 63, pl = threadIdx.x >> 6;
  for (int c0 = 0; c0 < NCH; c0 += 64) {
    const int cc = c0 + cl;
    float acc[E];
#pragma unroll
    for (int e = 0; e < E; ++e) acc[e] = 0.f;
#pragma unroll 8
    for (int p = pl; p < npx; p += PL) {
      const int h = h0 + p / ww, w = w0 + p % ww;
      float x[E];
      unpack_chunk(*reinterpret_cast<const uint4*>(in + ((v * H + h) * W + w) * ldi + cc * E), x, T());
#pragma unroll
      for (int e = 0; e < E; ++e) acc[e] += x[e];
    }
#pragma unroll
    for (int e = 0; e < E; ++e) red[pl][cl][e] = acc[e];
    __syncthreads();
    if (pl == 0) {
#pragma unroll
      for (int e = 0; e < E; ++e) {
        float t = red[0][cl][e];
#pragma unroll
        for (int q = 1; q < PL; ++q) t += red[q][cl][e];
        acc[e] = t * inv;
      }
      pooled[cc] = pack_chunk(acc, T());
    }
    __syncthreads();
  }
  const T* __restrict__ wg = reinterpret_cast<const T*>(ps.w[g]);
  float x[NCH / 64][E];
#pragma unroll
  for (int q = 0; q < NCH / 64; ++q) unpack_chunk(pooled[q * 64 + cl], x[q], T());
  float part[16];
#pragma unroll
  for (int o = 0; o < 16; ++o) {
    float sum = 0.f;
#pragma unroll
    for (int q = 0; q < NCH / 64; ++q) {
      float wv[E];
      unpack_chunk(*reinterpret_cast<const uint4*>(wg + (long long)(pl * 16 + o) * C + (q * 64 + cl) * E), wv, T());
#pragma unroll
      for (int e = 0; e < E; ++e) sum = fmaf(wv[e], x[q][e], sum);
    }
    part[o] = sum;
  }
#pragma unroll
  for (int m = 32; m >= 1; m >>= 1)
#pragma unroll
    for (int o = 0; o < 16; ++o) part[o] += __shfl_xor(part[o], m, 64);
  if (cl == 0) {
#pragma unroll
    for (int o = 0; o < 16; ++o) {
      const float r = part[o];
      res[pl * 16 + o] = act == ACT_RELU ? (r < 0.f ? 0.f : r) : act == ACT_PRELU ? (r < 0.f ? r * slope : r) : r;
    }
  }
  __syncthreads();
  if (threadIdx.x < CO / E) {
    float r[E];
#pragma unroll
    for (int e = 0; e < E; ++e) r[e] = res[threadIdx.x * E + e];
    T* __restrict__ out = reinterpret_cast<T*>(ps.out[g]);
    *reinterpret_cast<uint4*>(out + ((long long)v * S * S + cell) * CO + threadIdx.x * E) = pack_chunk(r, T());
  }
}

template <typename T>
__global__ __launch_bounds__(256) void psp_resize_cat_kernel(const T* __restrict__ f, const PspStage ps, T* __restrict__ out, int V, int Ho, int Wo) {
  constexpr int E = 16 / sizeof(T);
  constexpr int CF = 512, CO = 128, CPS = CO / E, CPF = CF / E, CPP = CPF + 4 * CPS;
  const long long total = (long long)V * Ho * Wo * CPP;
  for (long long i = blockIdx.x * (long long)blockDim.x + threadIdx.x; i < total; i += (long long)gridDim.x * blockDim.x) {
    const int cp = (int)(i % CPP);
    long long t = i / CPP;
    if (cp < CPF) {
      reinterpret_cast<uint4*>(out)[i] = *reinterpret_cast<const uint4*>(f + t * CF + cp * E);
      continue;
    }
    const int cq = cp - CPF;
    const int wo = (int)(t % Wo); t /= Wo;
    const int ho = (int)(t % Ho); t /= Ho;
    const long long v = t;
    const int g = cq / CPS, cc = cq - g * CPS;
    const int S = ps.S[g];
    const Lerp ly = lerp_ac(ho, S, ps.sy[g]), lx = lerp_ac(wo, S, ps.sx[g]);
    const T* base = reinterpret_cast<const T*>(ps.in[g]) + v * S * S * CO + cc * E;
    float a[E], b[E], c[E], dd[E], r[E];
    unpack_chunk(*reinterpret_cast<const uint4*>(base + ((long long)ly.i0 * S + lx.i0) * CO), a, T());
    unpack_chunk(*reinterpret_cast<const uint4*>(base + ((long long)ly.i0 * S + lx.i1) * CO), b, T());
    unpack_chunk(*reinterpret_cast<const uint4*>(base + ((long long)ly.i1 * S + lx.i0) * CO), c, T());
    unpack_chunk(*reinterpret_cast<const uint4*>(base + ((long long)ly.i1 * S + lx.i1) * CO), dd, T());
#pragma unroll
    for (int e = 0; e < E; ++e) r[e] = bilerp(a[e], b[e], c[e], dd[e], lx, ly);
    reinterpret_cast<uint4*>(out)[i] = pack_chunk(r, T());
  }
}

static int psp_stage_desc(const int* bins, PspStage& ps) {
  ps.first[0] = 0;
  for (int i = 0; i < 4; ++i) {
    RGBM_REQUIRE(bins[i] >= 1, "psp bin size");
    ps.S[i] = bins[i];
    ps.first[i + 1] = ps.first[i] + bins[i] * bins[i];
  }
  return 0;
}

int launch_psp_pool_conv(int dtype, const void* in, int ldi, const void* const* w, void* const* outs, const int* bins, int V, int H, int W,
                         int act, float slope, hipStream_t s) {
  const int E = dtype_chunk(dtype);
  RGBM_REQUIRE(ldi % E == 0 && ldi >= 512 && V > 0, "psp stage arguments");
  PspStage ps{};
  if (int rc = psp_stage_desc(bins, ps)) return rc;
  for (int i = 0; i < 4; ++i) { ps.w[i] = w[i]; ps.out[i] = outs[i]; }
  const long long blocks = (long long)V * ps.first[4];
  RGBM_REQUIRE(blocks < (1ll << 31), "psp stage grid");
  if (dtype == BF16)
    hipLaunchKernelGGL(psp_pool_conv_kernel<unsigned short>, dim3((unsigned)blocks), dim3(512), 0, s, (const unsigned short*)in, ps, V, H, W, ldi, act, slope);
  else if (dtype == F16)
    hipLaunchKernelGGL(psp_pool_conv_kernel<f16_t>, dim3((unsigned)blocks), dim3(512), 0, s, (const f16_t*)in, ps, V, H, W, ldi, act, slope);
  else if (dtype == BF16X3)
    hipLaunchKernelGGL(psp_pool_conv_kernel<bx3_t>, dim3((unsigned)blocks), dim3(512), 0, s, (const bx3_t*)in, ps, V, H, W, ldi, act, slope);
  else
    hipLaunchKernelGGL(psp_pool_conv_kernel<float>, dim3((unsigned)blocks), dim3(512), 0, s, (const float*)in, ps, V, H, W, ldi, act, slope);
  RGBM_CHECK_HIP(hipGetLastError());
  return 0;
}

int launch_psp_resize_cat(int dtype, const void* f, const void* const* stages, const int* bins, void* out, int V, int Ho, int Wo, hipStream_t s) {
  const int E = dtype_chunk(dtype);
  RGBM_REQUIRE(V > 0 && f && out, "psp resize arguments");
  PspStage ps{};
  if (int rc = psp_stage_desc(bins, ps)) return rc;
  for (int i = 0; i < 4; ++i) {
    ps.in[i] = stages[i];
    ps.sy[i] = Ho > 1 ? (float)(bins[i] - 1) / (float)(Ho - 1) : 0.f;
    ps.sx[i] = Wo > 1 ? (float)(bins[i] - 1) / (float)(Wo - 1) : 0.f;
  }
  const long long total = (long long)V * Ho * Wo * (1024 / E);
  if (dtype == BF16)
    hipLaunchKernelGGL(psp_resize_cat_kernel<unsigned short>, dim3(grid_for(total)), dim3(256), 0, s, (const unsigned short*)f, ps, (unsigned short*)out, V, Ho, Wo);
  else if (dtype == F16)
    hipLaunchKernelGGL(psp_resize_cat_kernel<f16_t>, dim3(grid_for(total)), dim3(256), 0, s, (const f16_t*)f, ps, (f16_t*)out, V, Ho, Wo);
  else if (dtype == BF16X3)
    hipLaunchKernelGGL(psp_resize_cat_kernel<bx3_t>, dim3(grid_for(total)), dim3(256), 0, s, (const bx3_t*)f, ps, (bx3_t*)out, V, Ho, Wo);
  else
    hipLaunchKernelGGL(psp_resize_cat_kernel<float>, dim3(grid_for(total)), dim3(256), 0, s, (const float*)f, ps, (float*)out, V, Ho, Wo);
  RGBM_CHECK_HIP(hipGetLastError());
  return 0;
}

__global__ void homography_kernel(const float* __restrict__ P, float* __restrict__ out, int V, int B) {
  const int v = blockIdx.x * blockDim.x + threadIdx.x;
  if (v >= V) return;
  const int partner = (v + B) % V;
  const float* Pref = P + (long long)v * 16;
  const float* Psrc = P + (long long)partner * 16;
  double a[4][8];
  for (int i = 0; i < 4; ++i)
    for (int jj = 0; jj < 4; ++jj) { a[i][jj] = (double)Pref[i * 4 + jj]; a[i][4 + jj] = i == jj ? 1.0 : 0.0; }
  for (int c = 0; c < 4; ++c) {
    int piv = c; double best = fabs(a[c][c]);
    for (int r = c + 1; r < 4; ++r) if (fabs(a[r][c]) > best) { best = fabs(a[r][c]); piv = r; }
    if (piv != c) for (int k = 0; k < 8; ++k) { double t = a[c][k]; a[c][k] = a[piv][k]; a[piv][k] = t; }
    const double inv = 1.0 / a[c][c];
    for (int k = 0; k < 8; ++k) a[c][k] *= inv;
    for (int r = 0; r < 4; ++r) if (r != c) { const double f = a[r][c]; for (int k = 0; k < 8; ++k) a[r][k] -= f * a[c][k]; }
  }
  float inv32[16];
  for (int i = 0; i < 4; ++i) for (int jj = 0; jj < 4; ++jj) inv32[i * 4 + jj] = (float)a[i][4 + jj];
  float* o = out + (long long)v * 12;
  for (int i = 0; i < 3; ++i)
    for (int jj = 0; jj < 4; ++jj) {
      float acc = 0.f;
      for (int k = 0; k < 4; ++k) acc = fmaf(Psrc[i * 4 + k], inv32[k * 4 + jj], acc);
      if (jj < 3) o[i * 3 + jj] = acc; else o[9 + i] = acc;
    }
}

int launch_homography(const float* P_views, float* out, int V, int B, hipStream_t s) {
  hipLaunchKernelGGL(homography_kernel, dim3((V + 63) / 64), dim3(64), 0, s, P_views, out, V, B);
  RGBM_CHECK_HIP(hipGetLastError());
  return 0;
}

__device__ __forceinline__ void warp_coords(const float* __restrict__ hm, float x, float y, float depth, int H, int W,
                                            float& ix, float& iy) {
  const float rx = hm[0] * x + hm[1] * y + hm[2];
  const float ry = hm[3] * x + hm[4] * y + hm[5];
  const float rz = hm[6] * x + hm[7] * y + hm[8];
  const float px = rx * depth + hm[9], py = ry * depth + hm[10], pz = rz * depth + hm[11];
  const float u = px / pz, vv = py / pz;
  const float gx = u / ((float)(W - 1) / 2.f) - 1.f;
  const float gy = vv / ((float)(H - 1) / 2.f) - 1.f;
  ix = ((gx + 1.f) * (float)W - 1.f) / 2.f;
  iy = ((gy + 1.f) * (float)H - 1.f) / 2.f;
}

struct Bilin { int x0, y0; float w00, w01, w10, w11; bool nan; };
__device__ __forceinline__ Bilin bilin_setup(float ix, float iy) {
  Bilin b;
  b.nan = !(isfinite(ix) && isfinite(iy));
  if (b.nan) { b.x0 = b.y0 = -100; b.w00 = b.w01 = b.w10 = b.w11 = 0.f; return b; }
  ix = fminf(fmaxf(ix, -4.f), 1.0e6f);
  iy = fminf(fmaxf(iy, -4.f), 1.0e6f);
  const float fx = floorf(ix), fy = floorf(iy);
  b.x0 = (int)fx; b.y0 = (int)fy;
  const float tx = ix - fx, ty = iy - fy;
  b.w00 = (1.f - tx) * (1.f - ty);
  b.w01 = tx * (1.f - ty);
  b.w10 = (1.f - tx) * ty;
  b.w11 = tx * ty;
  return b;
}

template <typename T>
__global__ void build_volume_kernel(const T* __restrict__ feat, const float* __restrict__ homog, const float* __restrict__ depths,
                                    T* __restrict__ vol, int v0, int Vc, int V, int B, int D, int H, int W) {
  constexpr int C = 32;
  constexpr int E = 16 / sizeof(T);
  constexpr int NCH = C / E;
  const long long total = (long long)Vc * D * H * W;
  for (long long i = blockIdx.x * (long long)blockDim.x + threadIdx.x; i < total; i += (long long)gridDim.x * blockDim.x) {
    long long t = i;
    const int x = (int)(t % W); t /= W;
    const int y = (int)(t % H); t /= H;
    const int dz = (int)(t % D); t /= D;
    const int v = v0 + (int)t;
    const int partner = (v + B) % V;
    const int b = v % B;
    float ix, iy;
    warp_coords(homog + (long long)v * 12, (float)x, (float)y, depths[b * D + dz], H, W, ix, iy);
    const Bilin bl = bilin_setup(ix, iy);
    const T* ref = feat + (((long long)v * H + y) * W + x) * C;
    const T* src = feat + (long long)partner * H * W * C;
    const bool in00 = (unsigned)bl.x0 < (unsigned)W && (unsigned)bl.y0 < (unsigned)H;
    const bool in01 = (unsigned)(bl.x0 + 1) < (unsigned)W && (unsigned)bl.y0 < (unsigned)H;
    const bool in10 = (unsigned)bl.x0 < (unsigned)W && (unsigned)(bl.y0 + 1) < (unsigned)H;
    const bool in11 = (unsigned)(bl.x0 + 1) < (unsigned)W && (unsigned)(bl.y0 + 1) < (unsigned)H;
    T* o = vol + i * C;
#pragma unroll
    for (int cc = 0; cc < NCH; ++cc) {
      float r[E], acc[E];
      unpack_chunk(*reinterpret_cast<const uint4*>(ref + cc * E), r, T());
#pragma unroll
      for (int e = 0; e < E; ++e) acc[e] = 0.f;
      float s[E];
      if (in00) { unpack_chunk(*reinterpret_cast<const uint4*>(src + ((long long)bl.y0 * W + bl.x0) * C + cc * E), s, T());
#pragma unroll
        for (int e = 0; e < E; ++e) acc[e] += s[e] * bl.w00; }
      if (in01) { unpack_chunk(*reinterpret_cast<const uint4*>(src + ((long long)bl.y0 * W + bl.x0 + 1) * C + cc * E), s, T());
#pragma unroll
        for (int e = 0; e < E; ++e) acc[e] += s[e] * bl.w01; }
      if (in10) { unpack_chunk(*reinterpret_cast<const uint4*>(src + ((long long)(bl.y0 + 1) * W + bl.x0) * C + cc * E), s, T());
#pragma unroll
        for (int e = 0; e < E; ++e) acc[e] += s[e] * bl.w10; }
      if (in11) { unpack_chunk(*reinterpret_cast<const uint4*>(src + ((long long)(bl.y0 + 1) * W + bl.x0 + 1) * C + cc * E), s, T());
#pragma unroll
        for (int e = 0; e < E; ++e) acc[e] += s[e] * bl.w11; }
#pragma unroll
      for (int e = 0; e < E; ++e) acc[e] = bl.nan ? __builtin_nanf("") : (r[e] + acc[e]);
      *reinterpret_cast<uint4*>(o + cc * E) = pack_chunk(acc, T());
    }
  }
}

int launch_build_volume(int dtype, const void* feat, const float* homog, const float* depths, void* vol, int v0, int Vc, int V,
                        int B, int D, int H, int W, hipStream_t s) {
  const long long total = (long long)Vc * D * H * W;
  if (dtype == BF16)
    hipLaunchKernelGGL(build_volume_kernel<unsigned short>, dim3(grid_for(total) * 4), dim3(256), 0, s,
                       (const unsigned short*)feat, homog, depths, (unsigned short*)vol, v0, Vc, V, B, D, H, W);
  else if (dtype == F16)
    hipLaunchKernelGGL(build_volume_kernel<f16_t>, dim3(grid_for(total) * 4), dim3(256), 0, s,
                       (const f16_t*)feat, homog, depths, (f16_t*)vol, v0, Vc, V, B, D, H, W);
  else if (dtype == BF16X3)
    hipLaunchKernelGGL(build_volume_kernel<bx3_t>, dim3(grid_for(total) * 4), dim3(256), 0, s,
                       (const bx3_t*)feat, homog, depths, (bx3_t*)vol, v0, Vc, V, B, D, H, W);
  else
    hipLaunchKernelGGL(build_volume_kernel<float>, dim3(grid_for(total) * 4), dim3(256), 0, s, (const float*)feat, homog,
                       depths, (float*)vol, v0, Vc, V, B, D, H, W);
  RGBM_CHECK_HIP(hipGetLastError());
  return 0;
}

template <typename T>
__global__ void to_f32_kernel(const T* __restrict__ in, float* __restrict__ out, long long n) {
  for (long long i = blockIdx.x * (long long)blockDim.x + threadIdx.x; i < n; i += (long long)gridDim.x * blockDim.x)
    out[i] = Elem<T>::ld(in + i);
}

int launch_to_f32(int dtype, const void* in, float* out, long long n, hipStream_t s) {
  if (dtype == BF16)
    hipLaunchKernelGGL(to_f32_kernel<unsigned short>, dim3(grid_for(n)), dim3(256), 0, s, (const unsigned short*)in, out, n);
  else if (dtype == F16)
    hipLaunchKernelGGL(to_f32_kernel<f16_t>, dim3(grid_for(n)), dim3(256), 0, s, (const f16_t*)in, out, n);
  else if (dtype == BF16X3)
    hipLaunchKernelGGL(to_f32_kernel<bx3_t>, dim3(grid_for(n)), dim3(256), 0, s, (const bx3_t*)in, out, n);
  else
    hipLaunchKernelGGL(to_f32_kernel<float>, dim3(grid_for(n)), dim3(256), 0, s, (const float*)in, out, n);
// ... 50 lines not shown
```

Before: 5841.

## Add row-line avgpool with fused copy, ws64 residual epilogue, split PSP concat copy

Adds a new adaptive average-pool kernel that sums whole pooling lines per block over a strided input, and can write the feature passthrough copy into the concat buffer in the same pass. The PSP resize/concat kernel therefore skips re-copying the 512 feature channels on the large path. Separately, the 64-channel workspace conv kernel gains a pre-activation residual path that prefetches residual rows into the staging LDS and adds them in the epilogue, and the planner now routes such convs to it. These changes bring more code paths and template instantiations, and the residual staging adds LDS traffic and synchronisation inside the conv.

```diff
diff --git a/include/rgbm.h b/include/rgbm.h
--- a/include/rgbm.h
+++ b/include/rgbm.h
@@ -243,6 +243,9 @@
 int rgbm_conv_plan(int dtype, int N, int D, int H, int W, int Cin, int Cin_pad, int Cout, int Cout_pad, int KD, int KH, int KW,
                    int stride_d, int stride_hw, int pad_d, int pad_hw, int dil_hw, int transposed, int has_bias, int res_mode, int act,
                    int cls, int n_cu, int32_t* plan);
+int rgbm_conv_plan_ex(int dtype, int N, int D, int H, int W, int Cin, int Cin_pad, int Cout, int Cout_pad, int KD, int KH, int KW,
+                      int stride_d, int stride_hw, int pad_d, int pad_hw, int dil_hw, int transposed, int has_bias, int res_mode, int act,
+                      int cls, int n_cu, int ldo, int res_offset_bytes, int32_t* plan);
 int rgbm_bn_per_sample_scratch_bytes(int V, size_t* bytes);
 int rgbm_bn_per_sample(int dtype, void* y_dev, const void* res_dev, const float* gamma_dev, const float* beta_dev, void* scratch_dev,
                        int V, int64_t nvox, int C, int relu, void* stream);
@@ -257,6 +260,8 @@
 int rgbm_resize_bilinear_ac(int dtype, const void* in_dev, void* out_dev, int V, int Hs, int Ws, int C, int Ho, int Wo,
                             void* stream);
 int rgbm_adaptive_avgpool(int dtype, const void* in_dev, void* out_dev, int V, int H, int W, int C, int S, void* stream);
+int rgbm_adaptive_avgpool_multi(int dtype, const void* in_dev, int ldi, void* const* outs_dev, const int32_t* bins, int nb, int V, int H, int W,
+                                int C, void* stream);
 int rgbm_build_volume(int dtype, const void* feat_dev, const float* P_views_dev, const float* depths_dev, float* homog_scratch,
                       void* vol_dev, int V, int B, int D, int H, int W, void* stream);
 int rgbm_conv0_sweep(const void* feat_dev, const float* P_views_dev, const float* depths_dev, float* homog_scratch,
diff --git a/rgbmanip_amd/_lib.py b/rgbmanip_amd/_lib.py
--- a/rgbmanip_amd/_lib.py
+++ b/rgbmanip_amd/_lib.py
@@ -155,6 +155,7 @@
     "rgbm_conv_nd": (_i, [_i, _vp, _i, _i, _i, _i, _i, _i, _vp, _i, _i, _i, _i, _i, _i, _i, _i, _i, _i, _i, _vp, _vp, _vp,
                           _vp, _i, _i, _f, _vp, _vp]),
     "rgbm_conv_plan": (_i, [_i] * 23 + [C.POINTER(C.c_int32)]),
+    "rgbm_conv_plan_ex": (_i, [_i] * 25 + [C.POINTER(C.c_int32)]),
     "rgbm_bn_per_sample_scratch_bytes": (_i, [_i, C.POINTER(_sz)]),
     "rgbm_bn_per_sample": (_i, [_i, _vp, _vp, _vp, _vp, _vp, _i, _i64, _i, _i, _vp]),
     "rgbm_conv3d_tile": (_i, [_i, _i, _vp, _i, _i, _i, _i, _vp, _vp, _vp, _vp, _vp, _vp]),
@@ -164,6 +165,7 @@
     "rgbm_maxpool3x3s2": (_i, [_i, _vp, _vp, _i, _i, _i, _i, _vp]),
     "rgbm_resize_bilinear_ac": (_i, [_i, _vp, _vp, _i, _i, _i, _i, _i, _i, _vp]),
     "rgbm_adaptive_avgpool": (_i, [_i, _vp, _vp, _i, _i, _i, _i, _i, _vp]),
+    "rgbm_adaptive_avgpool_multi": (_i, [_i, _vp, _i, C.POINTER(C.c_void_p), C.POINTER(C.c_int32), _i, _i, _i, _i, _i, _vp]),
     "rgbm_build_volume": (_i, [_i, _vp, _vp, _vp, _vp, _vp, _i, _i, _i, _i, _i, _vp]),
     "rgbm_conv0_sweep": (_i, [_vp, _vp, _vp, _vp, _vp, _vp, _vp, _vp, _i, _i, _i, _i, _i, _vp]),
     "rgbm_conv0_sweep_dt": (_i, [_i, _vp, _vp, _vp, _vp, _vp, _vp, _vp, _vp, _i, _i, _i, _i, _i, _vp]),
diff --git a/rgbmanip_amd/csrc/adapose.cpp b/rgbmanip_amd/csrc/adapose.cpp
--- a/rgbmanip_amd/csrc/adapose.cpp
+++ b/rgbmanip_amd/csrc/adapose.cpp
@@ -418,7 +418,7 @@
     if (int rc = launch_copy_channels(dtype, f, bf.cat, (long long)V * H * W, 512, 1024, 0, s)) return rc;
     {
       void* outs[4] = {bf.pooled[0], bf.pooled[1], bf.pooled[2], bf.pooled[3]};
-      if (int rc = launch_adaptive_avgpool_multi(dtype, f, outs, kPspBins, 4, V, H, W, 512, s)) return rc;
+      if (int rc = launch_adaptive_avgpool_multi(dtype, f, 512, outs, kPspBins, 4, V, H, W, 512, s)) return rc;
     }
     for (int i = 0; i < 4; ++i) {
       const int Sb = kPspBins[i];
@@ -435,12 +435,12 @@
       if (int rc = launch_psp_pool_conv(dtype, f, 512, w, outs, kPspBins, V, H, W, psp[0].g.act, psp[0].g.slope, s)) return rc;
     } else {
       void* outs[4] = {bf.pooled[0], bf.pooled[1], bf.pooled[2], bf.pooled[3]};
-      if (int rc = launch_adaptive_avgpool_multi(dtype, f, outs, kPspBins, 4, V, H, W, 512, s)) return rc;
+      if (int rc = launch_adaptive_avgpool_multi(dtype, f, 512, outs, kPspBins, 4, V, H, W, 512, s, bf.cat, 1024)) return rc;
       for (int i = 0; i < 4; ++i)
         if (int rc = psp[i].run(bf.pooled[i], bf.stage[i], V, 1, kPspBins[i], kPspBins[i], 128, nullptr, 0, nullptr, 0, s)) return rc;
     }
     const void* stages[4] = {bf.stage[0], bf.stage[1], bf.stage[2], bf.stage[3]};
-    if (int rc = launch_psp_resize_cat(dtype, f, stages, kPspBins, bf.cat, V, H, W, s)) return rc;
+    if (int rc = launch_psp_resize_cat(dtype, small ? f : nullptr, stages, kPspBins, bf.cat, V, H, W, s)) return rc;
   }
   RGBM_REQUIRE(drop == nullptr || (upconv & 3) == 3, "dropout needs option upconv bits 0 and 1 (up_1 / up_2 through the tap combination)");
   if (samples > 1) {
diff --git a/rgbmanip_amd/csrc/capi.cpp b/rgbmanip_amd/csrc/capi.cpp
--- a/rgbmanip_amd/csrc/capi.cpp
+++ b/rgbmanip_amd/csrc/capi.cpp
@@ -595,16 +595,24 @@
 int rgbm_conv_plan(int dtype, int N, int D, int H, int W, int Cin, int Cin_pad, int Cout, int Cout_pad, int KD, int KH, int KW,
                    int stride_d, int stride_hw, int pad_d, int pad_hw, int dil_hw, int transposed, int has_bias, int res_mode, int act,
                    int cls, int n_cu, int32_t* plan) {
+  return rgbm_conv_plan_ex(dtype, N, D, H, W, Cin, Cin_pad, Cout, Cout_pad, KD, KH, KW, stride_d, stride_hw, pad_d, pad_hw, dil_hw, transposed,
+                           has_bias, res_mode, act, cls, n_cu, Cout_pad, 0, plan);
+}
+
+int rgbm_conv_plan_ex(int dtype, int N, int D, int H, int W, int Cin, int Cin_pad, int Cout, int Cout_pad, int KD, int KH, int KW,
+                      int stride_d, int stride_hw, int pad_d, int pad_hw, int dil_hw, int transposed, int has_bias, int res_mode, int act,
+                      int cls, int n_cu, int ldo, int res_offset_bytes, int32_t* plan) {
   RGBM_REQUIRE(plan && n_cu >= 0 && dtype >= F32 && dtype <= BF16X3 && N > 0 && D > 0 && H > 0 && W > 0, "conv_plan arguments");
+  RGBM_REQUIRE(ldo >= Cout_pad && res_offset_bytes >= 0 && res_offset_bytes < 16, "conv_plan_ex arguments");
   const ConvGeom g = conv_nd_geom(Cin, Cout, KD, KH, KW, stride_d, stride_hw, pad_d, pad_hw, dil_hw, transposed, act, 0.f);
   PackedConv pc;
   if (int rc = conv_pack_geom(g, dtype, Cin_pad, Cout_pad, cls, &pc)) return rc;
   ConvDesc d;
-  conv_desc_geom(d, g, pc, Cin_pad, Cout_pad, N, D, H, W, Cout_pad, cls);
-  alignas(16) static const float buffer[4] = {};
+  conv_desc_geom(d, g, pc, Cin_pad, Cout_pad, N, D, H, W, ldo, cls);
+  alignas(16) static const float buffer[8] = {};
   d.in = d.wgt = buffer; d.out = const_cast<float*>(buffer);
   d.bias = has_bias ? buffer : nullptr;
-  d.res = res_mode != RES_NONE ? buffer : nullptr;
+  d.res = res_mode != RES_NONE ? reinterpret_cast<const char*>(buffer) + res_offset_bytes : nullptr;
   d.res_mode = res_mode;
   ConvTuning t;
   ConvPlan p;
@@ -659,6 +667,13 @@
 }
 int rgbm_adaptive_avgpool(int dtype, const void* in_dev, void* out_dev, int V, int H, int W, int C, int S, void* stream) {
   return launch_adaptive_avgpool(dtype, in_dev, out_dev, V, H, W, C, S, (hipStream_t)stream);
+}
+int rgbm_adaptive_avgpool_multi(int dtype, const void* in_dev, int ldi, void* const* outs_dev, const int32_t* bins, int nb, int V, int H, int W,
+                                int C, void* stream) {
+  RGBM_REQUIRE(in_dev && outs_dev && bins && nb >= 1 && nb <= 4 && V > 0 && H > 0 && W > 0 && C > 0, "adaptive_avgpool_multi arguments");
+  int b[4] = {1, 1, 1, 1};
+  for (int i = 0; i < nb; ++i) { RGBM_REQUIRE(bins[i] >= 1 && outs_dev[i], "adaptive_avgpool_multi bins / outputs"); b[i] = bins[i]; }
+  return launch_adaptive_avgpool_multi(dtype, in_dev, ldi, outs_dev, b, nb, V, H, W, C, (hipStream_t)stream);
 }
 int rgbm_build_volume(int dtype, const void* feat_dev, const float* P_views_dev, const float* depths_dev, float* homog_scratch,
                       void* vol_dev, int V, int B, int D, int H, int W, void* stream) {
diff --git a/rgbmanip_amd/csrc/conv_igemm_glds.hip b/rgbmanip_amd/csrc/conv_igemm_glds.hip
--- a/rgbmanip_amd/csrc/conv_igemm_glds.hip
+++ b/rgbmanip_amd/csrc/conv_igemm_glds.hip
@@ -1217,8 +1217,9 @@
 #include "conv_igemm_m32.inc"
 
 
-template <bool RH, typename T>
+template <bool RH, typename T, bool RES = false>
 __global__ __launch_bounds__(768) void conv_igemm_ws64_kernel(const ConvDesc d) {
+  static_assert(RH || !RES, "the residual path exists in the row-halo variant only");
   constexpr int BCH = 64, BPIX = 256;
   constexpr int E = 8, BK = 64;
   constexpr int XR = BPIX / 32;
@@ -1324,6 +1325,63 @@
         }
       }
     };
+    if constexpr (RES) {
+      const T* __restrict__ res = reinterpret_cast<const T*>(d.res);
+      uint4 rv[4];
+      auto row_offset = [&](int k, int i, long long& o) -> bool {
+        const long long m = (long long)tile_of(k) * BPIX + r0 + 32 * i;
+        if (m >= d.M) return false;
+        unsigned n, qd, qh, qw;
+        decode_row(d, (unsigned)m, n, qd, qh, qw);
+        o = ((((long long)n * d.Do + (qd * d.osd + d.opd)) * d.Ho + (qh * d.osh + d.oph)) * d.Wo + (qw * d.osw + d.opw)) * d.ldo + ch;
+        return true;
+      };
+      auto request = [&](int k, int kt) {
+#pragma unroll
+        for (int j = 0; j < 4; ++j) {
+          const int i = kt * per + j;
+          rv[j] = make_uint4(0u, 0u, 0u, 0u);
+          long long o;
+          if (j < per && i < 8 && nch > 0 && row_offset(k, i, o)) {
+            if (nch >= 8) rv[j] = *reinterpret_cast<const uint4*>(res + o);
+            else { const uint2 h = *reinterpret_cast<const uint2*>(res + o); rv[j] = make_uint4(h.x, h.y, 0u, 0u); }
+          }
+        }
+      };
+      request(0, 0);
+      for (int k = 0; k < n_my; ++k)
+        for (int kt = 0; kt < KT; ++kt) {
+          RGBM_BARRIER();
+          if (kt >= KT - 1) continue;
+          uint4 dv[4];
+#pragma unroll
+          for (int j = 0; j < 4; ++j) {
+            const int i = kt * per + j;
+            if (j < per && i < 8) {
+              uint4* slot = reinterpret_cast<uint4*>(stg + (r0 + 32 * i) * SROW + c * 16);
+              dv[j] = *slot;
+              *slot = rv[j];
+            }
+          }
+          asm volatile("s_waitcnt lgkmcnt(0)" ::: "memory");
+          if (k > 0 && nch > 0) {
+#pragma unroll
+            for (int j = 0; j < 4; ++j) {
+              const int i = kt * per + j;
+              long long o;
+              if (j < per && i < 8 && row_offset(k - 1, i, o)) {
+                if (nch >= 8) *reinterpret_cast<uint4*>(out + o) = dv[j];
+                else *reinterpret_cast<uint2*>(out + o) = make_uint2(dv[j].x, dv[j].y);
+              }
+            }
+          }
+          if (kt + 1 < KT - 1) request(k, kt + 1);
+          else if (k + 1 < n_my) request(k + 1, 0);
+        }
+      RGBM_BARRIER();
+      flush(n_my - 1, 0, 8);
+      return;
+    }
     int g = 0;
     for (int k = 0; k < n_my; ++k)
       for (int kt = 0; kt < KT; ++kt, ++g) {
@@ -1598,10 +1656,21 @@
 #pragma unroll
           for (int a = 0; a < FM; ++a) {
             float v[4];
-#pragma unroll
-            for (int e = 0; e < 4; ++e) {
-              const float x = acc[a][b][e];
-              v[e] = ACT == ACT_RELU ? (x < 0.f ? 0.f : x) : ACT == ACT_PRELU ? (x < 0.f ? x * slope : x) : x;
+            if constexpr (RES) {
+              const float nslope = ACT == ACT_RELU ? 0.f : ACT == ACT_PRELU ? slope : 1.f;
+              float rf[4];
+              load4(reinterpret_cast<const T*>(stg + row * SROW + (a * 16 + lg * 4) * 2), rf);
+#pragma unroll
+              for (int e = 0; e < 4; ++e) {
+                const float x = acc[a][b][e] + rf[e];
+                v[e] = x < 0.f ? __builtin_fmaxf(x, -3.402823466e38f) * nslope : x;
+              }
+            } else {
+#pragma unroll
+              for (int e = 0; e < 4; ++e) {
+                const float x = acc[a][b][e];
+                v[e] = ACT == ACT_RELU ? (x < 0.f ? 0.f : x) : ACT == ACT_PRELU ? (x < 0.f ? x * slope : x) : x;
+              }
             }
             store4(reinterpret_cast<T*>(stg + row * SROW + (a * 16 + lg * 4) * 2), v);
           }
@@ -1655,11 +1724,16 @@
   make_fastdiv(d.Dq, d.fd_m[2], d.fd_s[2]);
   if (int rc = ensure_dynamic_lds(reinterpret_cast<const void*>(conv_igemm_ws64_kernel<false, T>), 160 * 1024)) return rc;
   if (int rc = ensure_dynamic_lds(reinterpret_cast<const void*>(conv_igemm_ws64_kernel<true, T>), 160 * 1024)) return rc;
+  if (int rc = ensure_dynamic_lds(reinterpret_cast<const void*>(conv_igemm_ws64_kernel<true, T, true>), 160 * 1024)) return rc;
+  const bool with_res = d.res_mode != RES_NONE;
+  RGBM_REQUIRE(!with_res || (rh && d.res_mode == RES_PRE_ACT && d.res && !d.w2 && (!d.bias || d.bias_stride == 0) && d.act != ACT_TANH),
+               "ws64 residual path");
   int n_cu = 0;
   if (int rc = persistent_grid_cus(&n_cu)) return rc;
   const int grid = d.n_tiles < n_cu ? d.n_tiles : n_cu;
   prof_begin_launch(s, 15, d.algo_flops, d.algo_bytes);
-  if (rh) hipLaunchKernelGGL((conv_igemm_ws64_kernel<true, T>), dim3((unsigned)grid), dim3(768), LDS, s, d);
+  if (with_res) hipLaunchKernelGGL((conv_igemm_ws64_kernel<true, T, true>), dim3((unsigned)grid), dim3(768), LDS, s, d);
+  else if (rh) hipLaunchKernelGGL((conv_igemm_ws64_kernel<true, T>), dim3((unsigned)grid), dim3(768), LDS, s, d);
   else hipLaunchKernelGGL((conv_igemm_ws64_kernel<false, T>), dim3((unsigned)grid), dim3(768), LDS, s, d);
   prof_end_launch(s);
   RGBM_CHECK_HIP(hipGetLastError());
diff --git a/rgbmanip_amd/csrc/conv_plan.cpp b/rgbmanip_amd/csrc/conv_plan.cpp
--- a/rgbmanip_amd/csrc/conv_plan.cpp
+++ b/rgbmanip_amd/csrc/conv_plan.cpp
@@ -137,6 +137,9 @@
     }
     return pick(CONV_WS, 128, 256);
   }
+  if (bits16 && uni && !(f & (DBG_NO_WS64 | DBG_NO_ROWHALO | DBG_NO_WS64_RESIDUAL)) && d.Cout == 64 && d.res_mode == RES_PRE_ACT && d.res != nullptr &&
+      rows16 && d.w2 == nullptr && ws_rows && rowhalo_ok(d) && (d.bias == nullptr || d.bias_stride == 0) && d.act != ACT_TANH)
+    return pick(CONV_WS64_ROWHALO, 64, 256);
   if (bits16 && uni && !(f & DBG_NO_WS64) && ch_tile == 64 && d.res_mode == RES_NONE && d.KT >= 2 && ws_rows &&
       (d.w2 ? d.Cout == 64 && d.kpad2 == 64 && (d.cout2 == 16 || d.cout2 == 32) && d.ldo2 % 4 == 0 : out16))
     return rowhalo_ok(d) && !(f & DBG_NO_ROWHALO) ? pick(CONV_WS64_ROWHALO, 64, 256) : pick(CONV_WS64, 64, 256);
diff --git a/rgbmanip_amd/csrc/kernels.h b/rgbmanip_amd/csrc/kernels.h
--- a/rgbmanip_amd/csrc/kernels.h
+++ b/rgbmanip_amd/csrc/kernels.h
@@ -11,8 +11,8 @@
                               int ch_off, hipStream_t s);
 int launch_copy_channels(int dtype, const void* in, void* out, long long npix, int C, int ldo, int ch_off, hipStream_t s);
 int launch_adaptive_avgpool(int dtype, const void* in, void* out, int V, int H, int W, int C, int S, hipStream_t s);
-int launch_adaptive_avgpool_multi(int dtype, const void* in, void* const* outs, const int* bins, int nb, int V, int H, int W, int C,
-                                  hipStream_t s);
+int launch_adaptive_avgpool_multi(int dtype, const void* in, int ldi, void* const* outs, const int* bins, int nb, int V, int H, int W, int C,
+                                  hipStream_t s, void* copy = nullptr, int ldc = 0);
 int launch_psp_pool_conv(int dtype, const void* in, int ldi, const void* const* w, void* const* outs, const int* bins, int V, int H, int W,
                          int act, float slope, hipStream_t s);
 int launch_psp_resize_cat(int dtype, const void* f, const void* const* stages, const int* bins, void* out, int V, int Ho, int Wo, hipStream_t s);
@@ -135,7 +135,7 @@
   DBG_PSP_STAGE_R5 = 1024, DBG_POINT_MLP_R5 = 2048, DBG_TILE_CONV0 = 4096, DBG_NO_KSPLIT = 16384, DBG_L2_SLIM_TILE = 32768,
   DBG_WS_128x256 = 65536, DBG_NO_SLIM64 = 262144, DBG_KORDER_TAPS_OUTER = 1 << 20, DBG_SWEEP_ALT_BLEND = 1 << 21, DBG_SWEEP_DOT2 = 1 << 22,
   DBG_PP_ONE_KERNEL = 1 << 23, DBG_NO_SLIM_SMALL = 1 << 24, DBG_PP_GENERIC_SELECT = 1 << 25, DBG_PP_GUARD = 1 << 26, DBG_GLOBAL_ADDR = 1 << 27,
-  DBG_SWEEP_PER_TILE = 1 << 28, DBG_SPARSE_TAIL_R5 = 1 << 29, DBG_M32_TAILS_R5 = 1 << 30, DBG_POSE_MLP_R6 = 1 << 19,
+  DBG_SWEEP_PER_TILE = 1 << 28, DBG_SPARSE_TAIL_R5 = 1 << 29, DBG_M32_TAILS_R5 = 1 << 30, DBG_POSE_MLP_R6 = 1 << 19, DBG_POOL_PER_CELL = 32, DBG_NO_WS64_RESIDUAL = 2,
 };
 extern int g_debug_flags;
 extern long long g_ws_min_rows;
diff --git a/rgbmanip_amd/csrc/misc_kernels.hip b/rgbmanip_amd/csrc/misc_kernels.hip
--- a/rgbmanip_amd/csrc/misc_kernels.hip
+++ b/rgbmanip_amd/csrc/misc_kernels.hip
@@ -295,10 +295,11 @@
   return 0;
 }
 
-struct PoolBins { void* out[4]; int S[4]; int first[5]; int n; };
-
-template <typename T>
-__global__ __launch_bounds__(512) void adaptive_avgpool_kernel(const T* __restrict__ in, const PoolBins pb, int V, int H, int W, int C) {
+struct PoolBins { void* out[4]; int S[4]; int first[5]; int n; int copy_grid; };
+constexpr int kPoolMaxRows = 16;
+
+template <typename T>
+__global__ __launch_bounds__(512) void adaptive_avgpool_kernel(const T* __restrict__ in, const PoolBins pb, int V, int H, int W, int C, int ldi) {
   constexpr int E = 16 / sizeof(T);
   constexpr int PL = 8;
   __shared__ float red[PL][64][E];
@@ -326,7 +327,7 @@
       for (int p = pl; p < npx; p += PL) {
         const int h = h0 + p / ww, w = w0 + p % ww;
         float x[E];
-        unpack_chunk(*reinterpret_cast<const uint4*>(in + ((v * H + h) * W + w) * C + cc * E), x, T());
+        unpack_chunk(*reinterpret_cast<const uint4*>(in + ((v * H + h) * W + w) * ldi + cc * E), x, T());
 #pragma unroll
         for (int e = 0; e < E; ++e) acc[e] += x[e];
       }
@@ -347,10 +348,91 @@
   }
 }
 
-int launch_adaptive_avgpool_multi(int dtype, const void* in, void* const* outs, const int* bins, int nb, int V, int H, int W, int C,
-                                  hipStream_t s) {
+template <typename T>
+__global__ __launch_bounds__(1024) void adaptive_avgpool_lines_kernel(const T* __restrict__ in, const PoolBins pb, int V, int H, int W, int C, int ldi,
+                                                                       T* __restrict__ copy, int ldc) {
+  constexpr int E = 16 / sizeof(T);
+  constexpr int PL = 8, CK = 8, U = 8;
+  __shared__ float red[kPoolMaxRows][PL][CK][E];
+  const int wave = __builtin_amdgcn_readfirstlane((int)(threadIdx.x >> 6));
+  int g = 0, sy = wave;
+#pragma unroll
+  for (int i = 0; i < 4; ++i)
+    if (g == i && i < pb.n && sy >= pb.S[i]) { sy -= pb.S[i]; g = i + 1; }
+  if (g >= pb.n) return;
+  const int lane = threadIdx.x & 63, pl = lane >> 3, ck = lane & 7;
+  const int ngrp = C / (CK * E);
+  const int grp = blockIdx.x % ngrp;
+  const long long v = blockIdx.x / ngrp;
+  const int cc = grp * CK + ck;
+  const int S = pb.S[g];
+  T* __restrict__ out = reinterpret_cast<T*>(pb.out[g]);
+  const T* __restrict__ base = in + v * H * W * ldi + cc * E;
+  T* __restrict__ cbase = copy != nullptr && g == pb.copy_grid ? copy + v * H * W * ldc + cc * E : nullptr;
+  float (*my)[CK][E] = red[wave];
+  {
+    const int h0 = (sy * H) / S, h1 = ((sy + 1) * H + S - 1) / S;
+    for (int sx = 0; sx < S; ++sx) {
+      const int w0 = (sx * W) / S, w1 = ((sx + 1) * W + S - 1) / S;
+      const int ww = w1 - w0, npx = (h1 - h0) * ww;
+      const int trips = (npx + PL - 1) / PL;
+      const int dh = PL / ww, dw = PL % ww;
+      int h = h0, w = w0 + pl;
+      while (w >= w1) { w -= ww; ++h; }
+      float acc[E];
+#pragma unroll
+      for (int e = 0; e < E; ++e) acc[e] = 0.f;
+      for (int t = 0; t < trips; t += U) {
+        uint4 x[U];
+#pragma unroll
+        for (int u = 0; u < U; ++u) {
+          x[u] = make_uint4(0u, 0u, 0u, 0u);
+          if (t + u < trips) {
+            if (h < h1) {
+              x[u] = *reinterpret_cast<const uint4*>(base + (long long)(h * W + w) * ldi);
+              if (cbase) *reinterpret_cast<uint4*>(cbase + (long long)(h * W + w) * ldc) = x[u];
+            }
+            h += dh; w += dw;
+            if (w >= w1) { w -= ww; ++h; }
+          }
+        }
+#pragma unroll
+        for (int u = 0; u < U; ++u) {
+          if (t + u < trips) {
+            float xf[E];
+            unpack_chunk(x[u], xf, T());
+#pragma unroll
+            for (int e = 0; e < E; ++e) acc[e] += xf[e];
+          }
+        }
+      }
+      __builtin_amdgcn_fence(__ATOMIC_ACQ_REL, "wavefront");
+#pragma unroll
+      for (int e = 0; e < E; ++e) my[pl][ck][e] = acc[e];
+      __builtin_amdgcn_fence(__ATOMIC_ACQ_REL, "wavefront");
+      if (pl < E) {
+        float t = my[0][ck][pl];
+#pragma unroll
+        for (int q = 1; q < PL; ++q) t += my[q][ck][pl];
+        my[0][ck][pl] = t * (1.0f / (float)npx);
+      }
+      __builtin_amdgcn_fence(__ATOMIC_ACQ_REL, "wavefront");
+      if (pl == 0) {
+        float r[E];
+#pragma unroll
+        for (int e = 0; e < E; ++e) r[e] = my[0][ck][e];
+        *reinterpret_cast<uint4*>(out + (v * S * S + sy * S + sx) * C + cc * E) = pack_chunk(r, T());
+      }
+    }
+  }
+}
+
+int launch_adaptive_avgpool_multi(int dtype, const void* in, int ldi, void* const* outs, const int* bins, int nb, int V, int H, int W, int C,
+                                  hipStream_t s, void* copy, int ldc) {
   const int E = dtype_chunk(dtype);
   RGBM_REQUIRE(C % E == 0 && nb >= 1 && nb <= 4, "avgpool channel alignment / bin count");
+  RGBM_REQUIRE(ldi >= C && ldi % E == 0 && H > 0 && W > 0 && (long long)H * W < (1ll << 31), "avgpool row stride / grid");
+  RGBM_REQUIRE(copy == nullptr || (ldc >= C && ldc % E == 0), "avgpool copy row stride");
   PoolBins pb;
   pb.n = nb;
   pb.first[0] = 0;
@@ -359,24 +441,44 @@
     pb.S[i] = i < nb ? bins[i] : 1;
     pb.first[i + 1] = pb.first[i] + (i < nb ? bins[i] * bins[i] : 0);
   }
-  pb.first[nb] = pb.first[nb];
+  int rows = 0;
+  pb.copy_grid = 0;
+  for (int i = 0; i < nb; ++i) { rows += bins[i]; if (bins[i] > bins[pb.copy_grid]) pb.copy_grid = i; }
+  if (C % (8 * E) == 0 && rows <= kPoolMaxRows && !(g_debug_flags & DBG_POOL_PER_CELL)) {
+    const long long groups = (long long)V * (C / (8 * E));
+    RGBM_REQUIRE(groups > 0 && groups < (1ll << 31), "avgpool grid");
+    if (dtype == BF16)
+      hipLaunchKernelGGL(adaptive_avgpool_lines_kernel<unsigned short>, dim3((unsigned)groups), dim3(64 * rows), 0, s, (const unsigned short*)in, pb, V, H, W, C, ldi, (unsigned short*)copy, ldc);
+    else if (dtype == F16)
+      hipLaunchKernelGGL(adaptive_avgpool_lines_kernel<f16_t>, dim3((unsigned)groups), dim3(64 * rows), 0, s, (const f16_t*)in, pb, V, H, W, C, ldi, (f16_t*)copy, ldc);
+    else if (dtype == BF16X3)
+      hipLaunchKernelGGL(adaptive_avgpool_lines_kernel<bx3_t>, dim3((unsigned)groups), dim3(64 * rows), 0, s, (const bx3_t*)in, pb, V, H, W, C, ldi, (bx3_t*)copy, ldc);
+    else
+      hipLaunchKernelGGL(adaptive_avgpool_lines_kernel<float>, dim3((unsigned)groups), dim3(64 * rows), 0, s, (const float*)in, pb, V, H, W, C, ldi, (float*)copy, ldc);
+    RGBM_CHECK_HIP(hipGetLastError());
+    return 0;
+  }
+  if (copy != nullptr) {
+    RGBM_REQUIRE(ldi == C, "avgpool copy beside the per-cell kernel needs a dense input");
+    if (int rc = launch_copy_channels(dtype, in, copy, (long long)V * H * W, C, ldc, 0, s)) return rc;
+  }
   const long long blocks = (long long)V * pb.first[nb];
   RGBM_REQUIRE(blocks > 0 && blocks < (1ll << 31), "avgpool grid");
   if (dtype == BF16)
-    hipLaunchKernelGGL(adaptive_avgpool_kernel<unsigned short>, dim3((unsigned)blocks), dim3(512), 0, s, (const unsigned short*)in, pb, V, H, W, C);
+    hipLaunchKernelGGL(adaptive_avgpool_kernel<unsigned short>, dim3((unsigned)blocks), dim3(512), 0, s, (const unsigned short*)in, pb, V, H, W, C, ldi);
   else if (dtype == F16)
-    hipLaunchKernelGGL(adaptive_avgpool_kernel<f16_t>, dim3((unsigned)blocks), dim3(512), 0, s, (const f16_t*)in, pb, V, H, W, C);
+    hipLaunchKernelGGL(adaptive_avgpool_kernel<f16_t>, dim3((unsigned)blocks), dim3(512), 0, s, (const f16_t*)in, pb, V, H, W, C, ldi);
   else if (dtype == BF16X3)
-    hipLaunchKernelGGL(adaptive_avgpool_kernel<bx3_t>, dim3((unsigned)blocks), dim3(512), 0, s, (const bx3_t*)in, pb, V, H, W, C);
+    hipLaunchKernelGGL(adaptive_avgpool_kernel<bx3_t>, dim3((unsigned)blocks), dim3(512), 0, s, (const bx3_t*)in, pb, V, H, W, C, ldi);
   else
-    hipLaunchKernelGGL(adaptive_avgpool_kernel<float>, dim3((unsigned)blocks), dim3(512), 0, s, (const float*)in, pb, V, H, W, C);
+    hipLaunchKernelGGL(adaptive_avgpool_kernel<float>, dim3((unsigned)blocks), dim3(512), 0, s, (const float*)in, pb, V, H, W, C, ldi);
   RGBM_CHECK_HIP(hipGetLastError());
   return 0;
 }
 
 int launch_adaptive_avgpool(int dtype, const void* in, void* out, int V, int H, int W, int C, int S, hipStream_t s) {
   void* outs[1] = {out};
-  return launch_adaptive_avgpool_multi(dtype, in, outs, &S, 1, V, H, W, C, s);
+  return launch_adaptive_avgpool_multi(dtype, in, C, outs, &S, 1, V, H, W, C, s);
 }
 
 struct PspStage { const void* in[4]; const void* w[4]; void* out[4]; int S[4]; int first[5]; float sy[4], sx[4]; };
@@ -469,16 +571,18 @@
   }
 }
 
-template <typename T>
+template <typename T, bool COPY>
 __global__ __launch_bounds__(256) void psp_resize_cat_kernel(const T* __restrict__ f, const PspStage ps, T* __restrict__ out, int V, int Ho, int Wo) {
   constexpr int E = 16 / sizeof(T);
-  constexpr int CF = 512, CO = 128, CPS = CO / E, CPF = CF / E, CPP = CPF + 4 * CPS;
+  constexpr int CF = 512, CO = 128, CPS = CO / E, CPF = CF / E, CPO = CPF + 4 * CPS;
+  constexpr int CPP = COPY ? CPO : 4 * CPS;
   const long long total = (long long)V * Ho * Wo * CPP;
   for (long long i = blockIdx.x * (long long)blockDim.x + threadIdx.x; i < total; i += (long long)gridDim.x * blockDim.x) {
-    const int cp = (int)(i % CPP);
+    const int cp = (int)(i % CPP) + (COPY ? 0 : CPF);
     long long t = i / CPP;
-    if (cp < CPF) {
-      reinterpret_cast<uint4*>(out)[i] = *reinterpret_cast<const uint4*>(f + t * CF + cp * E);
+    const long long oi = t * CPO + cp;
+    if (COPY && cp < CPF) {
+      reinterpret_cast<uint4*>(out)[oi] = *reinterpret_cast<const uint4*>(f + t * CF + cp * E);
       continue;
     }
     const int cq = cp - CPF;
@@ -496,7 +600,7 @@
     unpack_chunk(*reinterpret_cast<const uint4*>(base + ((long long)ly.i1 * S + lx.i1) * CO), dd, T());
 #pragma unroll
     for (int e = 0; e < E; ++e) r[e] = bilerp(a[e], b[e], c[e], dd[e], lx, ly);
-    reinterpret_cast<uint4*>(out)[i] = pack_chunk(r, T());
+    reinterpret_cast<uint4*>(out)[oi] = pack_chunk(r, T());
   }
 }
 
@@ -533,7 +637,7 @@
 
 int launch_psp_resize_cat(int dtype, const void* f, const void* const* stages, const int* bins, void* out, int V, int Ho, int Wo, hipStream_t s) {
   const int E = dtype_chunk(dtype);
-  RGBM_REQUIRE(V > 0 && f && out, "psp resize arguments");
+  RGBM_REQUIRE(V > 0 && out, "psp resize arguments");
   PspStage ps{};
   if (int rc = psp_stage_desc(bins, ps)) return rc;
   for (int i = 0; i < 4; ++i) {
@@ -541,15 +645,15 @@
     ps.sy[i] = Ho > 1 ? (float)(bins[i] - 1) / (float)(Ho - 1) : 0.f;
     ps.sx[i] = Wo > 1 ? (float)(bins[i] - 1) / (float)(Wo - 1) : 0.f;
   }
-  const long long total = (long long)V * Ho * Wo * (1024 / E);
-  if (dtype == BF16)
-    hipLaunchKernelGGL(psp_resize_cat_kernel<unsigned short>, dim3(grid_for(total)), dim3(256), 0, s, (const unsigned short*)f, ps, (unsigned short*)out, V, Ho, Wo);
-  else if (dtype == F16)
-    hipLaunchKernelGGL(psp_resize_cat_kernel<f16_t>, dim3(grid_for(total)), dim3(256), 0, s, (const f16_t*)f, ps, (f16_t*)out, V, Ho, Wo);
-  else if (dtype == BF16X3)
-    hipLaunchKernelGGL(psp_resize_cat_kernel<bx3_t>, dim3(grid_for(total)), dim3(256), 0, s, (const bx3_t*)f, ps, (bx3_t*)out, V, Ho, Wo);
-  else
-    hipLaunchKernelGGL(psp_resize_cat_kernel<float>, dim3(grid_for(total)), dim3(256), 0, s, (const float*)f, ps, (float*)out, V, Ho, Wo);
+  const bool copy = f != nullptr;
+  const long long total = (long long)V * Ho * Wo * ((copy ? 1024 : 512) / E);
+#define RGBM_PSP_CAT(T, COPY) \
+  hipLaunchKernelGGL((psp_resize_cat_kernel<T, COPY>), dim3(grid_for(total)), dim3(256), 0, s, (const T*)f, ps, (T*)out, V, Ho, Wo)
+  if (dtype == BF16) { if (copy) RGBM_PSP_CAT(unsigned short, true); else RGBM_PSP_CAT(unsigned short, false); }
+  else if (dtype == F16) { if (copy) RGBM_PSP_CAT(f16_t, true); else RGBM_PSP_CAT(f16_t, false); }
+  else if (dtype == BF16X3) { if (copy) RGBM_PSP_CAT(bx3_t, true); else RGBM_PSP_CAT(bx3_t, false); }
+  else { if (copy) RGBM_PSP_CAT(float, true); else RGBM_PSP_CAT(float, false); }
+#undef RGBM_PSP_CAT
   RGBM_CHECK_HIP(hipGetLastError());
   return 0;
 }
```

New measurement: 5870 (median of 6 runs). No clear change (+0.5%).
